# dkouzoup/ms-eetc

Hardware: AMD Instinct MI355X
Metric: OCP solves/sec (N=100, VIRM6, var-speed-limit track) (higher is better)
Workload: dtype f64

## Files before the change

__graft_entry__.py:

```python

import os
import subprocess
import sys
from pathlib import Path

ROOT = Path(__file__).resolve().parent
PKG = ROOT / 'ms-eetc_amd'

for p in (str(PKG), str(ROOT), str(ROOT / 'tests')):
    if p not in sys.path:
        sys.path.insert(0, p)

HIPCC = os.environ.get('HIPCC', '/opt/rocm/bin/hipcc')
HIP_FLAGS = ['--offload-arch=gfx950', '-O3', '-std=c++17', '-fPIC', '-shared', '-Wno-unused-value']
SOLVE_KERNEL_FLAGS = ['-fno-unroll-loops']


def _digest(sources, extra=()):

    import hashlib
    h = hashlib.sha256()
    for s in sources:
        h.update(s.name.encode()); h.update(s.read_bytes())
    for e in extra:
        h.update(str(e).encode())
    return h.hexdigest()


def _stale(target, digest):
    stamp = target.with_name(target.name + '.stamp')
    return (not target.exists()) or (not stamp.exists()) or stamp.read_text().strip() != digest


def _locked(path):

    import contextlib
    import fcntl

    @contextlib.contextmanager
    def cm():
        path.parent.mkdir(exist_ok=True)
        with open(path, 'w') as fh:
            fcntl.flock(fh, fcntl.LOCK_EX)
            try:
                yield
            finally:
                fcntl.flock(fh, fcntl.LOCK_UN)

    return cm()


def _jobs():

    if os.environ.get('MAX_JOBS', '').isdigit() and int(os.environ['MAX_JOBS']) > 0:
        return int(os.environ['MAX_JOBS'])
    n = len(os.sched_getaffinity(0))
    try:
        quota, period = open('/sys/fs/cgroup/cpu.max').read().split()[:2]
        if quota != 'max':
            n = min(n, max(1, int(float(quota)/float(period))))
    except Exception:
        pass
    return n


UNITS = ['msd_api.hip', 'msd_kernels_full.hip', 'msd_kernels_full2.hip', 'msd_kernels_full3.hip', 'msd_kernels_full4.hip', 'msd_kernels_rg.hip', 'msd_kernels_rg2.hip', 'msd_kernels_static.hip', 'msd_kernels_time.hip', 'msd_kernels_time2.hip', 'msd_kernels_dynamic.hip', 'msd_kernels_dynamic2.hip', 'msd_kernels_dynamic3.hip', 'msd_kernels_stream.hip', 'msd_kernels_stream2.hip', 'msd_kernels_stream3.hip', 'msd_kernels_stream4.hip', 'msd_kernels_stream5.hip', 'msd_kernels_stream6.hip', 'msd_kernels_stream7.hip', 'msd_kernels_compose.hip', 'msd_kernels_general.hip', 'msd_kernels_general2.hip', 'msd_kernels_intloss.hip', 'msd_kernels_intloss_table.hip', 'msd_kernels_intloss_table2.hip', 'msd_post.hip',
         'msd_integrators.hip', 'msd_mpc.hip']
SLOWEST_FIRST = ['msd_kernels_stream7.hip', 'msd_kernels_stream2.hip', 'msd_kernels_stream6.hip', 'msd_kernels_stream5.hip', 'msd_kernels_dynamic.hip', 'msd_kernels_stream3.hip',
                 'msd_kernels_stream4.hip', 'msd_kernels_intloss.hip', 'msd_kernels_compose.hip', 'msd_kernels_static.hip', 'msd_kernels_stream.hip']
HOST_UNITS = ('msd_api.hip', 'msd_mpc.hip')
HOST_ONLY_HEADERS = ('msd_handle.hpp', 'msd_select.hpp')


def _unit_headers(u):
    csrc = PKG / 'csrc'
    host = u in HOST_UNITS
    return ([h for h in sorted(csrc.glob('*.hpp')) if host or h.name not in HOST_ONLY_HEADERS] + [ROOT / 'include' / 'mseetc_hip.h']
            + ([ROOT / 'include' / 'mseetc_mpc.h', ROOT / 'include' / 'mseetc_aux.h'] if host else []))


def _hip_digest():
    csrc = PKG / 'csrc'
    deps = [csrc / u for u in UNITS] + sorted(csrc.glob('*.hpp')) + [ROOT / 'include' / 'mseetc_hip.h', ROOT / 'include' / 'mseetc_mpc.h', ROOT / 'include' / 'mseetc_aux.h']
    return _digest(deps, HIP_FLAGS + SOLVE_KERNEL_FLAGS)


def hip_digest():

    return _hip_digest()


def stale():

    return _stale(PKG / 'lib' / 'libmseetc_hip.so', _hip_digest())


def build(force=False):

    lib = PKG / 'lib' / 'libmseetc_hip.so'
    csrc = PKG / 'csrc'
    units = UNITS

    digest = _hip_digest()

    import contextlib
    from oracle import oracle
    fresh = not force and not _stale(lib, digest) and not oracle.stale()

    with (contextlib.nullcontext() if fresh else _locked(PKG / 'lib' / '.build.lock')):
        if force or _stale(lib, digest):
            objdir = PKG / 'lib' / 'obj'
            objdir.mkdir(exist_ok=True)
            flags = [f for f in HIP_FLAGS if f != '-shared']
            todo = []
            for u in units:
                fl = flags + (SOLVE_KERNEL_FLAGS if u.startswith('msd_kernels_') else [])
                obj = objdir / (u + '.o')
                dg = _digest([csrc / u] + _unit_headers(u), fl)
                if force or _stale(obj, dg):
                    todo.append((u, fl, obj, dg))
            from concurrent.futures import ThreadPoolExecutor
            todo.sort(key=lambda t: SLOWEST_FIRST.index(t[0]) if t[0] in SLOWEST_FIRST else len(SLOWEST_FIRST))
            with ThreadPoolExecutor(max_workers=_jobs()) as pool:
                codes = list(pool.map(lambda t: subprocess.call([HIPCC] + t[1] + ['-c', '-o', str(t[2]), str(csrc / t[0])]), todo))
            if any(codes):
                raise RuntimeError("hipcc failed: {}".format(codes))
            for u, fl, obj, dg in todo:
                obj.with_name(obj.name + '.stamp').write_text(dg)
            tmp = lib.with_name(lib.name + '.tmp')
            subprocess.run([HIPCC, '--offload-arch=gfx950', '-shared', '-fPIC', '-o', str(tmp)] + [str(objdir / (u + '.o')) for u in units], check=True)
            os.replace(tmp, lib)
            lib.with_name(lib.name + '.stamp').write_text(digest)

        oracle.build(force)

    import mseetc.ocp
    import mseetc._device

    return lib


def smoke():

    import numpy as np

    build()

    import cases
    from mseetc.ocp import casadiSolver
# ... 28 lines not shown
```

include/mseetc_aux.h:

```cpp
#ifndef MSEETC_AUX_H
#define MSEETC_AUX_H

#include "mseetc_hip.h"

#ifdef __cplusplus
extern "C" {
#endif

int msd_problem_time_first_pass(msd_handle h, int on);
int msd_problem_first_pass_ms(msd_handle h, float *mean_ms, int *launches);

int msd_host_alloc(unsigned long long bytes, void **ptr);
int msd_host_free(void *ptr);

int msd_problem_direct_results(msd_handle h, int on);

int msd_tuning(const char *name, int value);

int msd_plan_describe(const msd_problem_desc *desc, char *buf, int len);

int msd_fastmath_probe(int device, int n, const double *x, double *rcp_out, double *sqrt_out, double *rsqrt_out);

#ifdef __cplusplus
}
#endif
#endif
```

ms-eetc_amd/csrc/msd_api.hip:

```cpp
#include <hip/hip_runtime.h>
#include <dlfcn.h>

#include <algorithm>
#include <cmath>
#include <cstdio>
#include <cstdlib>
#include <cstring>
#include <map>
#include <mutex>
#include <string>
#include <utility>
#include <vector>

#include "msd_handle.hpp"

namespace {
thread_local std::string g_err;
}

#define MSD_KERNEL_UNITS(X) X(full) X(full2) X(full3) X(full4) X(rg) X(rg2) X(static) X(time) X(time2) X(dynamic) X(dynamic2) X(dynamic3) X(stream) X(stream2) X(stream3) \
    X(stream4) X(stream5) X(stream6) X(stream7) X(compose) X(general) X(general2) X(intloss) X(intloss_table) X(intloss_table2)
namespace msd {
#define X(unit) KernelFn kernels_##unit(const KernelId &id);
MSD_KERNEL_UNITS(X)
#undef X
}

namespace msd_host {
int fail(int code, const std::string &msg) { g_err = msg; return code; }
Tuning &tuning() { static Tuning t; return t; }

msd::KernelFn find_kernel(const msd::KernelId &id)
{
    if (!id) return nullptr;
#define X(unit) if (const msd::KernelFn fn = msd::kernels_##unit(id)) return fn;
    MSD_KERNEL_UNITS(X)
#undef X
    return nullptr;
}
bool has_kernel(const msd::KernelId &id) { return find_kernel(id) != nullptr; }
}
using msd_host::fail;

namespace msd_host {

int check_desc(const msd_problem_desc *d)
{
    if (d->abi_version != MSD_ABI_VERSION) return fail(MSD_E_INVALID, "ABI version mismatch");
    if (d->num_intervals < 1) return fail(MSD_E_INVALID, "Number of intervals must be a strictly positive integer!");
    if (d->max_iterations < 1) return fail(MSD_E_INVALID, "Maximum number of iterations must be a strictly positive integer!");
    if (d->num_steps < 1 || d->num_approx_steps < 0) return fail(MSD_E_INVALID, "bad integrator options");
    if (!d->ds || !d->grad || !d->curv || !d->bmax) return fail(MSD_E_INVALID, "null profile array");
    if (!(d->vmin_sq > 0) || !(d->obj_den > 0) || !(d->tol > 0)) return fail(MSD_E_INVALID, "vmin_sq, obj_den and tol must be positive");
    if (d->start_kind != MSD_START_REFERENCE && d->start_kind != MSD_START_PROFILE) return fail(MSD_E_INVALID, "unknown starting point");
    if (d->loss_kind < 0 || d->loss_kind > 2) return fail(MSD_E_UNSUPPORTED, "loss model not available on the device");
    if (d->loss_kind == 2) {
        if (!d->loss_table || d->loss_table_len < 13) return fail(MSD_E_INVALID, "dynamic loss model without its table");
        const int nx = (int)d->loss_table[11], ny = (int)d->loss_table[12];
        if (nx < 1 || ny < 1 || d->loss_table_len != 13 + (nx + 1) + (ny + 1) + 16*nx*ny) return fail(MSD_E_INVALID, "inconsistent loss table");
    }
    for (int i = 0; i < d->num_intervals; i++)
        if (!(d->ds[i] > 0)) return fail(MSD_E_INVALID, "interval lengths must be positive");
    if (d->integrator != 0 && d->integrator != MSD_INTEGRATOR_ADAPTIVE && d->integrator != MSD_INTEGRATOR_COLLOCATION)
        return fail(MSD_E_INVALID, "Unknown integration method!");
    if (d->integrator == MSD_INTEGRATOR_COLLOCATION) {
        if (d->coll_degree < 1 || d->coll_degree > 9) return fail(MSD_E_INVALID, "Order of implicit Runge-Kutta should be a positive integer between 1 and 9!");
        if (d->newton_iterations < 1) return fail(MSD_E_INVALID, "Maximum number of iterations must be a strictly positive integer!");
        if (!d->coll_tables) return fail(MSD_E_INVALID, "collocation integrator without its tables");
    }
    if (d->integrator == MSD_INTEGRATOR_ADAPTIVE && (!(d->int_abstol > 0) || !(d->int_reltol > 0))) return fail(MSD_E_INVALID, "tolerances of the adaptive integrator must be positive");
    if (d->integrate_losses && d->energy_optimal && d->loss_kind == 0)
        return fail(MSD_E_UNSUPPORTED, "integrateLosses needs a loss model (loss_kind 1 or 2)");
    if (d->integrate_losses && d->energy_optimal && d->loss_kind == 2 && d->integrator != 0)
        return fail(MSD_E_UNSUPPORTED, "integrateLosses with a loss table runs with explicit Runge-Kutta shooting (integrator 0)");
    return MSD_OK;
}


static int cu_count(int device, int *out)
{
    static std::mutex mu;
    static int cached[64] = {0};
    std::lock_guard<std::mutex> lock(mu);
    if (device < 64 && cached[device] > 0) { *out = cached[device]; return MSD_OK; }
    hipDeviceProp_t prop;
    HIP_TRY(hipGetDeviceProperties(&prop, device));
    if (device < 64) cached[device] = prop.multiProcessorCount;
    *out = prop.multiProcessorCount;
    return MSD_OK;
}

static int kernel_limits(int device, const void *fn, int threads, size_t lds, int *per_cu)
{
    struct Info { size_t lds_attr = 0; std::map<size_t, int> occupancy; };
    static std::mutex mu;
    static std::map<std::pair<int, const void *>, Info> cache;
    std::lock_guard<std::mutex> lock(mu);
    Info &info = cache[{device, fn}];
    if (lds > info.lds_attr) {
        HIP_TRY(hipFuncSetAttribute(fn, hipFuncAttributeMaxDynamicSharedMemorySize, (int)lds));
        info.lds_attr = lds;
    }
    const size_t step = 8*1024, top = std::min<size_t>(((lds + step - 1)/step)*step, 160*1024);
    auto it = info.occupancy.find(top);
    if (it == info.occupancy.end()) {
        int n = 0;
        if (hipOccupancyMaxActiveBlocksPerMultiprocessor(&n, fn, threads, top) != hipSuccess || n < 1) n = 1;
        it = info.occupancy.emplace(top, n).first;
    }
    *per_cu = it->second;
    return MSD_OK;
}


int select_plan(const msd_problem_desc *d, Plan *out, msd::KernelFn *soc_out)
{
    Plan &pl = *out;
    const int N = d->num_intervals;
    const Family family = family_of(d);
    const int structure = structure_of(d);
    const bool wide = msd_host::dyn_of(family) != msd::LOSS_STATIC;
    msd::Geometry geo = resident(family, N, structure, tuning());
    if (!geo.first || lds_bytes(geo, geo.first, N) > 160*1024) {
        geo = streamed(family, N, structure, tuning());
        if (!geo.first)
            return fail(MSD_E_UNSUPPORTED, family != STATIC ? "numIntervals = " + std::to_string(N) + " exceeds the 1023 intervals of the streamed kernels for the dynamic loss model, the collocation / adaptive shooting integrators and integrateLosses"
                                           : "numIntervals = " + std::to_string(N) + " exceeds the 5119 intervals of the streamed kernel");
    }
    size_t work2 = 0;
    if (!geo.follow) {
        geo.follow = streamed(family, N, structure, tuning()).follow;
        if (!geo.follow) return fail(MSD_E_UNSUPPORTED, "no follow-up kernel for numIntervals = " + std::to_string(N));
        work2 = msd::stream_doubles(N, geo.follow.NT*geo.follow.SPT, wide);
    }
    pl.NT = geo.first.NT; pl.SPT = geo.first.SPT; pl.lds_bytes = lds_bytes(geo, geo.first, N); pl.stream = geo.stream;
    pl.NT2 = geo.follow.NT; pl.SPT2 = geo.follow.SPT; pl.lds_bytes2 = lds_bytes(geo, geo.follow, N);
    fill_problem(pl.P, d);
    pl.fused_family = geo.xch == msd::XCH_FAST;
    pl.work_doubles = geo.stream ? msd::stream_doubles(N, pl.NT*pl.SPT, wide) : std::max(work2, msd::work_doubles(std::max(pl.NT*pl.SPT, work2 ? 0 : pl.NT2*pl.SPT2)));
    pl.nz = (4 + pl.P.withPn)*N + 2; pl.nl = ((pl.P.hasPower ? 2 : 0) + 3 + (pl.P.energyOpt ? 2 : 0))*N;
    pl.kernel = find_kernel(geo.first); pl.kernel2 = find_kernel(geo.follow); pl.kernel_lsq = find_kernel(geo.lsq);
    pl.kernel_soc = nullptr;
    *soc_out = find_kernel(geo.soc);
    return MSD_OK;
}

int make_plan(int device, const msd_problem_desc *d, Plan *out)
{
    Plan &pl = *out;
    msd::KernelFn soc = nullptr;
    int rc = select_plan(d, &pl, &soc);
    if (rc != MSD_OK) return rc;
    int per_cu = 0, cus = 0;
    rc = kernel_limits(device, (const void *)pl.kernel, pl.NT, pl.lds_bytes, &per_cu);
    if (rc != MSD_OK) return rc;
    rc = cu_count(device, &cus);
    if (rc != MSD_OK) return rc;
    pl.max_grid = per_cu*cus;
    pl.max_grid2 = 0;
    if (pl.kernel2) {
        rc = kernel_limits(device, (const void *)pl.kernel2, pl.NT2, pl.lds_bytes2, &per_cu);
        if (rc != MSD_OK) return rc;
        pl.max_grid2 = per_cu*cus;
    }
    pl.max_grid_lsq = 0;
    if (pl.kernel_lsq) {
        rc = kernel_limits(device, (const void *)pl.kernel_lsq, pl.NT, pl.lds_bytes, &per_cu);
        if (rc != MSD_OK) return rc;
        pl.max_grid_lsq = per_cu*cus;
    }
    if (soc) {
        int per_cu_soc = 0;
        if (kernel_limits(device, (const void *)soc, pl.NT, pl.lds_bytes, &per_cu_soc) == MSD_OK && per_cu_soc*cus >= pl.max_grid) pl.kernel_soc = soc;
    }
    return MSD_OK;
}

void pack_profile(const msd_problem_desc *d, double *out)
{
    const int N = d->num_intervals;
    double *ds = out, *grad = ds + N, *curv = grad + N, *bmax = curv + N, *pos = bmax + N + 1;
    memcpy(ds, d->ds, sizeof(double)*N); memcpy(grad, d->grad, sizeof(double)*N); memcpy(curv, d->curv, sizeof(double)*N);
    memcpy(bmax, d->bmax, sizeof(double)*(N + 1));
    pos[0] = 0;
    for (int i = 0; i < N; i++) pos[i + 1] = pos[i] + d->ds[i];
}

static std::string kernel_name(msd::KernelFn fn)
{
    if (!fn) return "-";
    static std::mutex mu;
    static std::map<const void *, std::string> cache;
    std::lock_guard<std::mutex> lock(mu);
    std::string &name = cache[(const void *)fn];
    if (name.empty()) {
        Dl_info info;
        name = (dladdr((const void *)fn, &info) && info.dli_sname && info.dli_saddr == (const void *)fn) ? info.dli_sname : "?";
    }
    return name;
}

std::string plan_text(const Plan &pl, msd::KernelFn soc)
{
    char buf[256];
    snprintf(buf, sizeof buf, "NT=%d SPT=%d lds_bytes=%zu stream=%d fused_family=%d work_doubles=%zu nz=%d nl=%d NT2=%d SPT2=%d lds_bytes2=%zu", pl.NT, pl.SPT, pl.lds_bytes,
             (int)pl.stream, (int)pl.fused_family, pl.work_doubles, pl.nz, pl.nl, pl.NT2, pl.SPT2, pl.lds_bytes2);
    return std::string(buf) + " kernel=" + kernel_name(pl.kernel) + " kernel_lsq=" + kernel_name(pl.kernel_lsq) + " kernel2=" + kernel_name(pl.kernel2) + " kernel_soc=" + kernel_name(soc);
}

int launch_plan(const Plan &pl, hipStream_t stream, double *d_work, int *d_follow, int *d_queue, int nscen, const double *d_scen, const double *d_ovr,
                double *d_z, double *d_lam, double *d_stats, double *d_hist, int hist_cap, const WarmStart &ws, int *d_list, hipEvent_t first_begin, hipEvent_t first_end)
{
    if (!pl.kernel) return fail(MSD_E_INVALID, "the handle holds no problem: its last (re)configuration failed");
    msd::DevProb P = pl.P;
    P.follow = nullptr; P.list = nullptr; P.queue = nullptr; P.socSeen = ws.d_soc_seen;
    P.guess = ws.d_guess; P.guessStride = ws.stride; P.guessStatus = ws.d_status; P.warmMu = ws.mu; P.warmPush = ws.push;
    P.dualIn = ws.d_dual_in; P.dualInStride = ws.dual_stride; P.dualShift = ws.dual_shift; P.dualOut = ws.d_dual_out;
    P.oneAttempt = ws.one_attempt ? 1 : 0;
    P.done = ws.d_done; P.statsHost = ws.d_stats_host; P.budget = ws.budget;
    const bool split = pl.kernel2 != nullptr;
    const bool plain = !pl.fused_family || (ws.d_guess ? ws.d_dual_in != nullptr : P.start == MSD_START_PROFILE);
    const bool first_pass = split && (plain || pl.kernel_lsq != nullptr);
    if (d_list && !first_pass) {
        const msd::KernelFn fn = split ? pl.kernel2 : pl.kernel;
        const int cap = split ? pl.max_grid2 : pl.max_grid;
        P.list = d_list;
        hipLaunchKernelGGL(fn, dim3(std::min(nscen, cap)), dim3(split ? pl.NT2 : pl.NT), split ? pl.lds_bytes2 : pl.lds_bytes, stream, P, nscen, d_scen, d_ovr, d_z, d_lam, d_stats, d_hist, hist_cap, d_work);
        HIP_TRY(hipGetLastError());
        return MSD_OK;
    }
    P.list = d_list;
    const msd::KernelFn fn = (split && !first_pass) ? pl.kernel2 : plain ? ((ws.use_soc && pl.kernel_soc) ? pl.kernel_soc : pl.kernel) : pl.kernel_lsq;
    const int cap = (split && !first_pass) ? pl.max_grid2 : plain ? pl.max_grid : pl.max_grid_lsq;
    const int grid = nscen < cap ? nscen : cap;
    const int threads = (split && !first_pass) ? pl.NT2 : pl.NT;
    const size_t lds_bytes = (split && !first_pass) ? pl.lds_bytes2 : pl.lds_bytes;
    if (first_pass) {
        if (!d_follow) return fail(MSD_E_INVALID, "split solve without its list");
        P.follow = d_follow;
    }
    if (nscen > grid && !d_list) {
        if (!d_queue) return fail(MSD_E_INVALID, "launch without its scenario counter");
        P.queue = d_queue;
        HIP_TRY(hipMemsetAsync(P.queue, 0, sizeof(int), stream));
    }
    if (first_begin) HIP_TRY(hipEventRecord(first_begin, stream));
    hipLaunchKernelGGL(fn, dim3(grid), dim3(threads), lds_bytes, stream, P, nscen, d_scen, d_ovr, d_z, d_lam, d_stats, d_hist, hist_cap, d_work);
    HIP_TRY(hipGetLastError());
    if (first_end) HIP_TRY(hipEventRecord(first_end, stream));
#ifdef MSD_DEBUG_HOOKS
    const bool skip_follow_up = getenv("MSD_DEBUG_NO_FOLLOW_UP") && *getenv("MSD_DEBUG_NO_FOLLOW_UP") == '1';
#else
    constexpr bool skip_follow_up = false;
#endif
    if (first_pass && !skip_follow_up) {
        const int grid2 = std::min(nscen, pl.max_grid2);
        P.queue = nullptr; P.list = d_follow; P.follow = nullptr;
        hipLaunchKernelGGL(pl.kernel2, dim3(grid2), dim3(pl.NT2), pl.lds_bytes2, stream, P, nscen, d_scen, d_ovr, d_z, d_lam, d_stats, d_hist, hist_cap, d_work);
        HIP_TRY(hipGetLastError());
    }
    return MSD_OK;
}

}

using msd_host::check_desc;

extern "C" {

const char *msd_last_error(void) { return g_err.c_str(); }

int msd_tuning(const char *name, int value)
{
    if (!name) return fail(MSD_E_INVALID, "null argument");
    if (!strcmp(name, "no_full")) msd_host::tuning().no_full = value != 0;
    else if (!strcmp(name, "two_nodes_per_lane")) msd_host::tuning().two_nodes_per_lane = value != 0;
    else return fail(MSD_E_INVALID, std::string("unknown tuning switch: ") + name);
    return MSD_OK;
}

int msd_plan_describe(const msd_problem_desc *d, char *buf, int len)
{
    if (!d || !buf || len < 1) return fail(MSD_E_INVALID, "null argument");
    int rc = check_desc(d);
    if (rc != MSD_OK) return rc;
    msd_host::Plan pl;
    msd::KernelFn soc = nullptr;
    rc = msd_host::select_plan(d, &pl, &soc);
    if (rc != MSD_OK) return rc;
    static const char *const family[] = {"STATIC", "DYNAMIC", "INTLOSS", "INTLOSS_TABLE", "GENERAL", "GENERAL_DYNAMIC", "GENERAL_INTLOSS"};
    static const char *const structure[] = {"0", "FULL_BOTH", "FULL_RG", "FULL_TIME_BOTH", "FULL_TIME_RG"};
    const std::string line = std::string("family=") + family[msd_host::family_of(d)] + " structure=" + structure[msd_host::structure_of(d)] + " " + msd_host::plan_text(pl, soc);
    if ((int)line.size() >= len) return fail(MSD_E_INVALID, "msd_plan_describe: the line needs " + std::to_string(line.size() + 1) + " bytes");
    memcpy(buf, line.c_str(), line.size() + 1);
    return MSD_OK;
}

int msd_device_count(void)
{
    int n = 0;
    if (hipGetDeviceCount(&n) != hipSuccess) return 0;
    return n;
}

static int configure(msd_problem *h, const msd_problem_desc *d)
{
    const int N = d->num_intervals;
    msd_host::Plan pl;
    int rc = msd_host::make_plan(h->device, d, &pl);
    if (rc != MSD_OK) return rc;
    HIP_TRY(hipSetDevice(h->device));
    HIP_TRY(hipStreamSynchronize(h->stream));
    h->plan.kernel = nullptr;

    const size_t len = msd_host::profile_doubles(N);
    if (N > h->cap_N) {
        hipFree(h->d_prof); h->d_prof = nullptr; h->cap_N = 0;
        HIP_TRY(hipMalloc((void **)&h->d_prof, sizeof(double)*len));
        h->cap_N = N;
    }
    if (len > h->cap_stage) {
        if (h->h_stage) hipHostFree(h->h_stage);
        h->h_stage = nullptr; h->cap_stage = 0;
        HIP_TRY(hipHostMalloc((void **)&h->h_stage, sizeof(double)*len, hipHostMallocDefault));
        h->cap_stage = len;
    }
    msd_host::pack_profile(d, h->h_stage);
    HIP_TRY(hipMemcpyAsync(h->d_prof, h->h_stage, sizeof(double)*len, hipMemcpyHostToDevice, h->stream));
    if (d->loss_kind == 2) {
        if (d->loss_table_len > h->cap_loss) {
            hipFree(h->d_loss); h->d_loss = nullptr; h->cap_loss = 0;
            HIP_TRY(hipMalloc((void **)&h->d_loss, sizeof(double)*d->loss_table_len));
            h->cap_loss = d->loss_table_len;
        }
        HIP_TRY(hipMemcpy(h->d_loss, d->loss_table, sizeof(double)*d->loss_table_len, hipMemcpyHostToDevice));
    }

    if (d->integrator == MSD_INTEGRATOR_COLLOCATION) {
        const int len = (d->coll_degree + 1)*(d->coll_degree + 2);
        if (!h->d_coll) HIP_TRY(hipMalloc((void **)&h->d_coll, sizeof(double)*10*11));
        HIP_TRY(hipMemcpy(h->d_coll, d->coll_tables, sizeof(double)*len, hipMemcpyHostToDevice));
    }

    msd_host::point_profile(pl.P, h->d_prof);
    pl.P.loss = (d->loss_kind == 2) ? h->d_loss : nullptr;
    pl.P.coll = (d->integrator == MSD_INTEGRATOR_COLLOCATION) ? h->d_coll : nullptr;
    if (pl.work_area() > h->cap_work) {
        hipFree(h->d_work); h->d_work = nullptr; h->cap_work = 0;
        HIP_TRY(hipMalloc((void **)&h->d_work, sizeof(double)*pl.work_area()));
        h->cap_work = pl.work_area();
    }
    if (pl.nz > h->cap_nz || pl.nl > h->cap_nl) {
        hipFree(h->d_scen); hipFree(h->d_ovr); hipFree(h->d_z); hipFree(h->d_lam); hipFree(h->d_stats); hipFree(h->d_guess); hipFree(h->d_z2); hipFree(h->d_stats2);
        h->d_scen = h->d_ovr = h->d_z = h->d_lam = h->d_stats = h->d_guess = h->d_z2 = h->d_stats2 = nullptr; h->cap_scen = 0; h->cap_guess = 0;
        h->prev_nscen = 0;
        h->cap_nz = pl.nz; h->cap_nl = pl.nl;
    }
    if (pl.kernel_soc && !h->h_soc_seen) {
        HIP_TRY(hipHostMalloc((void **)&h->h_soc_seen, sizeof(int), hipHostMallocMapped));
// ... 24 lines not shown
    *out = h;
    return MSD_OK;
}

int msd_problem_reconfigure(msd_handle h, const msd_problem_desc *d)
{
    if (!h || !d) return fail(MSD_E_INVALID, "null argument");
    if (h->begun) return fail(MSD_E_INVALID, "a batch begun with msd_solve_batch_begin has not been waited for (MSD_WAIT_ALL)");
    int rc = check_desc(d);
    if (rc == MSD_OK) rc = configure(h, d);
    if (rc != MSD_OK) h->plan.kernel = nullptr;
    return rc;
}

int msd_problem_destroy(msd_handle h)
{
    if (!h) return MSD_OK;
    if (h->attached_loops > 0) return fail(MSD_E_INVALID, "a receding-horizon loop (msd_mpc_create) still runs on this handle: destroy the loop first");
    hipSetDevice(h->device);
    if (h->begun) hipStreamSynchronize(h->stream);
    hipFree(h->d_prof); hipFree(h->d_loss); hipFree(h->d_work); hipFree(h->d_queue); hipFree(h->d_follow);
    hipFree(h->d_scen); hipFree(h->d_ovr); hipFree(h->d_z); hipFree(h->d_lam); hipFree(h->d_stats); hipFree(h->d_hist); hipFree(h->d_guess); hipFree(h->d_eval);
    hipFree(h->d_z2); hipFree(h->d_stats2); hipFree(h->d_dual); hipFree(h->d_dual2); hipFree(h->d_coll);
    if (h->h_stage) hipHostFree(h->h_stage);
    if (h->h_soc_seen) hipHostFree((void *)h->h_soc_seen);
    if (h->h_done) hipHostFree((void *)h->h_done);
    if (h->h_stats_now) hipHostFree(h->h_stats_now);
    if (h->ev_first) hipEventDestroy(h->ev_first);
    for (int k = 0; k < msd_problem::FP_RING; k++) { if (h->fp_beg[k]) hipEventDestroy(h->fp_beg[k]); if (h->fp_end[k]) hipEventDestroy(h->fp_end[k]); }
    if (h->ev0) hipEventDestroy(h->ev0);
    if (h->ev1) hipEventDestroy(h->ev1);
    if (h->stream) hipStreamDestroy(h->stream);
    delete h;
    return MSD_OK;
}

int msd_problem_nz(msd_handle h) { return h ? h->plan.nz : 0; }
int msd_problem_rows_per_interval(msd_handle h) { return h ? h->plan.nl/h->plan.P.N : 0; }

constexpr int QUEUE_RING = 64;

using msd_host::WarmStart;

static int launch(msd_handle h, int nscen, const double *d_scen, const double *d_ovr, double *d_z, double *d_lam, double *d_stats, double *d_hist, int hist_cap,
                  const WarmStart &ws_in = WarmStart())
{
    if (!h->plan.kernel) return fail(MSD_E_INVALID, "the handle holds no problem: its last (re)configuration failed");
    WarmStart ws = ws_in;
    ws.budget = h->budget;
    if (h->plan.kernel_soc) {
        ws.d_soc_seen = h->d_soc_seen;
        if (*h->h_soc_seen != 0) ws.use_soc = true;
    }
    if (h->plan.kernel2) {
        const size_t need = msd::FOLLOW_HDR + 2*(size_t)nscen;
        if (need > h->cap_follow) {
            HIP_TRY(hipStreamSynchronize(h->stream));
            int keep[msd::FOLLOW_HDR] = {0};
            if (h->d_follow) HIP_TRY(hipMemcpy(keep, h->d_follow, sizeof(int)*msd::FOLLOW_HDR, hipMemcpyDeviceToHost));
            keep[0] = keep[1] = keep[2] = 0;
            hipFree(h->d_follow); h->d_follow = nullptr; h->cap_follow = 0;
            HIP_TRY(hipMalloc((void **)&h->d_follow, sizeof(int)*need));
            HIP_TRY(hipMemcpy(h->d_follow, keep, sizeof(int)*msd::FOLLOW_HDR, hipMemcpyHostToDevice));
            h->cap_follow = need;
        }
    }
    if (!h->d_queue) HIP_TRY(hipMalloc((void **)&h->d_queue, sizeof(int)*QUEUE_RING));
    int *queue = h->d_queue + h->queue_slot;
    h->queue_slot = (h->queue_slot + 1) % QUEUE_RING;
    hipEvent_t e0 = nullptr, e1 = nullptr;
    if (h->time_first_pass && !ws.d_done) {
        const int k = (int)(h->fp_count % msd_problem::FP_RING);
        if (!h->fp_beg[k]) { HIP_TRY(hipEventCreate(&h->fp_beg[k])); HIP_TRY(hipEventCreate(&h->fp_end[k])); }
        e0 = h->fp_beg[k]; e1 = h->fp_end[k];
        h->fp_count++;
    }
    if (ws.d_done) e1 = h->ev_first;
#ifdef MSD_DEBUG_HOOKS
    if (getenv("MSD_DEBUG_PTRS"))
        fprintf(stderr, "[msd] launch nscen %d  work %p (+%zu B)  follow %p  queue %p  prof %p  scen %p  z %p  lam %p  stats %p  hist %p  %s  grid caps %d %d %d\n",
                nscen, (void *)h->d_work, sizeof(double)*h->cap_work, (void *)h->d_follow, (void *)queue, (void *)h->d_prof, (const void *)d_scen, (void *)d_z, (void *)d_lam, (void *)d_stats, (void *)d_hist,
                msd_host::plan_text(h->plan, h->plan.kernel_soc).c_str(), h->plan.max_grid, h->plan.max_grid_lsq, h->plan.max_grid2);
#endif
    return msd_host::launch_plan(h->plan, h->stream, h->d_work, h->d_follow, queue, nscen, d_scen, d_ovr, d_z, d_lam, d_stats, d_hist, hist_cap, ws, nullptr, e0, e1);
}

int msd_solve_batch_device(msd_handle h, int nscen, const double *d_scen, double *d_z, double *d_lam, double *d_stats)
{
    return msd_solve_batch_device_ex(h, nscen, d_scen, nullptr, d_z, d_lam, d_stats);
}

int msd_solve_batch_device_ex(msd_handle h, int nscen, const double *d_scen, const double *d_overrides, double *d_z, double *d_lam, double *d_stats)
{
    if (!h || nscen < 1 || !d_scen || !d_z || !d_stats) return fail(MSD_E_INVALID, "bad argument");
    if (h->begun) return fail(MSD_E_INVALID, "a batch begun with msd_solve_batch_begin has not been waited for (MSD_WAIT_ALL)");
    HIP_TRY(hipSetDevice(h->device));
    return launch(h, nscen, d_scen, d_overrides, d_z, d_lam, d_stats, nullptr, 0);
}

int msd_problem_geometry(msd_handle h, int *threads_per_scenario, int *nodes_per_thread)
{
    if (!h || !threads_per_scenario || !nodes_per_thread) return fail(MSD_E_INVALID, "bad argument");
    *threads_per_scenario = h->plan.NT; *nodes_per_thread = h->plan.SPT;
    return MSD_OK;
}

int msd_problem_follow_counts(msd_handle h, int *counts, int n)
{
    if (!h || !counts || n < 1) return fail(MSD_E_INVALID, "bad argument");
#ifdef MSD_DEBUG_HOOKS
    if (n > 9 && !(getenv("MSD_DEBUG_NO_FOLLOW_UP") && *getenv("MSD_DEBUG_NO_FOLLOW_UP") == '1')) n = 9;
#else
    if (n > 9) n = 9;
#endif
    if (n > (int)h->cap_follow - msd::FOLLOW_TOTAL && h->d_follow) n = (int)h->cap_follow - msd::FOLLOW_TOTAL;
    for (int k = 0; k < n; k++) counts[k] = 0;
    HIP_TRY(hipSetDevice(h->device));
    HIP_TRY(hipStreamSynchronize(h->stream));
    if (h->d_follow) HIP_TRY(hipMemcpy(counts, h->d_follow + msd::FOLLOW_TOTAL, sizeof(int)*n, hipMemcpyDeviceToHost));
    return MSD_OK;
}

int msd_problem_time_first_pass(msd_handle h, int on)
{
    if (!h) return fail(MSD_E_INVALID, "null handle");
    h->time_first_pass = on != 0; h->fp_count = 0;
    return MSD_OK;
}

int msd_problem_first_pass_ms(msd_handle h, float *mean_ms, int *launches)
{
    if (!h || !mean_ms || !launches) return fail(MSD_E_INVALID, "bad argument");
    HIP_TRY(hipSetDevice(h->device));
    HIP_TRY(hipStreamSynchronize(h->stream));
    const int n = (int)std::min<long long>(h->fp_count, msd_problem::FP_RING);
    double sum = 0;
    for (int k = 0; k < n; k++) { float ms = 0; HIP_TRY(hipEventElapsedTime(&ms, h->fp_beg[k], h->fp_end[k])); sum += ms; }
    *mean_ms = n ? (float)(sum/n) : 0.0f; *launches = n;
    return MSD_OK;
}

int msd_synchronize(msd_handle h)
{
    if (!h) return fail(MSD_E_INVALID, "null handle");
    HIP_TRY(hipSetDevice(h->device));
    HIP_TRY(hipStreamSynchronize(h->stream));
    return MSD_OK;
}

int msd_set_history(msd_handle h, double *host_hist, int cap)
{
    if (!h) return fail(MSD_E_INVALID, "null handle");
    h->h_hist = host_hist; h->hist_cap = host_hist ? cap : 0;
    return MSD_OK;
}

int msd_solve_batch(msd_handle h, int nscen, const double *scen, double *z_out, double *lam_out, double *stats, float *kernel_ms)
{
    return msd_solve_batch_ex(h, nscen, scen, nullptr, z_out, lam_out, stats, kernel_ms);
}

int msd_solve_batch_ex(msd_handle h, int nscen, const double *scen, const double *overrides, double *z_out, double *lam_out, double *stats, float *kernel_ms)
{
    return msd_solve_batch_warm(h, nscen, scen, overrides, nullptr, 0.0, 0.0, z_out, lam_out, stats, kernel_ms);
}

static int check_batch(msd_handle h, int nscen, const double *scen, const double *overrides, const double *z_guess, double mu_init, double bound_push,
// ... 372 lines not shown
```

ms-eetc_amd/csrc/msd_geometry.hpp:

```cpp
#pragma once

#include "msd_kernel.hpp"

namespace msd {

using KernelFn = void (*)(DevProb, int, const double *, const double *, double *, double *, double *, double *, int, double *);

struct KernelId {
    int NT = 0, SPT = 0, WPS = 1, DYN = LOSS_STATIC;
    bool STREAM = false, GEN = false;
    int FULL = 0, PART = 0;
    bool SLDS = false, SOCK = false;
    explicit operator bool() const { return NT != 0; }
};
inline bool operator==(const KernelId &a, const KernelId &b)
{
    return a.NT == b.NT && a.SPT == b.SPT && a.WPS == b.WPS && a.DYN == b.DYN && a.STREAM == b.STREAM && a.GEN == b.GEN && a.FULL == b.FULL && a.PART == b.PART
           && a.SLDS == b.SLDS && a.SOCK == b.SOCK;
}

#define MSD_KERNEL(...) if (id == KernelId{__VA_ARGS__}) return solve_kernel<__VA_ARGS__>;
#define MSD_KERNEL_UNUSED(...) if (false) return solve_kernel<__VA_ARGS__>;

struct Geometry {
    KernelId first;
    KernelId follow;
    KernelId lsq;
    KernelId soc;
    bool stream = false;
    int xch = XCH_GENERAL;
    int red = RED_DOUBLES;
    int extra = 0;
};

}
```

ms-eetc_amd/csrc/msd_handle.hpp:

```cpp
#pragma once
#include <hip/hip_runtime.h>

#include <algorithm>
#include <cmath>
#include <string>

#include "msd_kernel.hpp"
#include "msd_geometry.hpp"
#include "msd_select.hpp"
#include "../../include/mseetc_aux.h"

namespace msd_host {

int fail(int code, const std::string &msg);

#define HIP_TRY(expr)                                                                                               \
    do {                                                                                                            \
        hipError_t e_ = (expr);                                                                                     \
        if (e_ != hipSuccess) return msd_host::fail(MSD_E_HIP, std::string(#expr) + ": " + hipGetErrorString(e_));  \
    } while (0)

struct Plan {
    msd::DevProb P;
    int NT = 0, SPT = 0;
    size_t lds_bytes = 0;
    bool stream = false;
    msd::KernelFn kernel = nullptr;
    msd::KernelFn kernel_lsq = nullptr;
    msd::KernelFn kernel2 = nullptr;
    msd::KernelFn kernel_soc = nullptr;
    int NT2 = 0, SPT2 = 0;
    size_t lds_bytes2 = 0;
    int max_grid = 0, max_grid_lsq = 0, max_grid2 = 0;
    bool fused_family = false;
    size_t work_doubles = 0;
    size_t work_area() const { return work_doubles*(size_t)std::max(max_grid, std::max(max_grid2, max_grid_lsq)); }
    int nz = 0, nl = 0;
};

int check_desc(const msd_problem_desc *d);
int select_plan(const msd_problem_desc *d, Plan *out, msd::KernelFn *soc);
int make_plan(int device, const msd_problem_desc *d, Plan *out);
std::string plan_text(const Plan &pl, msd::KernelFn soc);

Tuning &tuning();
msd::KernelFn find_kernel(const msd::KernelId &id);

constexpr size_t profile_doubles(int N) { return 5*(size_t)N + 2; }
void pack_profile(const msd_problem_desc *d, double *out);
inline void point_profile(msd::DevProb &P, const double *d_prof) { P.ds = d_prof; P.grad = P.ds + P.N; P.curv = P.grad + P.N; P.bmax = P.curv + P.N; P.pos = P.bmax + P.N + 1; }

struct WarmStart { const double *d_guess = nullptr; long long stride = 0; const double *d_status = nullptr; double mu = 0, push = 0;
                   const double *d_dual_in = nullptr; long long dual_stride = 0; int dual_shift = 0; double *d_dual_out = nullptr;
                   bool one_attempt = false;
                   bool use_soc = false;
                   int *d_soc_seen = nullptr;
                   int *d_done = nullptr; double *d_stats_host = nullptr;
                   int budget = 0; };

int launch_plan(const Plan &pl, hipStream_t stream, double *d_work, int *d_follow, int *d_queue, int nscen, const double *d_scen, const double *d_ovr,
                double *d_z, double *d_lam, double *d_stats, double *d_hist, int hist_cap, const WarmStart &ws, int *d_list = nullptr,
                hipEvent_t first_begin = nullptr, hipEvent_t first_end = nullptr);

}

struct msd_problem {
    msd_host::Plan plan;
    int device = 0;
    volatile int *h_soc_seen = nullptr;
    int *d_soc_seen = nullptr;
    int *d_follow = nullptr; size_t cap_follow = 0;
    hipStream_t stream = nullptr;
    hipEvent_t ev0 = nullptr, ev1 = nullptr;
    double *d_prof = nullptr, *d_loss = nullptr;
    double *h_stage = nullptr; size_t cap_stage = 0;
    double *d_work = nullptr;
    double *d_eval = nullptr; size_t cap_eval = 0;
    int *d_queue = nullptr;
    int queue_slot = 0;
    size_t cap_work = 0;
    int cap_N = 0, cap_loss = 0, cap_nz = 0, cap_nl = 0;
    double *d_scen = nullptr, *d_ovr = nullptr, *d_z = nullptr, *d_lam = nullptr, *d_stats = nullptr, *d_hist = nullptr, *d_guess = nullptr;
    double *d_z2 = nullptr, *d_stats2 = nullptr;
    int prev_nscen = 0, prev_nz = 0, prev_stp = 0;
    bool direct_results = false, last_direct = false;
    bool keep_duals = false;
    double *d_dual = nullptr, *d_dual2 = nullptr;
    double *d_coll = nullptr;
    size_t cap_dual = 0;
    int prev_dual_nodes = 0;
    int cap_scen = 0, cap_guess = 0;
    double *h_hist = nullptr;
    int hist_cap = 0;
    static constexpr int FP_RING = 64;
    bool time_first_pass = false;
    hipEvent_t fp_beg[FP_RING] = {}, fp_end[FP_RING] = {};
    long long fp_count = 0;
    bool early_results = false;
    int budget = 0;
    volatile int *h_done = nullptr; int *d_done = nullptr;
    double *h_stats_now = nullptr, *d_stats_now = nullptr;
    int cap_done = 0;
    int begun = 0;
    hipEvent_t ev_first = nullptr;
    int attached_loops = 0;
};
```

ms-eetc_amd/csrc/msd_kernel.hpp:

```cpp
#pragma once
#include <type_traits>

#include <hip/hip_runtime.h>

#include <float.h>
#include <math.h>

#include "../../include/mseetc_hip.h"
#include "msd_fastmath.hpp"
#include "msd_scan.hpp"

#ifndef MSD_PHASE_FENCE
#define MSD_PHASE_FENCE 1
#endif
#ifndef MSD_FENCE_PHASES
#define MSD_FENCE_PHASES 0x155
#endif
#ifndef MSD_HOT_FENCES
#define MSD_HOT_FENCES 0
#endif
#ifndef MSD_FENCE_MAX_NT
#define MSD_FENCE_MAX_NT 256
#endif
#ifndef MSD_FENCE_DUALS
// ... 393 lines not shown
    c.red_slot++;
    if (c.lane == 0) {
#pragma unroll
        for (int k = 0; k < K; k++) buf[c.wave*RED_K + k] = v[k];
    }
    __syncthreads();
#pragma unroll
    for (int k = 0; k < K; k++) {
        double r = buf[k];
        for (int w = 1; w < c.nw; w++) r = op(r, buf[w*RED_K + k]);
        v[k] = r;
    }
}

#ifndef MSD_HOST_EMULATION
template <int K> __device__ __forceinline__ void wave_fetch(const double (&x)[K], double (&y)[K], int src)
{
    const int addr = (src & 63) << 2;
#pragma unroll
    for (int k = 0; k < K; k++) {
        const int lo = __builtin_amdgcn_ds_bpermute(addr, __double2loint(x[k]));
        const int hi = __builtin_amdgcn_ds_bpermute(addr, __double2hiint(x[k]));
        y[k] = __hiloint2double(hi, lo);
    }
}
#else
template <int K> __device__ __forceinline__ void wave_fetch(const double (&x)[K], double (&y)[K], int src)
{
    emu_wave_fetch(x, y, K, src);
}
#endif

__device__ __forceinline__ void bar_terms(double x, double lb, double ub, bool hasL, bool hasU, double zL, double zU, double mu, double &Sg, double &gphi)
{
    double S = 0, g = 0;
    if (hasL) { S += zL/(x - lb); g -= mu/(x - lb); }
    if (hasU) { S += zU/(ub - x); g += mu/(ub - x); }
    if (hasL && !hasU) g += K_D*mu;
    if (!hasL && hasU) g -= K_D*mu;
    Sg = S; gphi = g;
}

__device__ __forceinline__ double sigma_clamp(double z, double mu, double s)
{
    const double r = mu/s;
    return fmax(fmin(z, K_SIGMA*r), r*(1.0/K_SIGMA));
}

__device__ __forceinline__ double push_in(double x, double lb, double ub, bool hasL, bool hasU, double kp)
{
    if (hasL && hasU) {
        double pL = fmin(kp*fmax(1.0, fabs(lb)), kp*(ub - lb));
        double pU = fmin(kp*fmax(1.0, fabs(ub)), kp*(ub - lb));
        if (x < lb + pL) x = lb + pL;
        if (x > ub - pU) x = ub - pU;
    } else if (hasL) { double pL = kp*fmax(1.0, fabs(lb)); if (x < lb + pL) x = lb + pL; }
    else if (hasU) { double pU = kp*fmax(1.0, fabs(ub)); if (x > ub - pU) x = ub - pU; }
    return x;
}

__device__ __forceinline__ double hpow(double x, double y)
{
    static_assert(K_MU_SUP == 1.5, "mu^1.5 is computed as mu*sqrt(mu) in the barrier update");
#ifndef MSD_HPOW
#define MSD_HPOW 1
#endif
    return MSD_HPOW ? (double)exp2f((float)y*log2f((float)x)) : pow(x, y);
}

struct LogSum {
    double m = 1.0;
    int e = 0;
#ifndef MSD_LOGSUM
#define MSD_LOGSUM 1
#endif
    double acc = 0.0;
    __device__ __forceinline__ void add(double prod) { if (MSD_LOGSUM) { int ex; m *= frexp(prod, &ex); e += ex; } else acc += log(prod); }
    __device__ __forceinline__ double value() const { return MSD_LOGSUM ? log(m) + 0.6931471805599453*(double)e : acc; }
};

__device__ __forceinline__ bool cmp_le(double lhs, double rhs, double basval) { return lhs - rhs <= 10.0*DBL_EPSILON*fabs(basval); }

constexpr unsigned F_ON_T = 1u, F_ON_B = 2u, F_ON_F = 4u, F_ON_P = 8u, F_ON_S = 16u, F_IVAL = 32u, F_NODE = 64u;

template <int CNT, int NS, bool MEM> struct Field;
template <int CNT, int NS> struct Field<CNT, NS, false> {
    static constexpr bool in_memory = false;
    double v[CNT];
    __device__ __forceinline__ void bind(double *) {}
    __device__ __forceinline__ double &operator[](int k) { return v[k]; }
    __device__ __forceinline__ const double &operator[](int k) const { return v[k]; }
};
template <int CNT, int NS> struct Field<CNT, NS, true> {
    static constexpr bool in_memory = true;
    double *p;
    __device__ __forceinline__ void bind(double *q) { p = q; }
    __device__ __forceinline__ double &operator[](int k) const { return p[k*NS]; }
};

constexpr int W_X = 0, W_SG = 5, W_LAM = 10, W_NU = 12, W_ZL = 17, W_ZU = 22, W_ZLS = 27, W_ZUS = 32, W_DSG = 37, W_RESC = 42, W_RESD = 44,
              W_EV = 49, W_LG = 62, W_LG_FIELDS = 30, W_FIELDS_ITERATE = W_LG + W_LG_FIELDS;
constexpr int W_SC = W_FIELDS_ITERATE, W_RN = W_SC + 2, W_RP = W_SC + 9, W_RZN = W_SC + 16, W_RZP = W_SC + 23, W_RDN = W_SC + 30, W_RDP = W_SC + 37, W_RDZN = W_SC + 44,
              W_RDZP = W_SC + 51, W_XR = W_SC + 58, W_SGR = W_SC + 63, W_OZL = W_SC + 68, W_OZU = W_SC + 73, W_OZLS = W_SC + 78, W_OZUS = W_SC + 83, W_RD = W_SC + 88,
              W_DNU = W_SC + 90, W_RFILT = W_SC + 95, W_SCAL = W_SC + 97, W_RTMP = W_SC + 98;
constexpr int W_WD = W_SC + 103, W_WD_FIELDS = 37;
static_assert(W_DSG == W_WD_FIELDS, "the iterate proper: the fields in front of the slack steps");
constexpr int W_RX = W_WD + W_WD_FIELDS, W_RX_FIELDS = 6;
constexpr int W_FIELDS = W_RX + W_RX_FIELDS;
__host__ __device__ constexpr size_t work_doubles(int node_slots) { return (size_t)W_FIELDS*node_slots; }
__host__ __device__ constexpr size_t stream_doubles(int N, int node_slots, bool dyn)
{
    return (size_t)W_FIELDS*node_slots + (size_t)(dyn ? 31 : 27)*(N + 1) + 6*(size_t)node_slots;
}

template <int NS, bool STREAM>
struct Node {
    int i;
    unsigned flags;
    double ds, G, sct, scb, ubB;
    Field<NV, NS, STREAM> x;
    Field<NR, NS, STREAM> sg;
    Field<2, NS, STREAM> lam;
    Field<NR, NS, STREAM> nu;
    Field<NV, NS, STREAM> zL, zU;
    Field<NR, NS, STREAM> zLs, zUs;
    Field<NR, NS, STREAM> dsg;
    __device__ __forceinline__ void bind(double *w)
    {
        x.bind(w + W_X*NS); sg.bind(w + W_SG*NS); lam.bind(w + W_LAM*NS); nu.bind(w + W_NU*NS); zL.bind(w + W_ZL*NS); zU.bind(w + W_ZU*NS);
        zLs.bind(w + W_ZLS*NS); zUs.bind(w + W_ZUS*NS); dsg.bind(w + W_DSG*NS);
    }
    __device__ __forceinline__ bool ival() const { return (flags & F_IVAL) != 0; }
    __device__ __forceinline__ bool node() const { return (flags & F_NODE) != 0; }
    __device__ __forceinline__ bool on(int k) const { return (flags >> k) & 1u; }
};

struct Uni {
    double tlo, thi, blo, flo, fhi, plo, phi, slo;
    bool rowOn[NR], rL[NR], rU[NR];
    double dL[NR], dU[NR], rs[NR];
    double irs[NR];
    double sf;
};

#ifndef MSD_NODE_FENCE
#define MSD_NODE_FENCE 1
#endif
#ifndef MSD_NODE_FENCE_SITES
#define MSD_NODE_FENCE_SITES 0xFFFu
#endif
template <int SITE> __device__ __forceinline__ void node_fence() { if (MSD_NODE_FENCE && ((MSD_NODE_FENCE_SITES >> SITE) & 1u)) __builtin_amdgcn_sched_barrier(0); }

__device__ __forceinline__ void opaque(double &v) { asm volatile("" : "+v"(v)); }
#ifndef MSD_FENCE_AGPR
#define MSD_FENCE_AGPR 0
#endif
__device__ __forceinline__ void opaque_a(double &v) { asm volatile("" : "+a"(v)); }
__device__ __forceinline__ void opaque_z(double &v) { if (MSD_FENCE_AGPR >= 1) opaque_a(v); else opaque(v); }
__device__ __forceinline__ void opaque_d(double &v) { if (MSD_FENCE_AGPR >= 2) opaque_a(v); else opaque(v); }

__device__ __forceinline__ void publish_done(int *word, int v)
{
#ifdef MSD_HOST_EMULATION
    __atomic_store_n(word, v, __ATOMIC_RELEASE);
#else
    __hip_atomic_store(word, v, __ATOMIC_RELEASE, __HIP_MEMORY_SCOPE_SYSTEM);
// ... 974 lines not shown
            for (int k = 0; k < 2; k++)
#pragma unroll
                for (int m = 0; m < LGW; m++) lgs[j][LGW*k + m] = e.lg[k][m];
        }
    }
    __device__ __forceinline__ void load_ev(int j, Ev &e) const
    {
        e.sb = evs[j][0]; e.sb1 = evs[j][1]; e.b1 = evs[j][2]; e.tb = evs[j][3]; e.tw = evs[j][4]; e.tbb = evs[j][5]; e.tbw = evs[j][6]; e.tww = evs[j][7];
        e.Bb = evs[j][8]; e.Bw = evs[j][9]; e.Bbb = evs[j][10]; e.Bbw = evs[j][11]; e.Bww = evs[j][12];
#pragma unroll
        for (int k = 0; k < 2; k++)
#pragma unroll
            for (int m = 0; m < LGW; m++) e.lg[k][m] = DYN ? lgs[j][LGW*k + m] : 0.0;
    }
    __device__ __forceinline__ void load_ev1(int j, Ev &e) const
    {
        e.sb = evs[j][0]; e.sb1 = evs[j][1]; e.b1 = evs[j][2]; e.tb = evs[j][3]; e.tw = evs[j][4]; e.Bb = evs[j][8]; e.Bw = evs[j][9];
        e.tbb = e.tbw = e.tww = e.Bbb = e.Bbw = e.Bww = 0;
#pragma unroll
        for (int k = 0; k < 2; k++)
#pragma unroll
            for (int m = 0; m < LGW; m++) e.lg[k][m] = DYN ? lgs[j][LGW*k + m] : 0.0;
    }
    static constexpr unsigned H_X = 1u, H_SG = 2u, H_LAM = 4u, H_NU = 8u, H_Z = 16u, H_ZS = 32u, H_DSG = 64u, H_RES = 128u, H_EV = 256u, H_ALL = 511u;
    template <int CNT, class F> __device__ __forceinline__ void put(const F &f, int off, int slot)
    {
        if constexpr (!F::in_memory) {
#pragma unroll
            for (int k = 0; k < CNT; k++) work[(off + k)*NS + slot] = f.v[k];
        }
    }
    template <int CNT, class F> __device__ __forceinline__ void get(F &f, int off, int slot)
    {
        if constexpr (!F::in_memory) {
#pragma unroll
            for (int k = 0; k < CNT; k++) f.v[k] = work[(off + k)*NS + slot];
        }
    }
    template <unsigned M, int BASE = 0> __device__ __forceinline__ void stash()
    {
#pragma unroll
        for (int j = 0; j < SPT; j++) {
            NodeT &nd = n[j];
            const int sl = nd.i + BASE*NS;
            if (M & H_X) put<NV>(nd.x, W_X, sl);
            if (M & H_SG) put<NR>(nd.sg, W_SG, sl);
            if (M & H_LAM) put<2>(nd.lam, W_LAM, sl);
            if (M & H_NU) put<NR>(nd.nu, W_NU, sl);
            if (M & H_Z) { put<NV>(nd.zL, W_ZL, sl); put<NV>(nd.zU, W_ZU, sl); }
            if (M & H_ZS) { put<NR>(nd.zLs, W_ZLS, sl); put<NR>(nd.zUs, W_ZUS, sl); }
            if (M & H_DSG) put<NR>(nd.dsg, W_DSG, sl);
            if (M & H_RES) { put<2>(resc[j], W_RESC, sl); put<NR>(resd[j], W_RESD, sl); }
            if (M & H_EV) { put<13>(evs[j], W_EV, sl); if (DYN) put<2*LGW>(lgs[j], W_LG, sl); }
        }
        asm volatile("" ::: "memory");
    }
    template <unsigned M> __device__ __forceinline__ void fetch()
    {
        asm volatile("" ::: "memory");
#pragma unroll
        for (int j = 0; j < SPT; j++) {
            NodeT &nd = n[j];
            const int sl = nd.i;
            if (M & H_X) get<NV>(nd.x, W_X, sl);
            if (M & H_SG) get<NR>(nd.sg, W_SG, sl);
            if (M & H_LAM) get<2>(nd.lam, W_LAM, sl);
            if (M & H_NU) get<NR>(nd.nu, W_NU, sl);
            if (M & H_Z) { get<NV>(nd.zL, W_ZL, sl); get<NV>(nd.zU, W_ZU, sl); }
            if (M & H_ZS) { get<NR>(nd.zLs, W_ZLS, sl); get<NR>(nd.zUs, W_ZUS, sl); }
            if (M & H_DSG) get<NR>(nd.dsg, W_DSG, sl);
            if (M & H_RES) { get<2>(resc[j], W_RESC, sl); get<NR>(resd[j], W_RESD, sl); }
            if (M & H_EV) { get<13>(evs[j], W_EV, sl); if (DYN) get<2*LGW>(lgs[j], W_LG, sl); }
        }
    }

    template <class F> __device__ static __forceinline__ void fence_v(F &f, int k) { if constexpr (!F::in_memory) opaque(f.v[k]); }
    template <class F> __device__ static __forceinline__ void fence_z(F &f, int k) { if constexpr (!F::in_memory) opaque_z(f.v[k]); }
    template <class F> __device__ static __forceinline__ void fence_d(F &f, int k) { if constexpr (!F::in_memory) opaque_d(f.v[k]); }
    template <class F> __device__ static __forceinline__ void fence_a(F &f, int k) { if constexpr (!F::in_memory) opaque_a(f.v[k]); }

    __device__ __forceinline__ double lbv(int k) const { return k == VT ? U.tlo : k == VB ? U.blo : k == VF ? U.flo : k == VP ? U.plo : U.slo; }
    __device__ __forceinline__ double ubv(int j, int k) const { return k == VT ? U.thi : k == VB ? n[j].ubB : k == VF ? U.fhi : k == VP ? U.phi : INFINITY; }
    __device__ static __forceinline__ bool hasU(int k) { return k != VS; }

    __device__ __forceinline__ void phase_fence(int phase)
    {
#if MSD_PHASE_FENCE
        if (!MSD_HOT_FENCES && (PART == 1 || PART == 3) && FAST) return;
        if (!((MSD_FENCE_PHASES >> phase) & 1)) return;
        if (NT > MSD_FENCE_MAX_NT || STREAM) return;
#pragma unroll
        for (int j = 0; j < SPT; j++) {
            NodeT &nd = n[j];
#pragma unroll
            for (int k = 0; k < NV; k++) { fence_v(nd.x, k); if (MSD_FENCE_DUALS) { fence_z(nd.zL, k); fence_z(nd.zU, k); } }
#pragma unroll
            for (int r = 0; r < NR; r++) { fence_v(nd.sg, r); if (MSD_FENCE_DUALS) { fence_d(nd.nu, r); fence_z(nd.zLs, r); fence_z(nd.zUs, r); fence_d(nd.dsg, r); fence_d(resd[j], r); } }
            if (MSD_FENCE_DUALS) { fence_d(nd.lam, 0); fence_d(nd.lam, 1); fence_d(resc[j], 0); fence_d(resc[j], 1); }
        }
#endif
    }

    __device__ __forceinline__ void commit_uniforms(const Uni &u)
    {
        __syncthreads();
        if (c.tid == 0) U = u;
        __syncthreads();
    }

    __device__ __forceinline__ void publish(const double (&x)[SPT][NV])
    {
        __syncthreads();
#pragma unroll
        for (int j = 0; j < SPT; j++) { const int i = n[j].i; c.xt[i] = x[j][VT]; c.xb[i] = x[j][VB]; c.xf[i] = x[j][VF]; }
        __syncthreads();
    }
    __device__ __forceinline__ void publish_current()
    {
        __syncthreads();
#pragma unroll
        for (int j = 0; j < SPT; j++) { const int i = n[j].i; c.xt[i] = n[j].x[VT]; c.xb[i] = n[j].x[VB]; c.xf[i] = n[j].x[VF]; }
        __syncthreads();
    }
    __device__ __forceinline__ double nb_q(int j) const { return (n[j].i > 0 && n[j].node()) ? c.xf[n[j].i - 1] : 0.0; }

    __device__ __forceinline__ void var_terms(int j, int k, double mu_, double &Sg, double &gphi) const
    {
        bar_terms(n[j].x[k], lbv(k), ubv(j, k), true, hasU(k), n[j].zL[k], n[j].zU[k], mu_, Sg, gphi);
    }
    __device__ __forceinline__ void row_terms(int j, int r, double mu_, double &Sg, double &gphi) const
    {
        bar_terms(n[j].sg[r], U.dL[r], U.dU[r], rL(r), rU(r), n[j].zLs[r], n[j].zUs[r], mu_, Sg, gphi);
    }

    struct LossHess { double bb, bf, bp, bd, ff, fp, fd, pp, pd, dd; };
    __device__ __forceinline__ LossHess loss_hess(double f, double b, const Ev &ev) const
    {
        const double Xv = ev.lg[0][1], Xd = ev.lg[0][2], Xw = ev.lg[0][3], Xvv = ev.lg[0][4], Xvd = ev.lg[1][0], Xvw = ev.lg[1][1], Xdd = ev.lg[1][2],
                     Xdw = ev.lg[1][3], Xww = ev.lg[1][4];
        const double vb = 0.5/ev.sb, vbb = -0.25/(b*ev.sb);
        LossHess L;
        L.bb = f*(Xvv*vb*vb + Xv*vbb); L.bf = f*Xvw*vb + Xv*vb; L.bp = f*Xvw*vb; L.bd = f*Xvd*vb;
        L.ff = f*Xww + 2*Xw; L.fp = f*Xww + Xw; L.fd = f*Xdw + Xd; L.pp = f*Xww; L.pd = f*Xdw; L.dd = f*Xdd;
        return L;
    }
    __device__ __forceinline__ LossHess rows_hess(int j, double f, double b, const Ev &ev) const
    {
        LossHess L;
        if constexpr (ITAB) {
            const double vb = 0.5/ev.sb, vbb = -0.25/(b*ev.sb);
            L.bb = L.bf = L.bp = L.bd = L.ff = L.fp = L.fd = L.pp = L.pd = L.dd = 0;
#pragma unroll
            for (int k = 0; k < 2; k++) {
                const int r = (k == 0) ? RLTR : RLRG;
                const double wk = -n[j].nu[r]*U.rs[r];
                const double *E = ev.lg[k];
                const double g0 = E[1], h00 = E[5 + j4h(0, 0)], h01 = E[5 + j4h(0, 1)], h02 = E[5 + j4h(0, 2)], h03 = E[5 + j4h(0, 3)], h11 = E[5 + j4h(1, 1)],
                             h12 = E[5 + j4h(1, 2)], h13 = E[5 + j4h(1, 3)], h22 = E[5 + j4h(2, 2)], h23 = E[5 + j4h(2, 3)], h33 = E[5 + j4h(3, 3)];
                L.bb += wk*(h00*vb*vb + g0*vbb); L.bf += wk*(h02 + h03)*vb; L.bp += wk*h02*vb; L.bd += wk*h01*vb;
                L.ff += wk*(h22 + 2*h23 + h33); L.fp += wk*(h22 + h23); L.fd += wk*(h12 + h13); L.pp += wk*h22; L.pd += wk*h12; L.dd += wk*h11;
            }
        } else {
            L = loss_hess(f, b, ev);
            const double W = n[j].nu[RLTR]*U.rs[RLTR]*(-P.ct) + n[j].nu[RLRG]*U.rs[RLRG]*P.cr;
            L.bb *= W; L.bf *= W; L.bp *= W; L.bd *= W; L.ff *= W; L.fp *= W; L.fd *= W; L.pp *= W; L.pd *= W; L.dd *= W;
        }
        return L;
    }

    __device__ __forceinline__ void row_grads(int j, const Ev &ev, double (&gb)[NR], double (&gf)[NR], double (&gp)[NR], double (&gs)[NR], double (&gb1)[NR],
                                              double (&gd)[NR]) const
    {
        const double f = n[j].x[VF];
#pragma unroll
        for (int r = 0; r < NR; r++) { gb[r] = gf[r] = gp[r] = gs[r] = gb1[r] = gd[r] = 0; }
        gf[RPW0] = ev.sb; gb[RPW0] = 0.5*f/ev.sb;
        gf[RPW1] = ev.sb1; gb1[RPW1] = 0.5*f/ev.sb1;
        gf[RACC] = 1; gp[RACC] = withPn() ? 1.0 : 0.0; gb[RACC] = -(0.5*P.sr1/ev.sb + P.sr2);
        if (DYN == LOSS_INTEGRATED_TABLE) {
            const double vb = 0.5/ev.sb;
#pragma unroll
            for (int k = 0; k < 2; k++) {
                const int r = (k == 0) ? RLTR : RLRG;
                gs[r] = 1; gf[r] = -(ev.lg[k][3] + ev.lg[k][4]); gp[r] = withPn() ? -ev.lg[k][3] : 0.0; gb[r] = -ev.lg[k][1]*vb; gd[r] = -ev.lg[k][2];
            }
        } else if (DYN == LOSS_INTEGRATED) {
            const double X = ev.lg[0][0], Xv = ev.lg[0][1], Xd = ev.lg[0][2], Xw = ev.lg[0][3], vb = 0.5/ev.sb;
#pragma unroll
            for (int k = 0; k < 2; k++) {
                const int r = (k == 0) ? RLTR : RLRG;
                const double kap = (k == 0) ? -P.ct : P.cr;
                gs[r] = 1; gf[r] = kap*(X + f*Xw); gp[r] = withPn() ? kap*f*Xw : 0.0; gb[r] = kap*f*Xv*vb; gd[r] = kap*f*Xd;
            }
        } else if (DYN == LOSS_TABLE) {
            const double vb = 0.25/ev.sb, vb1 = 0.25/ev.sb1;
            gs[RLTR] = 1; gf[RLTR] = -ev.lg[0][0]; gb[RLTR] = -ev.lg[0][1]*vb; gb1[RLTR] = -ev.lg[0][1]*vb1;
            gs[RLRG] = 1; gf[RLRG] = -ev.lg[1][0]; gb[RLRG] = -ev.lg[1][1]*vb; gb1[RLRG] = -ev.lg[1][1]*vb1;
        } else {
            gs[RLTR] = 1; gf[RLTR] = -P.ct;
            gs[RLRG] = 1; gf[RLRG] = P.cr;
        }
#pragma unroll
        for (int r = 0; r < NR; r++) { gb[r] *= U.rs[r]; gf[r] *= U.rs[r]; gp[r] *= U.rs[r]; gs[r] *= U.rs[r]; gb1[r] *= U.rs[r]; gd[r] *= U.rs[r]; }
    }
    __device__ __forceinline__ void fold_running_time(const Ev &ev, double (&gb)[NR], double (&gf)[NR], double (&gp)[NR], const double (&gd)[NR]) const
    {
        if (!INTEG) return;
#pragma unroll
        for (int r = RLTR; r <= RLRG; r++) { gb[r] += gd[r]*ev.tb; gf[r] += gd[r]*ev.tw; if (withPn()) gp[r] += gd[r]*ev.tw; }
    }

    __device__ __forceinline__ void obj_grads(int j, double q, double &of, double &op, double &os, double &oq, double &off, double &opp) const
    {
        const double sc = U.sf/P.objDen;
        of = op = os = oq = off = opp = 0;
        if (!n[j].ival()) return;
        const double f = n[j].x[VF], p = withPn() ? n[j].x[VP] : 0.0;
        if (energyOpt()) {
            of = sc*n[j].ds; os = INTEG ? sc : sc*n[j].ds;
            if (n[j].i > 0) { of += sc*2e-3*(f - q); oq = -sc*2e-3*(f - q); off = sc*2e-3; }
        } else {
            of = sc*2e-4*f; off = sc*2e-4;
            if (withPn()) { op = sc*2e-4*p; opp = sc*2e-4; }
        }
    }

    struct Dir { double dx[NV], lt, lb; };
    __device__ __forceinline__ void load_dir(int j, Dir &d) const
    {
        const NodeT &nd = n[j];
#pragma unroll
        for (int k = 0; k < NV; k++) d.dx[k] = 0;
        d.lt = d.lb = 0;
        if (!nd.node()) return;
        const double *s = c.S + nd.i*S_STRIDE;
        if (nd.on(VT)) d.dx[VT] = s[S_DT];
        if (nd.on(VB)) d.dx[VB] = s[S_DB];
        if (nd.ival()) {
            if (nd.on(VF)) d.dx[VF] = s[S_DF];
            if (nd.on(VP)) d.dx[VP] = s[S_DP];
            if (nd.on(VS)) d.dx[VS] = s[S_DS];
            d.lt = s[S_LT]; d.lb = s[S_LB];
        }
    }

    struct Err { double dual, primal, primal_u, cmax, cmin, sd, sc, theta, L, D, obj; };

    struct RsSums { double theta, np, lognp, prox; };
    __device__ __forceinline__ void kkt_pass(Err &E, const bool resto = false, const double eta = 0.0, const double rho = 0.0, RsSums *RS = nullptr)
    {
        Ev e[SPT];
#pragma unroll
        for (int j = 0; j < SPT; j++) load_ev1(j, e[j]);
        double gl[SPT][NV];
        double dual = 0, prim = 0, prim_u = 0, cmax = -INFINITY, cmin = INFINITY, sumlam = 0, sumz = 0, nlam = 0, nz = 0;
        double th = 0, logs = 0, damp = 0, obj = 0;
        double rs_th = 0, rs_np = 0, rs_log = 0, rs_prox = 0, rs_prim = 0;
        LogSum lsum;
#pragma unroll
        for (int j = 0; j < SPT; j++) {
            node_fence<0>();
            const NodeT &nd = n[j];
            const double q = nb_q(j);
            double out_q = 0, out_t1 = 0, out_b1 = 0, prod = 1.0;
#pragma unroll
            for (int k = 0; k < NV; k++) gl[j][k] = 0;
            if (nd.ival()) {
                double gb[NR], gf[NR], gp[NR], gs[NR], gb1[NR], gd[NR];
                row_grads(j, e[j], gb, gf, gp, gs, gb1, gd);
                double of, op, os, oq, off, opp;
                obj_grads(j, q, of, op, os, oq, off, opp);
                if (resto) { of = op = os = oq = 0; }
                gl[j][VF] = of; gl[j][VP] = op; gl[j][VS] = os; out_q = oq;
#pragma unroll
                for (int r = 0; r < NR; r++) {
                    if (!rowOn(r)) continue;
                    gl[j][VB] += nd.nu[r]*gb[r]; gl[j][VF] += nd.nu[r]*gf[r]; gl[j][VP] += nd.nu[r]*gp[r]; gl[j][VS] += nd.nu[r]*gs[r]; out_b1 += nd.nu[r]*gb1[r];
                    if (INTEG) { out_t1 += nd.nu[r]*gd[r]; gl[j][VT] -= nd.nu[r]*gd[r]; }
                }
                out_t1 += nd.lam[0]; gl[j][VT] -= nd.lam[0];
                gl[j][VB] -= nd.lam[0]*e[j].tb + nd.lam[1]*e[j].Bb;
                gl[j][VF] -= nd.lam[0]*e[j].tw + nd.lam[1]*e[j].Bw;
                if (withPn()) gl[j][VP] -= nd.lam[0]*e[j].tw + nd.lam[1]*e[j].Bw;
                out_b1 += nd.lam[1];
                prim = fmax(prim, fmax(nd.sct*fabs(resc[j][0]), nd.scb*fabs(resc[j][1])));
                prim_u = fmax(prim_u, fmax(fabs(resc[j][0]), fabs(resc[j][1])));
                th += nd.sct*fabs(resc[j][0]) + nd.scb*fabs(resc[j][1]);
                sumlam += fabs(nd.lam[0])/nd.sct + fabs(nd.lam[1])/nd.scb; nlam += 2;
#pragma unroll
                for (int r = 0; r < NR; r++) {
                    if (!rowOn(r)) continue;
                    const double viol = fabs(resd[j][r]);
                    prim = fmax(prim, viol); prim_u = fmax(prim_u, viol/U.rs[r]); th += viol;
                    sumlam += fabs(nd.nu[r]); nlam += 1;
                    double gsl = -nd.nu[r];
                    if (rL(r)) { const double s = nd.sg[r] - U.dL[r]; gsl -= nd.zLs[r]; const double cp = s*nd.zLs[r]; cmax = fmax(cmax, cp); cmin = fmin(cmin, cp); sumz += nd.zLs[r]; nz += 1; prod *= s; }
                    if (rU(r)) { const double s = U.dU[r] - nd.sg[r]; gsl += nd.zUs[r]; const double cp = s*nd.zUs[r]; cmax = fmax(cmax, cp); cmin = fmin(cmin, cp); sumz += nd.zUs[r]; nz += 1; prod *= s; }
                    if (rL(r) && !rU(r)) damp += nd.sg[r] - U.dL[r];
                    if (!rL(r) && rU(r)) damp += U.dU[r] - nd.sg[r];
                    dual = fmax(dual, fabs(gsl));
                }
                if (resto) {
#pragma unroll
                    for (int jr = 0; jr < 2 + NR; jr++) {
                        if (!rs_on(jr)) continue;
                        const double row = jr == 0 ? nd.sct*resc[j][0] : jr == 1 ? nd.scb*resc[j][1] : resd[j][jr >= 2 ? jr - 2 : 0];
                        const double y = jr == 0 ? nd.lam[0]/nd.sct : jr == 1 ? nd.lam[1]/nd.scb : nd.nu[jr >= 2 ? jr - 2 : 0];
                        const double rn = wf(W_RN + jr, nd.i), rp = wf(W_RP + jr, nd.i), zn = wf(W_RZN + jr, nd.i), zp = wf(W_RZP + jr, nd.i);
                        const double v = fabs(row + rn - rp);
                        rs_prim = fmax(rs_prim, v); rs_th += v;
                        dual = fmax(dual, fmax(fabs(rho + y - zn), fabs(rho - y - zp)));
                        cmax = fmax(cmax, fmax(rn*zn, rp*zp)); cmin = fmin(cmin, fmin(rn*zn, rp*zp));
                        sumz += zn + zp; nz += 2;
                        rs_np += rn + rp; rs_log += log(rn) + log(rp);
                    }
                }
            } else if (nd.i == P.N && !energyOpt() && !resto) gl[j][VT] = U.sf/P.objDen;
            if (nd.node()) {
#pragma unroll
                for (int k = 0; k < NV; k++) {
                    if (!nd.on(k)) continue;
                    prod *= nd.x[k] - lbv(k);
                    if (hasU(k)) prod *= ubv(j, k) - nd.x[k];
                    else damp += nd.x[k] - lbv(k);
// ... 574 lines not shown
    __device__ __forceinline__ bool acceptable(bool okt, double th_t, double ph_t, double th_ref, double phi, double alpha_test, double gphid, bool ftype,
                                              double theta_max, double theta_min, int nfilt) const
    {
        if (!okt || th_t > theta_max) return false;
        bool acc;
        if (ftype && th_ref <= theta_min) acc = cmp_le(ph_t - phi, ETA_PHI*alpha_test*gphid, phi);
        else acc = cmp_le(th_t, (1 - G_THETA)*th_ref, th_ref) || cmp_le(ph_t - phi, -G_PHI*th_ref, phi);
        return acc && filter_ok(nfilt, th_t, ph_t);
    }

    __device__ __forceinline__ void profile_start(double t0, double tEnd, double v0sq, double vNsq)
    {
        const int N = P.N;
        constexpr double A = 0.3, MARG = 0.97*0.97, BFL = 25.0, S0 = 0.02, TFR = 0.995;
        const double L = P.pos[N], span = tEnd - t0;
        double cs = L/span;
        double cap[SPT], up[SPT], dn[SPT];
#pragma unroll
        for (int j = 0; j < SPT; j++) {
            const int i = n[j].i;
            const double ps = (i <= N) ? P.pos[i] : L;
            cap[j] = (i >= 1 && i < N) ? MARG*P.bmax[i] : INFINITY;
            up[j] = v0sq + 2*A*ps; dn[j] = vNsq + 2*A*(L - ps);
        }
#pragma unroll 1
        for (int it = 0; it < 3; it++) {
#pragma unroll
            for (int j = 0; j < SPT; j++) {
                const int i = n[j].i;
                double bi = fmin(fmin(cap[j], cs*cs), fmin(up[j], dn[j]));
                if (i == 0) bi = v0sq;
                if (i == N) bi = vNsq;
                n[j].x[VB] = bi;
                if (i <= N) { c.xb[i] = sqrt(bi); c.o2[i] = bi; }
            }
            __syncthreads();
            double tt = 0;
#pragma unroll
            for (int j = 0; j < SPT; j++) {
                if (!n[j].ival()) continue;
                const int i = n[j].i;
                const double dti = 2*n[j].ds/(c.xb[i] + c.xb[i + 1]);
                c.o1[i] = dti; tt += dti;
            }
            double v[1] = {tt};
            block_reduce<1>(v, OpSum(), c);
            if (it < 2) cs *= uni(v[0])/(span*TFR);
            __syncthreads();
        }
        if (c.tid == 0) {
            double acc = t0;
            for (int i = 0; i <= N; i++) { c.xt[i] = fmin(acc, tEnd); if (i < N) acc += c.o1[i]; }
        }
        __syncthreads();
#pragma unroll
        for (int j = 0; j < SPT; j++) {
            NodeT &nd = n[j];
            const int i = nd.i;
            if (!nd.node()) continue;
            nd.x[VT] = c.xt[i];
            if (!nd.ival()) continue;
            const double b0 = c.o2[i], b1 = c.o2[i + 1], v0 = c.xb[i], v1 = c.xb[i + 1];
            const double bs0 = fmax(b0, BFL), bs1 = fmax(b1, BFL);
            const double vm = 0.5*(sqrt(bs0) + sqrt(bs1));
            const double f = (bs1 - bs0)/(2*nd.ds) + P.sr0 + P.sr1*vm + P.sr2*vm*vm + nd.G;
            double fel = fmin(fmax(f, P.fmin), P.fmax);
            if (hasPower()) { const double vmx = fmax(v0, v1); fel = fmin(fmax(fel, -fabs(P.pwL)/vmx), fabs(P.pwU)/vmx); }
            double fpb = 0.0;
            if (withPn()) {
                const double pb = K_PUSH*fmin(1.0, fabs(P.fminPn));
                fpb = fmin(fmin(fmax(f - fel, P.fminPn), 0.0), -pb);
                fel = fmin(fmax(f - fpb, P.fmin), P.fmax);
                if (hasPower()) { const double vmx = fmax(v0, v1); fel = fmin(fmax(fel, -fabs(P.pwL)/vmx), fabs(P.pwU)/vmx); }
            }
            double sl;
            if (DYN == LOSS_TABLE || ITAB) { const DynLoss D(P.loss, P.lossCoef, P.lossMass); double lr[2][6]; loss_rows(D, fel, 0.5*(v0 + v1), lr); sl = fmax(lr[0][0], lr[1][0])*(ITAB ? nd.ds : 1.0) + S0; }
            else sl = fmax(P.ct*fel, -P.cr*fel)*(INTEG ? nd.ds : 1.0) + S0;
            nd.x[VF] = fel; nd.x[VP] = fpb; nd.x[VS] = sl;
        }
        __syncthreads();
    }

    static constexpr bool FAST = full_energy(FULL) && DYN == LOSS_STATIC && !STREAM && !GEN && MSD_PARALLEL_RICCATI;
    static constexpr int HV = 6;
    double cnt_lam = 0, cnt_z = 0;

    __device__ static __forceinline__ double step_to(double x, double alpha, double d) { return fma(alpha, d, x); }

    static constexpr bool STATIC_LDS = SLDS;
    __device__ __forceinline__ void store_static()
    {
        if constexpr (STATIC_LDS) {
#pragma unroll
            for (int j = 0; j < SPT; j++) { const NodeT &nd = n[j]; const int i = nd.i; c.st[i] = nd.ds; c.st[NS + i] = nd.G; c.st[2*NS + i] = nd.sct; c.st[3*NS + i] = nd.scb; c.st[4*NS + i] = nd.ubB; }
            __syncthreads();
        }
    }
    template <int WHAT> __device__ __forceinline__ void load_static(int j)
    {
        if constexpr (STATIC_LDS) {
            NodeT &nd = n[j]; const int i = nd.i;
            if (WHAT & 1) { nd.ds = c.st[i]; nd.G = c.st[NS + i]; }
            if (WHAT & 2) { nd.sct = c.st[2*NS + i]; nd.scb = c.st[3*NS + i]; }
            if (WHAT & 4) nd.ubB = c.st[4*NS + i];
        }
    }

    __device__ __forceinline__ void publish_fast(const double (&x)[SPT][NV])
    {
        __syncthreads();
#pragma unroll
        for (int j = 0; j < SPT; j++) { const int i = n[j].i; c.xt[i] = x[j][VT]; c.xb[i] = x[j][VB]; c.xs[i] = fsqrt(x[j][VB]); c.xf[i] = x[j][VF]; }
        __syncthreads();
    }

    struct RowG { double g0f, g0b, g1f, g1b1, g2f, g2b, g3f, g3s, g4f, g4s; };
    __device__ __forceinline__ RowG row_grads_fast(double f, double sb, double sb1, double isb, double isb1) const
    {
        RowG g;
        const double r0 = U.rs[RPW0], r1 = U.rs[RPW1], r2 = U.rs[RACC], r3 = U.rs[RLTR], r4 = U.rs[RLRG];
        g.g0f = r0*sb; g.g0b = r0*(0.5*f*isb);
        g.g1f = r1*sb1; g.g1b1 = r1*(0.5*f*isb1);
        g.g2f = r2; g.g2b = -r2*(0.5*P.sr1*isb + P.sr2);
        g.g3f = -r3*P.ct; g.g3s = r3; g.g4f = r4*P.cr; g.g4s = r4;
        return g;
    }

    __device__ __forceinline__ void fused_pass(const bool MERIT, Err &E, double (&h0)[SPT][HV], double (&h1)[SPT][HV], const double dw = 0.0, const bool soc = false)
    {
        const int N = P.N;
        double dual = 0, prim = 0, prim_u = 0, cmax = -INFINITY, cmin = INFINITY, sumlam = 0, sumz = 0, nlam = 0, nz = 0;
        double th = 0, damp = 0, obj = 0;
        LogSum lsum;
        double gl[SPT][NV], Hbb_[SPT], Hbq_[SPT], resd[SPT][NR];
        const double sc = U.sf/P.objDen;
#pragma unroll
        for (int j = 0; j < SPT; j++) {
            node_fence<0>();
            load_static<7>(j);
            NodeT &nd = n[j];
            const int i = nd.i;
            double Htt = 0, Hbb = 0, Hbq = 0, Hbf = 0, Hbp = 0, Hqq = 0, Hqf = 0, Hff = 0, Hfp = 0, Hfs = 0, Hpp = 0, Hss = 0;
            double a0[HV] = {0, 0, 0, 0, 0, 0}, a1[HV] = {0, 0, 0, 0, 0, 0};
            double nHbb = 0, nHbq = 0, nhb0 = 0, nhb1 = 0, out_q = 0, out_t1 = 0, out_b1 = 0, prod = 1.0;
            double tb = 0, tw = 0, Bb = 0, Bw = 0, rt = 0, rb = 0, oa = 0;
#pragma unroll
            for (int k = 0; k < NV; k++) gl[j][k] = 0;
#pragma unroll
            for (int r = 0; r < NR; r++) resd[j][r] = 0;
            if (nd.ival()) {
                const double t = nd.x[VT], b = nd.x[VB], f = nd.x[VF], p = withPn() ? nd.x[VP] : 0.0, s = nd.x[VS];
                const double t1 = c.xt[i + 1], b1 = c.xb[i + 1], sb = c.xs[i], sb1 = c.xs[i + 1];
                const double q = (i > 0) ? c.xf[i - 1] : 0.0;
                Jet tau, bp;
                interval_map<Jet, true>(P, b, f + p, nd.G, nd.ds, tau, bp);
                double cv0_ = t1 - (t + tau.v), cv1_ = b1 - bp.v;
                if constexpr (SOCK) { if (soc) { cv0_ = wf(W_RESC, i); cv1_ = wf(W_RESC + 1, i); } }
                const double cv0 = cv0_, cv1 = cv1_;
                tb = tau.g0; tw = tau.g1; Bb = bp.g0; Bw = bp.g1; rt = -cv0; rb = -cv1;
                const double isb = frcp(sb), isb1 = frcp(sb1);
                const RowG g = row_grads_fast(f, sb, sb1, isb, isb1);
                double dv[NR];
                dv[RPW0] = U.rs[RPW0]*f*sb; dv[RPW1] = U.rs[RPW1]*f*sb1;
                dv[RACC] = U.rs[RACC]*(f + p - (P.sr0 + P.sr1*sb + P.sr2*b) - nd.G);
                dv[RLTR] = U.rs[RLTR]*(s - P.ct*f); dv[RLRG] = U.rs[RLRG]*(s + P.cr*f);
                double of = sc*nd.ds, oq = 0, off = 0;
                const double os = sc*nd.ds;
                if (i > 0) { of += sc*2e-3*(f - q); oq = -sc*2e-3*(f - q); off = sc*2e-3; }
                const double l0 = nd.lam[0], l1 = nd.lam[1];
                const double dyn_w = l0*tw + l1*Bw;
                gl[j][VT] = -l0;
                gl[j][VB] = nd.nu[RPW0]*g.g0b + nd.nu[RACC]*g.g2b - (l0*tb + l1*Bb);
                gl[j][VF] = of + nd.nu[RPW0]*g.g0f + nd.nu[RPW1]*g.g1f + nd.nu[RACC]*g.g2f + nd.nu[RLTR]*g.g3f + nd.nu[RLRG]*g.g4f - dyn_w;
                if (withPn()) gl[j][VP] = nd.nu[RACC]*g.g2f - dyn_w;
                gl[j][VS] = os + nd.nu[RLTR]*g.g3s + nd.nu[RLRG]*g.g4s;
                out_q = oq; out_t1 = l0; out_b1 = nd.nu[RPW1]*g.g1b1 + l1;
                prim = fmax(prim, fmax(nd.sct*fabs(cv0), nd.scb*fabs(cv1)));
                prim_u = fmax(prim_u, fmax(fabs(cv0), fabs(cv1)));
                if (MERIT) th += nd.sct*fabs(cv0) + nd.scb*fabs(cv1);
                sumlam += fabs(l0)*frcp(nd.sct) + fabs(l1)*frcp(nd.scb); if (MERIT) nlam += 2;
                a0[2] = oq; a0[3] = of; a0[5] = os;
                Hff = off;
                if (i > 0) { Hqq = off; Hqf = -off; }
                {
                    const double hbb = -(l0*tau.h00 + l1*bp.h00), hbw = -(l0*tau.h01 + l1*bp.h01), hww = -(l0*tau.h11 + l1*bp.h11);
                    Hbb += hbb; Hbf += hbw; Hff += hww;
                    if (withPn()) { Hbp += hbw; Hfp += hww; Hpp += hww; }
                }
                {
                    const double ib = isb*isb, ib1 = isb1*isb1;
                    Hbf += nd.nu[RPW0]*U.rs[RPW0]*0.5*isb; Hbb += nd.nu[RPW0]*U.rs[RPW0]*(-0.25*f*(ib*isb));
                    nHbq += nd.nu[RPW1]*U.rs[RPW1]*0.5*isb1; nHbb += nd.nu[RPW1]*U.rs[RPW1]*(-0.25*f*(ib1*isb1));
                    Hbb += nd.nu[RACC]*U.rs[RACC]*0.25*P.sr1*(ib*isb);
                }
                double Sg[NR], c0[NR], c1[NR];
#pragma unroll
                for (int r = 0; r < NR; r++) {
                    double rd0_ = dv[r] - nd.sg[r];
                    if constexpr (SOCK) { if (soc) rd0_ = wf(W_RESD + r, i); }
                    const double rd_ = rd0_;
                    resd[j][r] = rd_;
                    const double viol = fabs(rd_);
                    prim = fmax(prim, viol); prim_u = fmax(prim_u, viol*U.irs[r]);
                    if (MERIT) th += viol;
                    sumlam += fabs(nd.nu[r]); if (MERIT) nlam += 1;
                    double gsl = -nd.nu[r], S_, g1_;
                    {
                        const double sl = nd.sg[r] - U.dL[r], z = nd.zLs[r], ri = frcp(sl), cp = sl*z;
                        gsl -= z; cmax = fmax(cmax, cp); cmin = fmin(cmin, cp); sumz += z; nz += 1; prod *= sl;
                        S_ = z*ri; g1_ = -ri;
                    }
                    if (r <= RACC) {
                        const double su = U.dU[r] - nd.sg[r], z = nd.zUs[r], ri = frcp(su), cp = su*z;
                        gsl += z; cmax = fmax(cmax, cp); cmin = fmin(cmin, cp); sumz += z; nz += 1; prod *= su;
                        S_ += z*ri; g1_ += ri;
                    } else { g1_ += K_D; if (MERIT) damp += nd.sg[r] - U.dL[r]; }
                    dual = fmax(dual, fabs(gsl));
                    S_ += dw;
                    Sg[r] = S_; c0[r] = S_*rd_; c1[r] = g1_;
                }
                a0[1] += c0[RPW0]*g.g0b + c0[RACC]*g.g2b;                       a1[1] += c1[RPW0]*g.g0b + c1[RACC]*g.g2b;
                a0[3] += c0[RPW0]*g.g0f + c0[RPW1]*g.g1f + c0[RACC]*g.g2f + c0[RLTR]*g.g3f + c0[RLRG]*g.g4f;
                a1[3] += c1[RPW0]*g.g0f + c1[RPW1]*g.g1f + c1[RACC]*g.g2f + c1[RLTR]*g.g3f + c1[RLRG]*g.g4f;
                if (withPn()) { a0[4] += c0[RACC]*g.g2f; a1[4] += c1[RACC]*g.g2f; }
                a0[5] += c0[RLTR]*g.g3s + c0[RLRG]*g.g4s;                        a1[5] += c1[RLTR]*g.g3s + c1[RLRG]*g.g4s;
                nhb0 = c0[RPW1]*g.g1b1; nhb1 = c1[RPW1]*g.g1b1;
                Hbb += Sg[RPW0]*g.g0b*g.g0b + Sg[RACC]*g.g2b*g.g2b;
                Hbf += Sg[RPW0]*g.g0b*g.g0f + Sg[RACC]*g.g2b*g.g2f;
                if (withPn()) Hbp += Sg[RACC]*g.g2b*g.g2f;
                oa = off + (Sg[RPW0]*g.g0f*g.g0f + Sg[RPW1]*g.g1f*g.g1f + Sg[RLTR]*g.g3f*g.g3f + Sg[RLRG]*g.g4f*g.g4f);
                Hff += Sg[RPW0]*g.g0f*g.g0f + Sg[RPW1]*g.g1f*g.g1f + Sg[RACC]*g.g2f*g.g2f + Sg[RLTR]*g.g3f*g.g3f + Sg[RLRG]*g.g4f*g.g4f;
                if (withPn()) { Hfp += Sg[RACC]*g.g2f*g.g2f; Hpp += Sg[RACC]*g.g2f*g.g2f; }
                Hfs += Sg[RLTR]*g.g3f*g.g3s + Sg[RLRG]*g.g4f*g.g4s;
                Hss += Sg[RLTR]*g.g3s*g.g3s + Sg[RLRG]*g.g4s*g.g4s;
                nHbq += Sg[RPW1]*g.g1f*g.g1b1; nHbb += Sg[RPW1]*g.g1b1*g.g1b1;
            }
            if (nd.node()) {
                double Sv[NV], g1v[NV];
#pragma unroll
                for (int k = 0; k < NV; k++) {
                    Sv[k] = 0; g1v[k] = 0;
                    if ((k == VP && !withPn()) || !nd.on(k)) continue;
                    {
                        const double sl = nd.x[k] - lbv(k), z = nd.zL[k], ri = frcp(sl), cp = sl*z;
                        gl[j][k] -= z; cmax = fmax(cmax, cp); cmin = fmin(cmin, cp); sumz += z; nz += 1; prod *= sl;
                        Sv[k] = z*ri; g1v[k] = -ri;
                    }
                    if (hasU(k)) {
                        const double su = ubv(j, k) - nd.x[k], z = nd.zU[k], ri = frcp(su), cp = su*z;
                        gl[j][k] += z; cmax = fmax(cmax, cp); cmin = fmin(cmin, cp); sumz += z; nz += 1; prod *= su;
                        Sv[k] += z*ri; g1v[k] += ri;
                    } else { g1v[k] += K_D; if (MERIT) damp += nd.x[k] - lbv(k); }
                    Sv[k] += dw;
                }
                Htt += Sv[VT]; a1[0] += g1v[VT]; Hbb += Sv[VB]; a1[1] += g1v[VB]; Hff += Sv[VF]; a1[3] += g1v[VF]; Hpp += Sv[VP]; a1[4] += g1v[VP];
                Hss += Sv[VS]; a1[5] += g1v[VS];
                if (MERIT) {
                    double xl[NV];
#pragma unroll
                    for (int k = 0; k < NV; k++) xl[k] = nd.x[k];
                    obj += objective_term<false, FULL>(P, nd, xl, (i > 0) ? c.xf[i - 1] : 0.0, U.sf);
                }
                double *sB = c.S + i*S_STRIDE;
                if (nd.ival()) {
                    sB[S_TB] = tb; sB[S_TW] = tw; sB[S_BB] = Bb; sB[S_BW] = Bw; sB[S_RT] = rt; sB[S_RB] = rb;
                    const bool last = i == N - 1;
                    const double is = (Hss > 0) ? frcp(Hss) : NAN;
                    oa += Sv[VF];
                    if (!last) {
                        const double wf = Hfs*is;
                        Hff -= Hfs*wf; a0[3] -= wf*a0[5]; a1[3] -= wf*a1[5]; oa -= Hfs*wf;
                    }
                    sB[S_GFS] = Hfs; sB[S_IS] = is;
                    if (withPn()) { sB[S_OA] = oa; sB[S_OB] = Sv[VP]; }
                }
                sB[S_HTT] = Htt; sB[S_HBF] = Hbf; sB[S_HBP] = Hbp; sB[S_HQQ] = Hqq; sB[S_HQF] = Hqf; sB[S_HFF] = Hff; sB[S_HFP] = Hfp; sB[S_HPP] = Hpp;
            }
            Hbb_[j] = Hbb; Hbq_[j] = Hbq;
#pragma unroll
            for (int k = 0; k < HV; k++) { h0[j][k] = a0[k]; h1[j][k] = a1[k]; }
            if (MERIT) lsum.add(prod);
            c.o1[i] = nHbb; c.o2[i] = nHbq; c.o3[i] = nhb0; c.o4[i] = nhb1; c.o5[i] = out_q; c.o6[i] = out_t1; c.o7[i] = out_b1;
        }
        __syncthreads();
#pragma unroll
        for (int j = 0; j < SPT; j++) {
            node_fence<0>();
            const NodeT &nd = n[j];
            if (!nd.node()) continue;
            const int i = nd.i;
            double Hbb = Hbb_[j], Hbq = Hbq_[j];
            if (i > 0) {
                Hbb += c.o1[i - 1]; Hbq += c.o2[i - 1]; h0[j][1] += c.o3[i - 1]; h1[j][1] += c.o4[i - 1];
                gl[j][VT] += c.o6[i - 1]; gl[j][VB] += c.o7[i - 1];
            }
            if (i + 1 < N) gl[j][VF] += c.o5[i + 1];
            double *sB = c.S + i*S_STRIDE;
            sB[S_HBB] = Hbb; sB[S_HBQ] = Hbq;
#pragma unroll
            for (int k = 0; k < NV; k++) if (!(k == VP && !withPn()) && nd.on(k)) dual = fmax(dual, fabs(gl[j][k]));
        }
        __syncthreads();
#pragma unroll
        for (int j = 0; j < SPT; j++) {
            const int i = n[j].i;
            c.o1[i] = resd[j][RPW0]; c.o2[i] = resd[j][RPW1]; c.o3[i] = resd[j][RACC]; c.o4[i] = resd[j][RLTR]; c.o6[i] = resd[j][RLRG];
        }
        double vm[5] = {dual, prim, prim_u, cmax, -cmin};
        block_reduce<5>(vm, OpMax(), c);
        E.dual = uni(vm[0]); E.primal = uni(vm[1]); E.primal_u = uni(vm[2]); E.cmax = uni(vm[3]); E.cmin = -uni(vm[4]);
        if (MERIT) {
            double vs[8] = {sumlam, sumz, nlam, nz, th, lsum.value(), damp, obj};
            block_reduce<8>(vs, OpSum(), c);
            E.sd = uni(fmax(K_SMAX, (vs[0] + vs[1])/fmax(1.0, vs[2] + vs[3]))/K_SMAX);
            E.sc = uni(fmax(K_SMAX, vs[1]/fmax(1.0, vs[3]))/K_SMAX);
            E.theta = uni(vs[4]); E.L = uni(vs[5]); E.D = uni(vs[6]); E.obj = uni(vs[7]);
            cnt_lam = uni(vs[2]); cnt_z = uni(vs[3]);
        } else {
            double vs[2] = {sumlam, sumz};
            block_reduce<2>(vs, OpSum(), c);
            E.sd = uni(fmax(K_SMAX, (vs[0] + vs[1])/fmax(1.0, cnt_lam + cnt_z))/K_SMAX);
            E.sc = uni(fmax(K_SMAX, vs[1]/fmax(1.0, cnt_z))/K_SMAX);
        }
    }

    __device__ __forceinline__ void finish_blocks(const double (&h0)[SPT][HV], const double (&h1)[SPT][HV], double mu_)
    {
#pragma unroll
        for (int j = 0; j < SPT; j++) {
            const NodeT &nd = n[j];
            if (!nd.node()) continue;
            double *sB = c.S + nd.i*S_STRIDE;
            sB[S_HT] = h0[j][0] + mu_*h1[j][0]; sB[S_HB] = h0[j][1] + mu_*h1[j][1]; sB[S_HQ] = h0[j][2] + mu_*h1[j][2];
            sB[S_HF] = h0[j][3] + mu_*h1[j][3]; sB[S_HP] = h0[j][4] + mu_*h1[j][4];
            if (nd.ival()) sB[S_GS] = h0[j][5] + mu_*h1[j][5];
        }
        __syncthreads();
    }

    __device__ __forceinline__ void post_direction(double mu_, double tau_, double &gphid, double &dnorm, bool &tiny_step, double &amax, double &adu)
    {
        const int N = P.N;
        finish_direction();
        const double sc = U.sf/P.objDen;
        double gd = 0, dn = 0, rel = -1.0, rp = 0, rd = 0;
#pragma unroll
        for (int j = 0; j < SPT; j++) {
            node_fence<9>();
            load_static<5>(j);
            NodeT &nd = n[j];
#pragma unroll
            for (int r = 0; r < NR; r++) nd.dsg[r] = 0;
            if (!nd.node()) continue;
            const int i = nd.i;
            Dir d; load_dir(j, d);
            double og[NV] = {0, 0, 0, 0, 0};
            if (nd.ival()) {
                const double f = nd.x[VF], sb = c.xs[i], sb1 = c.xs[i + 1];
                const double q = (i > 0) ? c.xf[i - 1] : 0.0;
                og[VF] = sc*nd.ds; og[VS] = sc*nd.ds;
                if (i > 0) og[VF] += sc*2e-3*(f - q);
                if (i + 1 < N) og[VF] += c.o5[i + 1];
                const double isb = frcp(sb), isb1 = frcp(sb1);
                const RowG g = row_grads_fast(f, sb, sb1, isb, isb1);
                const double db1 = c.S[(i + 1)*S_STRIDE + S_DB];
                nd.dsg[RPW0] = c.o1[i] + (g.g0b*d.dx[VB] + g.g0f*d.dx[VF]);
                nd.dsg[RPW1] = c.o2[i] + (g.g1f*d.dx[VF] + g.g1b1*db1);
                nd.dsg[RACC] = c.o3[i] + (g.g2b*d.dx[VB] + g.g2f*d.dx[VF] + g.g2f*d.dx[VP]);
                nd.dsg[RLTR] = c.o4[i] + (g.g3f*d.dx[VF] + g.g3s*d.dx[VS]);
                nd.dsg[RLRG] = c.o6[i] + (g.g4f*d.dx[VF] + g.g4s*d.dx[VS]);
            }
#pragma unroll
            for (int k = 0; k < NV; k++) {
                if ((k == VP && !withPn()) || !nd.on(k)) continue;
                const double dk = d.dx[k];
                double gp;
                {
                    const double s = nd.x[k] - lbv(k), z = nd.zL[k], w = frcp(s*z), r = z*w, iz = s*w;
                    gp = -mu_*r; rp = fmax(rp, -dk*r);
                    rd = fmax(rd, -(r*(mu_ - z*dk) - z)*iz);
                }
                if (hasU(k)) {
                    const double s = ubv(j, k) - nd.x[k], z = nd.zU[k], w = frcp(s*z), r = z*w, iz = s*w;
                    gp += mu_*r; rp = fmax(rp, dk*r);
                    rd = fmax(rd, -(r*(mu_ + z*dk) - z)*iz);
                } else gp += K_D*mu_;
                gd += (og[k] + gp)*dk;
                dn = fmax(dn, fabs(dk)); rel = fmax(rel, fabs(dk) - 10*DBL_EPSILON*(1 + fabs(nd.x[k])));
            }
            if (nd.ival()) {
#pragma unroll
                for (int r_ = 0; r_ < NR; r_++) {
                    const double dk = nd.dsg[r_];
                    double gp;
                    {
                        const double s = nd.sg[r_] - U.dL[r_], z = nd.zLs[r_], w = frcp(s*z), r = z*w, iz = s*w;
                        gp = -mu_*r; rp = fmax(rp, -dk*r);
                        rd = fmax(rd, -(r*(mu_ - z*dk) - z)*iz);
                    }
                    if (r_ <= RACC) {
                        const double s = U.dU[r_] - nd.sg[r_], z = nd.zUs[r_], w = frcp(s*z), r = z*w, iz = s*w;
                        gp += mu_*r; rp = fmax(rp, dk*r);
                        rd = fmax(rd, -(r*(mu_ + z*dk) - z)*iz);
                    } else gp += K_D*mu_;
                    gd += gp*dk;
                    dn = fmax(dn, fabs(dk)); rel = fmax(rel, fabs(dk) - 10*DBL_EPSILON*(1 + fabs(nd.sg[r_])));
                }
            }
        }
        double v1[1] = {gd}; block_reduce<1>(v1, OpSum(), c);
        double v2[4] = {dn, rel, rp, rd}; block_reduce<4>(v2, OpMax(), c);
        gphid = uni(v1[0]); dnorm = uni(v2[0]); tiny_step = uni(v2[1]) < 0;
        const double rpm = uni(v2[2]), rdm = uni(v2[3]);
        amax = (rpm > tau_) ? tau_/rpm : 1.0;
        adu = (rdm > tau_) ? tau_/rdm : 1.0;
    }

    __device__ __forceinline__ void merit_fast(double alpha, double mu_, Err &T, double &phi, bool &ok, const int soc_store = 0)
    {
        double xt[SPT][NV], st[SPT][NR];
#pragma unroll
        for (int j = 0; j < SPT; j++) {
            node_fence<4>();
            Dir dd; load_dir(j, dd);
#pragma unroll
            for (int k = 0; k < NV; k++) xt[j][k] = step_to(n[j].x[k], alpha, dd.dx[k]);
#pragma unroll
            for (int r = 0; r < NR; r++) st[j][r] = step_to(n[j].sg[r], alpha, n[j].dsg[r]);
        }
        publish_fast(xt);
        double th = 0, damp = 0, bad = 0, obj = 0;
        LogSum lsum;
#pragma unroll
        for (int j = 0; j < SPT; j++) {
            node_fence<5>();
            load_static<7>(j);
            const NodeT &nd = n[j];
            const int i = nd.i;
            double prod = 1.0;
            if (nd.ival()) {
                const double t = xt[j][VT], b = xt[j][VB], f = xt[j][VF], p = withPn() ? xt[j][VP] : 0.0, s = xt[j][VS];
                const double t1 = c.xt[i + 1], b1 = c.xb[i + 1], sb = c.xs[i], sb1 = c.xs[i + 1];
                double tau, bp;
                interval_map<double, true>(P, b, f + p, nd.G, nd.ds, tau, bp);
                th += nd.sct*fabs(t1 - (t + tau)) + nd.scb*fabs(b1 - bp);
                double dv[NR];
                dv[RPW0] = U.rs[RPW0]*f*sb; dv[RPW1] = U.rs[RPW1]*f*sb1;
                dv[RACC] = U.rs[RACC]*(f + p - (P.sr0 + P.sr1*sb + P.sr2*b) - nd.G);
                dv[RLTR] = U.rs[RLTR]*(s - P.ct*f); dv[RLRG] = U.rs[RLRG]*(s + P.cr*f);
                if constexpr (SOCK) {
                    if (soc_store != 0) {
                        const bool first = soc_store == 1;
                        const double *sB = c.S + i*S_STRIDE;
                        const double o0 = first ? -sB[S_RT] : wf(W_RESC, i), o1 = first ? -sB[S_RB] : wf(W_RESC + 1, i);
                        wf(W_RESC, i) = alpha*o0 + (t1 - (t + tau)); wf(W_RESC + 1, i) = alpha*o1 + (b1 - bp);
                        const double oldr[NR] = {first ? c.o1[i] : wf(W_RESD + RPW0, i), first ? c.o2[i] : wf(W_RESD + RPW1, i), first ? c.o3[i] : wf(W_RESD + RACC, i),
                                                 first ? c.o4[i] : wf(W_RESD + RLTR, i), first ? c.o6[i] : wf(W_RESD + RLRG, i)};
#pragma unroll
                        for (int r = 0; r < NR; r++) wf(W_RESD + r, i) = alpha*oldr[r] + (dv[r] - st[j][r]);
                    }
                }
#pragma unroll
                for (int r = 0; r < NR; r++) {
                    th += fabs(dv[r] - st[j][r]);
                    { const double sl = st[j][r] - U.dL[r]; if (sl <= 0) bad = 1; else prod *= sl; }
                    if (r <= RACC) { const double su = U.dU[r] - st[j][r]; if (su <= 0) bad = 1; else prod *= su; }
                    else damp += st[j][r] - U.dL[r];
                }
            }
            if (nd.node()) {
#pragma unroll
                for (int k = 0; k < NV; k++) {
                    if ((k == VP && !withPn()) || !nd.on(k)) continue;
                    { const double sl = xt[j][k] - lbv(k); if (sl <= 0) bad = 1; else prod *= sl; }
                    if (hasU(k)) { const double su = ubv(j, k) - xt[j][k]; if (su <= 0) bad = 1; else prod *= su; }
                    else damp += xt[j][k] - lbv(k);
                }
                obj += objective_term<false, FULL>(P, nd, xt[j], (i > 0) ? c.xf[i - 1] : 0.0, U.sf);
            }
            lsum.add(prod);
        }
        double v[4] = {th, lsum.value(), damp, obj};
        const bool anybad = block_sum_any<4>(v, bad != 0, c);
        T.theta = uni(v[0]); T.L = uni(v[1]); T.D = uni(v[2]); T.obj = uni(v[3]);
        phi = T.obj - mu_*T.L + K_D*mu_*T.D;
        ok = !anybad && isfinite(T.theta) && isfinite(phi);
    }

    __device__ __forceinline__ void update_fast(double apr, double adu, double mu_, const double dw = 0.0)
    {
        const double hi = K_SIGMA*mu_, lo = mu_*(1.0/K_SIGMA);
        bool clamp = false;
#pragma unroll
        for (int j = 0; j < SPT; j++) {
            node_fence<10>();
            load_static<4>(j);
            NodeT &nd = n[j];
            if (!nd.node()) continue;
            Dir dd; load_dir(j, dd);
#pragma unroll
            for (int k = 0; k < NV; k++) {
                if ((k == VP && !withPn()) || !nd.on(k)) continue;
                const double dk = dd.dx[k], xo = nd.x[k], xn = step_to(xo, apr, dk);
                {
                    const double s = xo - lbv(k), z = nd.zL[k], r = frcp(s);
                    const double zn = z + adu*(r*(mu_ - z*dk) - z), cn = zn*(xn - lbv(k));
                    clamp |= !(cn <= hi && cn >= lo);
                    nd.zL[k] = zn;
                }
                if (hasU(k)) {
                    const double s = ubv(j, k) - xo, z = nd.zU[k], r = frcp(s);
                    const double zn = z + adu*(r*(mu_ + z*dk) - z), cn = zn*(ubv(j, k) - xn);
                    clamp |= !(cn <= hi && cn >= lo);
                    nd.zU[k] = zn;
                }
                nd.x[k] = xn;
            }
            if (nd.ival()) {
#pragma unroll
                for (int r_ = 0; r_ < NR; r_++) {
                    const double dk = nd.dsg[r_], so = nd.sg[r_], sn_ = step_to(so, apr, dk);
                    double Sg, gphi;
                    {
                        const double s = so - U.dL[r_], z = nd.zLs[r_], r = frcp(s);
                        Sg = z*r; gphi = -mu_*r;
                        const double zn = z + adu*(r*(mu_ - z*dk) - z), cn = zn*(sn_ - U.dL[r_]);
                        clamp |= !(cn <= hi && cn >= lo);
                        nd.zLs[r_] = zn;
                    }
                    if (r_ <= RACC) {
                        const double s = U.dU[r_] - so, z = nd.zUs[r_], r = frcp(s);
                        Sg += z*r; gphi += mu_*r;
                        const double zn = z + adu*(r*(mu_ + z*dk) - z), cn = zn*(U.dU[r_] - sn_);
                        clamp |= !(cn <= hi && cn >= lo);
                        nd.zUs[r_] = zn;
                    } else gphi += K_D*mu_;
                    nd.nu[r_] += apr*((Sg + dw)*dk + gphi - nd.nu[r_]);
                    nd.sg[r_] = sn_;
                }
                nd.lam[0] += apr*(dd.lt - nd.lam[0]); nd.lam[1] += apr*(dd.lb - nd.lam[1]);
            }
        }
        if (block_any(clamp, c)) {
#pragma unroll
            for (int j = 0; j < SPT; j++) {
                NodeT &nd = n[j];
                if (!nd.node()) continue;
#pragma unroll
                for (int k = 0; k < NV; k++) {
                    if ((k == VP && !withPn()) || !nd.on(k)) continue;
                    nd.zL[k] = sigma_clamp(nd.zL[k], mu_, nd.x[k] - lbv(k));
                    if (hasU(k)) nd.zU[k] = sigma_clamp(nd.zU[k], mu_, ubv(j, k) - nd.x[k]);
                }
                if (!nd.ival()) continue;
#pragma unroll
                for (int r_ = 0; r_ < NR; r_++) {
                    nd.zLs[r_] = sigma_clamp(nd.zLs[r_], mu_, nd.sg[r_] - U.dL[r_]);
                    if (r_ <= RACC) nd.zUs[r_] = sigma_clamp(nd.zUs[r_], mu_, U.dU[r_] - nd.sg[r_]);
                }
            }
        }
    }

    static constexpr int STATUS_GENERAL = -100;
    int why_general = 0;
#include "msd_resto.hpp"

#ifndef MSD_RESTO
#define MSD_RESTO 1
#endif
    static constexpr bool FIRST = PART == 1 || PART == 3;
    static constexpr bool FAMILY_HAS_RESTO = MSD_RESTO && (STREAM || FIRST || PART == 2 || (DYN == LOSS_STATIC && !GEN && NT <= 256));
    static constexpr bool HAS_RESTO = FAMILY_HAS_RESTO && !FIRST;
    static_assert(!(loss_integrated(DYN) && HAS_RESTO && !STREAM), "integrated loss rows: the restoration phase lives in the streamed follow-up kernels");
    static constexpr int STATUS_RESTO = -101;

#ifndef MSD_WATCHDOG
#define MSD_WATCHDOG 1
#endif
    static constexpr int WD_TRIGGER_DEFAULT = 10, WD_TRIAL_MAX = 3;
    static constexpr bool WD_FULL = MSD_WATCHDOG && (PART == 2 || (STREAM && PART == 0));
    static constexpr bool WD_HANDOVER = MSD_WATCHDOG && !WD_FULL && (PART == 1 || PART == 3);
    static constexpr bool RESUMABLE = (FAMILY_HAS_RESTO && !(PART == 1 || PART == 3)) || WD_FULL;
    __device__ static __noinline__ void wd_restore(double *work, const int tid, const int nt)
    {
        for (int j = 0; j < SPT; j++) {
            const int i = tid + j*nt;
            for (int f = 0; f < W_WD_FIELDS; f++) work[(size_t)f*NS + i] = work[(size_t)(W_WD + f)*NS + i];
        }
    }
    __device__ static __noinline__ void wd_store(double *work, const int tid, const int nt)
    {
        for (int j = 0; j < SPT; j++) {
            const int i = tid + j*nt;
            for (int f = 0; f < W_WD_FIELDS; f++) work[(size_t)(W_WD + f)*NS + i] = work[(size_t)f*NS + i];
        }
    }
    static constexpr int STATUS_WDSTART = -103;
    static constexpr int STATUS_WDSTOP = -102;

    template <bool FL>
    __device__ __forceinline__ int run(const double *scen, const double *guess, const double *dual_in, int startKind, int iter_offset, int &iters_out,
                                       double *z_out, double *lam_out, double *dual_out, double *stats, double *hist, int hist_cap, const bool resume = false)
    {
        const int N = P.N;
        const bool ext = guess != nullptr;
        const bool warm = ext || startKind == MSD_START_PROFILE;
        const double kp = ext ? P.warmPush : K_PUSH;
        const double mu_start = ext ? P.warmMu : K_MU_INIT;
        const unsigned long long cyc0 = __builtin_readcyclecounter();
        if (c.tid == 0) { c.misc[1] = 0.0; c.misc[MISC_FALLBACKS] = 0.0; for (int k = 0; k < PH_SLOTS; k++) c.misc[2 + k] = 0.0; }
        c.tmark = cyc0;
        const double t0 = scen[MSD_SC_T0], tEnd = scen[MSD_SC_TEND], v0sq = scen[MSD_SC_V0SQ], vNsq = scen[MSD_SC_VNSQ];

#pragma unroll
        for (int j = 0; j < SPT; j++) {
            node_fence<8>();
            NodeT &nd = n[j];
            nd.i = c.tid + j*c.nt;
            nd.bind(work + nd.i);
            resc[j].bind(work + W_RESC*NS + nd.i); resd[j].bind(work + W_RESD*NS + nd.i);
            evs[j].bind(work + W_EV*NS + nd.i); lgs[j].bind(work + W_LG*NS + nd.i);
            if constexpr (!STREAM) {
#pragma unroll
                for (int k = 0; k < 13; k++) evs[j][k] = 0.0;
            }
            const bool ival = nd.i < N, node = nd.i <= N;
            nd.ds = ival ? P.ds[nd.i] : 0.0;
            nd.G = ival ? track_resistance(P, P.grad[nd.i], P.curv[nd.i]) : 0.0;
            const double bm = (nd.i >= 1 && nd.i < N) ? P.bmax[nd.i] : INFINITY;
            unsigned fl = (ival ? F_IVAL : 0u) | (node ? F_NODE : 0u);
            if (nd.i >= 1 && node && t0 != tEnd) fl |= F_ON_T;
            if (nd.i >= 1 && nd.i < N && P.vminSq != bm) fl |= F_ON_B;
            if (ival && P.fmin != P.fmax) fl |= F_ON_F;
            if (ival && withPn() && P.fminPn != 0.0) fl |= F_ON_P;
            if (ival) fl |= F_ON_S;
            nd.flags = fl;
            nd.ubB = bm + K_BOUND_RELAX*fmax(1.0, fabs(bm));
            if (STREAM && RESUMABLE && !FL && resume) continue;
            const double dt = (tEnd - t0)/N, vel0 = (60/3.6)*(60/3.6);
            nd.x[VT] = t0 + dt*nd.i; nd.x[VB] = vel0; nd.x[VF] = 0.5; nd.x[VP] = withPn() ? -0.1 : 0.0; nd.x[VS] = 1;
            if (ext && node) {
                const int nu = 1 + withPn();
                const double *q = guess + (nu + 3)*nd.i;
                if (ival) { nd.x[VF] = q[0]; nd.x[VP] = withPn() ? q[1] : 0.0; nd.x[VS] = q[nu]; nd.x[VT] = q[nu + 1]; nd.x[VB] = q[nu + 2]; }
                else { nd.x[VT] = q[0]; nd.x[VB] = q[1]; }
            }
            if (nd.i == 0) { nd.x[VT] = t0; nd.x[VB] = v0sq; }
            if (nd.i == N) nd.x[VB] = vNsq;
#pragma unroll
            for (int k = 0; k < NV; k++) nd.zL[k] = nd.zU[k] = 0;
#pragma unroll
            for (int r = 0; r < NR; r++) { nd.sg[r] = nd.nu[r] = nd.zLs[r] = nd.zUs[r] = 0; nd.dsg[r] = 0; }
            nd.lam[0] = nd.lam[1] = 0;
            nd.sct = nd.scb = 1;
        }
        double mu = mu_start, tau = fmax(K_TAU_MIN, 1 - mu);
        if (!(RESUMABLE && !FL && resume)) {
        if (!ext && startKind == MSD_START_PROFILE) profile_start(t0, tEnd, v0sq, vNsq);
        Uni u;
        u.tlo = t0 - K_BOUND_RELAX*fmax(1.0, fabs(t0)); u.thi = tEnd + K_BOUND_RELAX*fmax(1.0, fabs(tEnd));
        u.blo = P.vminSq - K_BOUND_RELAX*fmax(1.0, fabs(P.vminSq));
        u.flo = P.fmin - K_BOUND_RELAX*fmax(1.0, fabs(P.fmin)); u.fhi = P.fmax + K_BOUND_RELAX*fmax(1.0, fabs(P.fmax));
        u.plo = P.fminPn - K_BOUND_RELAX*fmax(1.0, fabs(P.fminPn)); u.phi = K_BOUND_RELAX;
        u.slo = -K_BOUND_RELAX;
#pragma unroll
        for (int r = 0; r < NR; r++) { u.rowOn[r] = false; u.dL[r] = -INFINITY; u.dU[r] = INFINITY; u.rs[r] = 1.0; u.irs[r] = 1.0; u.rL[r] = u.rU[r] = false; }
        if (hasPower()) { u.rowOn[RPW0] = u.rowOn[RPW1] = true; u.dL[RPW0] = u.dL[RPW1] = -fabs(P.pwL); u.dU[RPW0] = u.dU[RPW1] = fabs(P.pwU); }
        u.rowOn[RACC] = true; u.dL[RACC] = P.accMin; u.dU[RACC] = P.accMax;
        if (energyOpt()) { u.rowOn[RLTR] = u.rowOn[RLRG] = true; u.dL[RLTR] = u.dL[RLRG] = 0; }
        u.sf = 1;

        commit_uniforms(u);

        evaluate_current();
        Ev e[SPT];
#pragma unroll
        for (int j = 0; j < SPT; j++) load_ev1(j, e[j]);
        {
            double gmax = 0, rmax[NR] = {0, 0, 0, 0, 0};
#pragma unroll
            for (int j = 0; j < SPT; j++) {
                node_fence<8>();
                NodeT &nd = n[j];
                if (nd.ival()) {
                    double of, op, os, oq, off, opp;
                    obj_grads(j, nb_q(j), of, op, os, oq, off, opp);
                    gmax = fmax(gmax, fmax(fabs(of), fmax(fabs(op), fabs(os))));
                    double mb = (nd.i == N - 1) ? 0.0 : 1.0;
                    if (nd.i > 0) mb = fmax(mb, fabs(e[j].Bb));
                    mb = fmax(mb, fabs(e[j].Bw));
                    nd.scb = mb > 100 ? 100/mb : 1;
                    double mt = 1.0;
                    if (nd.i > 0) mt = fmax(mt, fabs(e[j].tb));
                    mt = fmax(mt, fabs(e[j].tw));
                    nd.sct = mt > 100 ? 100/mt : 1;
                    double gb[NR], gf[NR], gp[NR], gs[NR], gb1[NR], gd[NR];
                    row_grads(j, e[j], gb, gf, gp, gs, gb1, gd);
#pragma unroll
                    for (int r = 0; r < NR; r++) {
                        double m = fmax(fmax(fabs(gf[r]), fabs(gd[r])), fmax(fabs(gp[r]), fabs(gs[r])));
                        if (nd.i > 0) m = fmax(m, fabs(gb[r]));
                        if (nd.i < N - 1) m = fmax(m, fabs(gb1[r]));
                        rmax[r] = fmax(rmax[r], m);
                    }
                } else if (nd.i == N && !energyOpt()) gmax = fmax(gmax, 1.0/P.objDen);
            }
            double v[6] = {gmax, rmax[0], rmax[1], rmax[2], rmax[3], rmax[4]};
            block_reduce<6>(v, OpMax(), c);
            if (uni(v[0]) > 100) u.sf = uni(100/v[0]);
#pragma unroll
            for (int r = 0; r < NR; r++) if (u.rowOn[r] && uni(v[1 + r]) > 100) u.rs[r] = uni(100/v[1 + r]);
        }
#pragma unroll
        for (int r = 0; r < NR; r++) {
            if (!u.rowOn[r]) continue;
            u.dL[r] *= u.rs[r]; u.dU[r] *= u.rs[r]; u.irs[r] = 1.0/u.rs[r];
            u.rL[r] = isfinite(u.dL[r]); u.rU[r] = isfinite(u.dU[r]);
            if (u.rL[r]) u.dL[r] -= K_BOUND_RELAX*fmax(1.0, fabs(u.dL[r]));
            if (u.rU[r]) u.dU[r] += K_BOUND_RELAX*fmax(1.0, fabs(u.dU[r]));
        }
        commit_uniforms(u);

        const bool dualStart = ext && dual_in != nullptr;
#pragma unroll
        for (int j = 0; j < SPT; j++) {
            node_fence<8>();
            const double *q = dualStart ? dual_in + (size_t)MSD_DUAL_STRIDE*n[j].i : nullptr;
#pragma unroll
            for (int k = 0; k < NV; k++) {
                if (!n[j].on(k)) continue;
                n[j].x[k] = push_in(n[j].x[k], lbv(k), ubv(j, k), true, hasU(k), kp);
                n[j].zL[k] = warm ? mu_start/(n[j].x[k] - lbv(k)) : 1.0;
                n[j].zU[k] = hasU(k) ? (warm ? mu_start/(ubv(j, k) - n[j].x[k]) : 1.0) : 0.0;
                if (dualStart) { n[j].zL[k] = fmax(q[7 + k], 1e-3*n[j].zL[k]); if (hasU(k)) n[j].zU[k] = fmax(q[12 + k], 1e-3*n[j].zU[k]); }
            }
        }
        evaluate_current();
#pragma unroll
        for (int j = 0; j < SPT; j++) {
            node_fence<8>();
            if (!n[j].ival()) continue;
#pragma unroll
            for (int r = 0; r < NR; r++) {
                if (!rowOn(r)) continue;
                n[j].sg[r] = push_in(resd[j][r], U.dL[r], U.dU[r], rL(r), rU(r), kp);
                n[j].zLs[r] = rL(r) ? (warm ? mu_start/(n[j].sg[r] - U.dL[r]) : 1.0) : 0.0;
                n[j].zUs[r] = rU(r) ? (warm ? mu_start/(U.dU[r] - n[j].sg[r]) : 1.0) : 0.0;
                resd[j][r] -= n[j].sg[r];
            }
            if (dualStart) {
                const double *q = dual_in + (size_t)MSD_DUAL_STRIDE*n[j].i;
                n[j].lam[0] = q[0]; n[j].lam[1] = q[1];
#pragma unroll
                for (int r = 0; r < NR; r++) {
                    if (!rowOn(r)) continue;
                    n[j].nu[r] = q[2 + r];
                    if (rL(r)) n[j].zLs[r] = fmax(q[17 + r], 1e-3*n[j].zLs[r]);
                    if (rU(r)) n[j].zUs[r] = fmax(q[22 + r], 1e-3*n[j].zUs[r]);
                }
            }
        }


        if constexpr (!FL || PART == 3)
        if (!dualStart)
#if MSD_PROFILE_SKIP_LSQ
        if (ext || startKind != MSD_START_PROFILE)
#endif
        {
            const bool ok = direction(MODE_LSQ, 0.0, 0.0);
            double lmax = 0;
            Dir dd[SPT];
#pragma unroll
            for (int j = 0; j < SPT; j++) {
                load_dir(j, dd[j]);
                if (ok && n[j].ival()) {
                    lmax = fmax(lmax, fmax(fabs(dd[j].lt)/n[j].sct, fabs(dd[j].lb)/n[j].scb));
#pragma unroll
                    for (int r = 0; r < NR; r++) if (rowOn(r)) lmax = fmax(lmax, fabs(n[j].dsg[r]));
                }
            }
            double v[1] = {lmax};
            block_reduce<1>(v, OpMax(), c);
            const double lm = uni(v[0]);
            const bool use = ok && lm <= LAM_INIT_MAX && isfinite(lm);
#pragma unroll
            for (int j = 0; j < SPT; j++) {
                NodeT &nd = n[j];
                const bool tk = use && nd.ival();
                nd.lam[0] = tk ? dd[j].lt : 0.0; nd.lam[1] = tk ? dd[j].lb : 0.0;
#pragma unroll
                for (int r = 0; r < NR; r++) { nd.nu[r] = (tk && rowOn(r)) ? nd.dsg[r] : 0.0; nd.dsg[r] = 0; }
            }
        }
        }

        int nfilt = 0;
        double delta_last = 0, theta_max = 0, theta_min = 0;
        int status = MSD_STATUS_MAXITER, iter = 0, acc_count = 0, tiny_count = 0;
        double ic_dw = 0;
        bool ic_retry = false;
        int soc_mode = 0;
        constexpr int MISC_SOC = 27;
        int n_reg = 0, n_soc = 0, n_back = 0, n_resto = 0, iter_first = 0, forced = 0;
        int wd_short = 0, wd_trial = 0, n_wd = 0, wd_reg_inc = 0;
        bool in_wd = false, wd_arm = false;
        double wd_theta = 0, wd_phi = 0, wd_gphid = 0, wd_delta_last = 0;
        Err E;
        double alpha_pr = 0, alpha_du = 0, dnorm = 0, objv = 0;
        const double mu_floor = fmin(P.tol, 1e-4)/(K_EPS + 1.0);
        bool skip_first = false;
        if constexpr (RESUMABLE && !FL) {
            if (resume) {
// ... 446 lines not shown
                    for (int r = 0; r < NR; r++) {
                        if (!rowOn(r)) continue;
                        const double dzl = rL(r) ? dzL_row(j, r, mu) : 0.0, dzu = rU(r) ? dzU_row(j, r, mu) : 0.0;
                        double Sg, gphi; row_terms(j, r, mu, Sg, gphi);
                        const double dnu = (Sg + dw)*nd.dsg[r] + gphi - nd.nu[r];
                        nd.sg[r] += alpha_pr*nd.dsg[r];
                        nd.nu[r] += alpha_pr*dnu;
                        if (rL(r)) { nd.zLs[r] += alpha_du*dzl; const double s = nd.sg[r] - U.dL[r]; nd.zLs[r] = sigma_clamp(nd.zLs[r], mu, s); }
                        if (rU(r)) { nd.zUs[r] += alpha_du*dzu; const double s = U.dU[r] - nd.sg[r]; nd.zUs[r] = sigma_clamp(nd.zUs[r], mu, s); }
                    }
                    nd.lam[0] += alpha_pr*(dd.lt - nd.lam[0]); nd.lam[1] += alpha_pr*(dd.lb - nd.lam[1]);
                }
            }
            c.mark(PH_UPDATE); phase_fence(PH_UPDATE);
            }
        }
        if ((FL || WD_HANDOVER) && status == STATUS_GENERAL) { iters_out = iter; return status; }
        if (status == STATUS_RESTO || status == STATUS_WDSTOP || status == STATUS_WDSTART) { iters_out = iter; return status; }

        if (dual_out) {
#pragma unroll
            for (int j = 0; j < SPT; j++) {
                node_fence<11>();
                const NodeT &nd = n[j];
                if (!nd.node()) continue;
                double *q = dual_out + (size_t)MSD_DUAL_STRIDE*nd.i;
                q[0] = nd.ival() ? nd.lam[0] : 0.0; q[1] = nd.ival() ? nd.lam[1] : 0.0;
#pragma unroll
                for (int r = 0; r < NR; r++) { q[2 + r] = nd.ival() ? nd.nu[r] : 0.0; q[17 + r] = nd.ival() ? nd.zLs[r] : 0.0; q[22 + r] = nd.ival() ? nd.zUs[r] : 0.0; }
#pragma unroll
                for (int k = 0; k < NV; k++) { q[7 + k] = nd.zL[k]; q[12 + k] = nd.zU[k]; }
            }
        }

        const int stp = 4 + withPn();
#pragma unroll
        for (int j = 0; j < SPT; j++) {
            node_fence<11>();
            const NodeT &nd = n[j];
            if (nd.ival()) {
                double *zi = z_out + stp*nd.i; int k = 0;
                zi[k++] = nd.x[VF]; if (withPn()) zi[k++] = nd.x[VP];
                zi[k++] = nd.x[VS]; zi[k++] = nd.x[VT]; zi[k++] = nd.x[VB];
                if (lam_out) {
                    const int rpi = (hasPower() ? 2 : 0) + 3 + (energyOpt() ? 2 : 0);
                    double *l = lam_out + rpi*nd.i; int m = 0;
                    if (hasPower()) { l[m++] = nd.nu[RPW0]*U.rs[RPW0]/U.sf; l[m++] = nd.nu[RPW1]*U.rs[RPW1]/U.sf; }
                    l[m++] = nd.nu[RACC]*U.rs[RACC]/U.sf;
                    l[m++] = nd.lam[0]/U.sf; l[m++] = nd.lam[1]/U.sf;
                    if (energyOpt()) { l[m++] = nd.nu[RLTR]*U.rs[RLTR]/U.sf; l[m++] = nd.nu[RLRG]*U.rs[RLRG]/U.sf; }
                }
            } else if (nd.i == N) { z_out[stp*N] = nd.x[VT]; z_out[stp*N + 1] = nd.x[VB]; }
        }
        if (c.tid == 0) {
            stats[MSD_ST_STATUS] = status; stats[MSD_ST_ITERS] = iter + iter_offset; stats[MSD_ST_OBJ] = objv;
            stats[MSD_ST_KKT] = total_err(E, 0.0); stats[MSD_ST_MU] = mu; stats[MSD_ST_DUAL_INF] = E.dual/U.sf;
            stats[MSD_ST_CONSTR_VIOL] = E.primal_u; stats[MSD_ST_COMPL] = compl_err(E, 0.0)/U.sf;
            stats[MSD_ST_N_REG] = n_reg; stats[MSD_ST_N_SOC] = n_soc; stats[MSD_ST_N_BACKTRACK] = n_back; stats[MSD_ST_N_RESTO] = n_resto; stats[MSD_ST_N_WATCHDOG] = n_wd;
            stats[MSD_ST_CYC_TOTAL] = (double)(__builtin_readcyclecounter() - cyc0); stats[MSD_ST_CYC_KKT] = c.misc[1]; stats[MSD_ST_N_FALLBACK] = c.misc[MISC_FALLBACKS];
            if (hist && hist_cap >= 4) for (int k = 0; k < PH_SLOTS; k++) hist[HIST_COLS*(hist_cap - 2) + k] = c.misc[2 + k];
        }
        __syncthreads();
        iters_out = iter;
        return status;
    }
};

template <int NT, int SPT, int DYN, bool GEN, int FULL>
__device__ __noinline__ int resto_entry(const DevProb *P, Ctx c, double *work, Uni *U, const double *scen, double *hist, int hist_cap)
{
    Solver<NT, SPT, DYN, true, GEN, FULL> r(*P, c, work, *U);
    int nit = 0;
    const int rr = r.restoration(scen, hist, hist_cap, nit);
    __syncthreads();
    if (c.tid == 0) {
        double *sc = work + (size_t)W_SCAL*NT*SPT;
        sc[Solver<NT, SPT, DYN, true, GEN, FULL>::SC_ITER] += nit;
        sc[Solver<NT, SPT, DYN, true, GEN, FULL>::SC_FORCED] = rr == 1 ? 0 : rr == -1 ? MSD_STATUS_INFEASIBLE : rr == -2 ? MSD_STATUS_MAXITER : MSD_STATUS_LINESEARCH;
    }
    __syncthreads();
    return rr;
}

template <int NT, int SPT, int WPS, int DYN, bool STREAM = false, bool GEN = false, int FULL = 0, int PART = 0, bool SLDS = false, bool SOCK = false>
__global__ void __launch_bounds__(NT, WPS) solve_kernel(DevProb P, int nscen, const double *scen, const double *overrides, double *z_out, double *lam_out,
                                                       double *stats, double *hist, int hist_cap, double *work)
{
    HIP_DYNAMIC_SHARED(double, lds)
    constexpr int NS = NT*SPT;
    if (P.list && P.list[0] == 0) return;
    Ctx c;
    c.tid = threadIdx.x; c.lane = threadIdx.x & 63; c.wave = threadIdx.x >> 6; c.nw = NT/64; c.nt = NT; c.red_slot = 0;
    double *wg_work = work + (STREAM ? stream_doubles(P.N, NS, DYN) : work_doubles(NS))*blockIdx.x;
    if (STREAM) {
        c.S = wg_work + (size_t)W_FIELDS*NS;
        c.xt = c.S + stage_stride(DYN)*(P.N + 1);
        c.filt = lds;
    } else {
        c.S = lds;
        c.xt = c.S + stage_stride(DYN)*(P.N + 1);
    }
    c.xb = c.xt + NS; c.xf = c.xb + NS;
    c.o1 = c.xf + NS; c.o2 = c.o1 + NS; c.o3 = c.o2 + NS;
    using SolverT = Solver<NT, SPT, DYN, STREAM, GEN, FULL, PART, SLDS, SOCK>;
    constexpr bool FASTK = SolverT::FAST;
    c.xs = c.o4 = c.o5 = c.o6 = c.o7 = nullptr;
    if (FASTK) { c.xs = c.o3 + NS; c.o4 = c.xs + NS; c.o5 = c.o4 + NS; c.o6 = c.o5 + NS; c.o7 = c.o6 + NS; }
    if (!STREAM) c.filt = c.o3 + NS + (FASTK ? (XCH_FAST - XCH_GENERAL)*NS : 0);
    c.red = c.filt + 2*FILT_CAP; c.misc = c.red + ((FASTK && NT == 64) ? 0 : RED_DOUBLES);
    double *loss_lds = c.misc + 32 + CONST_DOUBLES;
    c.st = loss_lds + (DYN != LOSS_STATIC ? LOSS_HEAD_CAP : 0);
    c.pool = c.st;
    const double *loss_head = P.loss, *loss_coef = nullptr;
    if ((DYN == LOSS_TABLE || DYN == LOSS_INTEGRATED_TABLE) && P.loss) {
        const int len = 13 + ((int)P.loss[11] + 1) + ((int)P.loss[12] + 1);
        loss_coef = P.loss + len;
        if (len <= LOSS_HEAD_CAP) {
            for (int k = threadIdx.x; k < len; k += NT) loss_lds[k] = P.loss[k];
            loss_head = loss_lds;
        }
    }
    DevProb *Pl = reinterpret_cast<DevProb *>(c.misc + 32);
    Uni *Ul = reinterpret_cast<Uni *>(c.misc + 32 + UNI_OFF);
    static_assert(sizeof(DevProb) <= 8*UNI_OFF && sizeof(Uni) <= 8*(CONST_DOUBLES - UNI_OFF), "LDS room for the uniform records");
    const int nz = (4 + P.withPn)*P.N + 2;
    const int rpi = (P.hasPower ? 2 : 0) + 3 + (P.energyOpt ? 2 : 0);
    constexpr int MISC_NEXT = 25, MISC_SPENT = 26;
    const bool listed = P.list != nullptr;
    for (int turn = 0;; turn++) {
        int sidx, spent0 = -1;
        if (listed) {
            __syncthreads();
            if (c.tid == 0) {
                const int k = atomicAdd(P.list + 1, 1);
                const bool have = k < P.list[0];
                c.misc[MISC_NEXT] = have ? (double)P.list[FOLLOW_HDR + 2*k] : (double)nscen;
                c.misc[MISC_SPENT] = have ? (double)P.list[FOLLOW_HDR + 2*k + 1] : -1.0;
            }
            __syncthreads();
            sidx = wg_uniform((int)c.misc[MISC_NEXT]); spent0 = wg_uniform((int)c.misc[MISC_SPENT]);
        } else if (P.queue) {
            __syncthreads();
            if (c.tid == 0) c.misc[MISC_NEXT] = (double)atomicAdd(P.queue, 1);
            __syncthreads();
            sidx = wg_uniform((int)c.misc[MISC_NEXT]);
        } else sidx = blockIdx.x + turn*gridDim.x;
        if (sidx >= nscen) break;
        DevProb Ps = P;
        Ps.loss = loss_head; Ps.lossCoef = loss_coef;
        if (overrides) {
            const double *o = overrides + (size_t)MSD_OV_COUNT*sidx;
            Ps.sr0 = o[MSD_OV_SR0]; Ps.sr1 = o[MSD_OV_SR1]; Ps.sr2 = o[MSD_OV_SR2];
            Ps.fmax = o[MSD_OV_F_MAX]; Ps.fmin = o[MSD_OV_F_MIN]; Ps.fminPn = o[MSD_OV_F_MIN_PN];
            Ps.pwU = o[MSD_OV_PW_UPPER]; Ps.pwL = o[MSD_OV_PW_LOWER]; Ps.objDen = o[MSD_OV_OBJ_DEN]; Ps.lossMass = o[MSD_OV_TOTAL_MASS];
        }
        const bool budgeted = SolverT::FIRST && P.follow && P.budget > 0 && P.budget < P.maxIter;
        if (budgeted) Ps.maxIter = P.budget;
        bool handed = false;
        __syncthreads();
        if (c.tid == 0) *Pl = Ps;
        __syncthreads();
        SolverT s(*Pl, c, wg_work, *Ul);
        const double *guess = P.guess ? P.guess + (size_t)P.guessStride*sidx : nullptr;
        if (guess && P.guessStatus && P.guessStatus[(size_t)MSD_ST_COUNT*sidx + MSD_ST_STATUS] < 0) guess = nullptr;
        const double *dual_in = (guess && P.dualIn) ? P.dualIn + (size_t)P.dualInStride*sidx + (size_t)MSD_DUAL_STRIDE*P.dualShift : nullptr;
        double *dual_out = P.dualOut ? P.dualOut + (size_t)MSD_DUAL_STRIDE*(P.N + 1)*sidx : nullptr;
        int startKind = P.start, spent = 0, attempt0 = 0;
        if ((PART == 2 || PART == 0) && spent0 >= 0) {
            attempt0 = 1; spent = spent0;
            if (guess) guess = nullptr; else startKind = (startKind == MSD_START_PROFILE) ? MSD_START_REFERENCE : MSD_START_PROFILE;
        }
#ifndef MSD_MAX_ATTEMPTS
#define MSD_MAX_ATTEMPTS 2
#endif
#pragma unroll 1
        for (int attempt = attempt0; attempt < MSD_MAX_ATTEMPTS; attempt++) {
            int iters = 0;
            int st = SolverT::STATUS_GENERAL;
            if constexpr (FASTK && PART != 2) {
                if (PART == 3 || (guess && dual_in) || (!guess && startKind == MSD_START_PROFILE))
                    st = status_uniform(s.template run<true>(scen + (size_t)MSD_SC_COUNT*sidx, guess, guess ? dual_in : nullptr, startKind, spent, iters, z_out + (size_t)nz*sidx,
                                              lam_out ? lam_out + (size_t)rpi*P.N*sidx : nullptr, dual_out, stats + (size_t)MSD_ST_COUNT*sidx,
                                              (hist && sidx == 0) ? hist : nullptr, hist_cap));
                __syncthreads();
            }
            if constexpr (SolverT::FIRST && !FASTK) {
                bool resume = false;
#pragma unroll 1
                for (;;) {
                    st = status_uniform(s.template run<false>(scen + (size_t)MSD_SC_COUNT*sidx, guess, guess ? dual_in : nullptr, startKind, spent, iters, z_out + (size_t)nz*sidx,
                                               lam_out ? lam_out + (size_t)rpi*P.N*sidx : nullptr, dual_out, stats + (size_t)MSD_ST_COUNT*sidx,
                                               (hist && sidx == 0) ? hist : nullptr, hist_cap, resume));
                    __syncthreads();
                    if constexpr (SolverT::WD_FULL) {
                        if (st == SolverT::STATUS_WDSTART) SolverT::wd_store(wg_work, c.tid, c.nt);
                        else if (st == SolverT::STATUS_WDSTOP) SolverT::wd_restore(wg_work, c.tid, c.nt);
                        else break;
                        __syncthreads();
                        resume = true;
                    } else break;
                }
            }
            if constexpr (SolverT::FIRST) {
                const bool over_budget = budgeted && st == MSD_STATUS_MAXITER;
                if (st >= 0 || st == MSD_STATUS_INFEASIBLE || (st == MSD_STATUS_MAXITER && !over_budget)) break;
                const bool again = st == SolverT::STATUS_GENERAL || (SolverT::FAMILY_HAS_RESTO && st == MSD_STATUS_LINESEARCH && P.resto) || over_budget;
                if (again) {
                    if (c.tid == 0) {
                        const int k = atomicAdd(P.follow, 1);
                        P.follow[FOLLOW_HDR + 2*k] = sidx; P.follow[FOLLOW_HDR + 2*k + 1] = (attempt == 0 || over_budget) ? -1 : spent;
                        atomicAdd(P.follow + FOLLOW_TOTAL, 1);
                        atomicAdd(P.follow + FOLLOW_WHY + (over_budget ? 7 : st == SolverT::STATUS_GENERAL ? s.why_general : 4), 1);
                        if (P.socSeen && st == SolverT::STATUS_GENERAL && s.why_general == 3) *P.socSeen = 1;
                    }
                    handed = true;
                    break;
                }
                if (P.oneAttempt) break;
                if (attempt == 0 && c.tid == 0) atomicAdd(P.follow + FOLLOW_WHY + 5, 1);
                spent = iters;
                if (guess) guess = nullptr;
                else startKind = (startKind == MSD_START_PROFILE) ? MSD_START_REFERENCE : MSD_START_PROFILE;
            } else {
            if (st == SolverT::STATUS_GENERAL) {
                bool resume = false;
#pragma unroll 1
                for (;;) {
                    st = status_uniform(s.template run<false>(scen + (size_t)MSD_SC_COUNT*sidx, guess, guess ? dual_in : nullptr, startKind, spent, iters, z_out + (size_t)nz*sidx,
                                               lam_out ? lam_out + (size_t)rpi*P.N*sidx : nullptr, dual_out, stats + (size_t)MSD_ST_COUNT*sidx,
                                               (hist && sidx == 0) ? hist : nullptr, hist_cap, resume));
                    __syncthreads();
                    if constexpr (SolverT::WD_FULL) {
                        if (st == SolverT::STATUS_WDSTOP) { SolverT::wd_restore(wg_work, c.tid, c.nt); __syncthreads(); resume = true; continue; }
                        if (st == SolverT::STATUS_WDSTART) { SolverT::wd_store(wg_work, c.tid, c.nt); __syncthreads(); resume = true; continue; }
                    }
                    if constexpr (SolverT::HAS_RESTO) {
                        if (st != SolverT::STATUS_RESTO) break;
                        resto_entry<NT, SPT, DYN, GEN, FULL>(Pl, c, wg_work, Ul, scen + (size_t)MSD_SC_COUNT*sidx, (hist && sidx == 0) ? hist : nullptr, hist_cap);
                        resume = true;
                    } else break;
                }
            }
            __syncthreads();
            if (st >= 0 || st == MSD_STATUS_INFEASIBLE) break;
            if (st == MSD_STATUS_MAXITER && !(SolverT::HAS_RESTO && stats[(size_t)MSD_ST_COUNT*sidx + MSD_ST_N_RESTO] > 0)) break;
            if (P.oneAttempt) break;
            spent = iters;
            if (guess) guess = nullptr;
            else startKind = (startKind == MSD_START_PROFILE) ? MSD_START_REFERENCE : MSD_START_PROFILE;
            }
        }
        if (P.done) {
            const int word = handed ? 0 : (PART == 2 ? 2 : 1);
            if (word != 0 && P.statsHost && c.tid < MSD_ST_COUNT) P.statsHost[(size_t)MSD_ST_COUNT*sidx + c.tid] = stats[(size_t)MSD_ST_COUNT*sidx + c.tid];
            __syncthreads();
            if (word != 0 && c.tid == 0) publish_done(P.done + sidx, word);
        }
    }
    if (listed) {
        __syncthreads();
        if (c.tid == 0) {
            __threadfence();
            if (atomicAdd(P.list + 2, 1) == (int)gridDim.x - 1) { P.list[0] = 0; P.list[1] = 0; P.list[2] = 0; __threadfence(); }
        }
    }
}

template <int UNUSED>
__global__ void stage_eval_kernel(DevProb P, int n, const double *b, const double *w, const double *ds, const double *grad, const double *curv, double *out)
{
    int k = blockIdx.x*blockDim.x + threadIdx.x;
    if (k >= n) return;
    Jet tau, bp;
    if (P.integ) interval_map_general<Jet>(P, b[k], w[k], track_resistance(P, grad[k], curv[k]), ds[k], tau, bp);
    else interval_map<Jet>(P, b[k], w[k], track_resistance(P, grad[k], curv[k]), ds[k], tau, bp);
    double *o = out + 12*(size_t)k;
    o[0] = tau.v; o[1] = bp.v; o[2] = tau.g0; o[3] = tau.g1; o[4] = bp.g0; o[5] = bp.g1;
    o[6] = tau.h00; o[7] = tau.h01; o[8] = tau.h11; o[9] = bp.h00; o[10] = bp.h01; o[11] = bp.h11;
}

}
```

ms-eetc_amd/csrc/msd_select.hpp:

```cpp
#pragma once

#include <cmath>

#include "msd_geometry.hpp"

namespace msd_host {

using msd::Geometry;
using msd::KernelId;

enum Family { STATIC, DYNAMIC, INTLOSS, INTLOSS_TABLE, GENERAL, GENERAL_DYNAMIC, GENERAL_INTLOSS };
inline Family family_of(const msd_problem_desc *d)
{
    const bool dyn = d->loss_kind == 2, gen = d->integrator != 0, intloss = d->integrate_losses != 0 && d->energy_optimal != 0;
    if (dyn && intloss) return INTLOSS_TABLE;
    if (gen) return dyn ? GENERAL_DYNAMIC : intloss ? GENERAL_INTLOSS : GENERAL;
    return intloss ? INTLOSS : dyn ? DYNAMIC : STATIC;
}
inline int structure_of(const msd_problem_desc *d)
{
    if (d->has_power_rows == 0 || !std::isfinite(d->acc_min) || !std::isfinite(d->acc_max) || !std::isfinite(d->pw_upper) || !std::isfinite(d->pw_lower)) return 0;
    if (d->energy_optimal != 0) return d->with_pn_brake != 0 ? msd::FULL_BOTH : msd::FULL_RG;
    return d->with_pn_brake != 0 ? msd::FULL_TIME_BOTH : msd::FULL_TIME_RG;
}
inline int dyn_of(Family f) { return (f == DYNAMIC || f == GENERAL_DYNAMIC) ? msd::LOSS_TABLE : (f == INTLOSS || f == GENERAL_INTLOSS) ? msd::LOSS_INTEGRATED : f == INTLOSS_TABLE ? msd::LOSS_INTEGRATED_TABLE : msd::LOSS_STATIC; }
inline bool gen_of(Family f) { return f == GENERAL || f == GENERAL_DYNAMIC || f == GENERAL_INTLOSS; }

inline void fill_problem(msd::DevProb &P, const msd_problem_desc *d)
{
    P.N = d->num_intervals; P.withPn = d->with_pn_brake != 0; P.hasPower = d->has_power_rows != 0; P.energyOpt = d->energy_optimal != 0;
    P.numSteps = d->num_steps; P.numApprox = d->num_approx_steps; P.lossKind = d->loss_kind; P.maxIter = d->max_iterations;
    P.sr0 = d->sr0; P.sr1 = d->sr1; P.sr2 = d->sr2; P.g = d->g; P.rho = d->rho; P.fmax = d->f_max; P.fmin = d->f_min; P.fminPn = d->f_min_pn;
    P.pwU = d->pw_upper; P.pwL = d->pw_lower; P.accMin = d->acc_min; P.accMax = d->acc_max; P.ct = d->loss_ct; P.cr = d->loss_cr;
    P.vminSq = d->vmin_sq; P.objDen = d->obj_den; P.tol = d->tol;
    P.guess = nullptr; P.guessStride = 0; P.guessStatus = nullptr; P.warmMu = 0; P.warmPush = 0; P.start = d->start_kind; P.lossMass = 0; P.queue = nullptr; P.follow = nullptr; P.list = nullptr; P.socSeen = nullptr; P.done = nullptr; P.statsHost = nullptr; P.budget = 0; P.dualOut = nullptr; P.dualIn = nullptr; P.dualInStride = 0; P.dualShift = 0;
    P.ds = P.grad = P.curv = P.bmax = P.pos = nullptr;
    P.loss = nullptr; P.lossCoef = nullptr;
    P.integ = d->integrator; P.collD = d->coll_degree; P.newtonIters = d->newton_iterations; P.intAtol = d->int_abstol; P.intRtol = d->int_reltol;
    P.coll = nullptr;
    P.resto = d->no_restoration ? 0 : 1;
    P.oneAttempt = 0;
    P.wdTrigger = d->watchdog_trigger == 0 ? 10 : d->watchdog_trigger;
    if (d->integrator == MSD_INTEGRATOR_ADAPTIVE) P.numApprox = 0;
}

struct Tuning {
    bool no_full = false, two_nodes_per_lane = false;
    int NT = 0, SPT = 0;
};

bool has_kernel(const KernelId &id);

inline size_t lds_bytes(const Geometry &g, const KernelId &k, int N)
{
    return sizeof(double)*(size_t)(k.STREAM ? msd::lds_doubles_stream() : msd::lds_doubles(N, k.NT*k.SPT, k.DYN != msd::LOSS_STATIC, g.xch, g.red) + msd::coop_doubles(k.NT, k.GEN) + g.extra);
}

inline Geometry resident(Family family, int N, int structure, const Tuning &t)
{
    using namespace msd;
    const int nodes = N + 1, DYN = dyn_of(family);
    const bool GEN = gen_of(family), two = t.two_nodes_per_lane;
    Geometry g;
    int FULL = t.no_full ? 0 : structure;
    const auto rung = [&](int top, int NT, int SPT, int WPS = 1) {
        if (t.NT) { NT = t.NT; SPT = t.SPT; top = NT*SPT; }
        const KernelId id{NT, SPT, WPS, DYN, false, GEN, FULL, 1};
        if (nodes > top || !has_kernel(id)) return false;
        g.first = id;
        return true;
    };
    const auto fused = [&](int NT, int SPT, bool slds = false) {
        if (t.NT) { NT = t.NT; SPT = t.SPT; }
        const KernelId id{NT, SPT, 1, LOSS_STATIC, false, false, FULL, 1, slds};
        const int red = NT == 64 ? 0 : RED_DOUBLES;
        if (nodes > NT*SPT || sizeof(double)*(size_t)lds_doubles(N, NT*SPT, false, XCH_FAST, red) > 160*1024 || !has_kernel(id)) return false;
        Geometry s;
        s.first = s.lsq = s.follow = s.soc = id;
        s.lsq.PART = 3;
        s.follow.PART = 2; s.follow.SLDS = false;
        if (NT == 64 && SPT == 1 && !has_kernel(s.follow)) s.follow.SPT = 2;
        if (!has_kernel(s.follow)) return false;
        if (!has_kernel(s.lsq)) s.lsq = KernelId{};
        s.soc.SOCK = true;
        if (!has_kernel(s.soc)) s.soc = KernelId{};
        s.xch = XCH_FAST; s.red = red; s.extra = slds ? STATIC_FIELDS*NT*SPT : 0;
        g = s;
        return true;
    };

    if (family == STATIC && full_energy(FULL)) {
        if (fused(64, 1)) return g;
        if (MSD_STATIC_LDS && nodes > 64 && sizeof(double)*(size_t)(lds_doubles(N, 128, false, XCH_FAST, 0) + STATIC_FIELDS*128) <= 40*1024 && fused(64, 2, true)) return g;
        if (fused(64, 2)) return g;
        if (fused(128, 2) || fused(192, 2) || fused(256, 2)) return g;
    }
    if (family == STATIC && full_time(FULL) && (rung(64, 64, 1) || rung(128, 64, 2) || rung(256, 128, 2))) return g;
    if (family == DYNAMIC && full_energy(FULL) && (rung(64, 64, 1) || (nodes > 64 && !(nodes <= 128 && two) && (rung(128, 128, 1) || rung(256, 128, 2) || rung(384, 192, 2))))) return g;
    if ((family == INTLOSS || family == GENERAL) && FULL == FULL_BOTH && (rung(64, 64, 1) || (two && rung(128, 64, 2)) || rung(128, 128, 1))) return g;

    FULL = 0;
    if (family == INTLOSS_TABLE) { (void)(rung(64, 64, 1) || rung(128, 128, 1)); return g; }
    if (family == GENERAL_DYNAMIC) { (void)(rung(64, 64, 1) || rung(128, 128, 1) || rung(256, 128, 2)); return g; }
    if (family == GENERAL_INTLOSS) { (void)(rung(64, 64, 1) || rung(128, 128, 1) || rung(256, 256, 1)); return g; }
    if (rung(64, 64, 1)) return g;
// ... 27 lines not shown
```

ms-eetc_amd/mseetc/_device.py:

```python

import ctypes
import os
from pathlib import Path

import numpy as np

LIB_PATH = Path(os.environ.get('MSD_LIB', Path(__file__).resolve().parent.parent / 'lib' / 'libmseetc_hip.so'))

ABI_VERSION = 6
INTEGRATOR_ADAPTIVE, INTEGRATOR_COLLOCATION = 1, 2
ST = dict(STATUS=0, ITERS=1, OBJ=2, KKT=3, MU=4, DUAL_INF=5, CONSTR_VIOL=6, COMPL=7, N_REG=8, N_SOC=9, N_BACKTRACK=10, CYC_TOTAL=11, CYC_KKT=12, N_FALLBACK=13, N_RESTO=14, N_WATCHDOG=15, COUNT=16)
SC_COUNT = 4
OV = dict(SR0=0, SR1=1, SR2=2, F_MAX=3, F_MIN=4, F_MIN_PN=5, PW_UPPER=6, PW_LOWER=7, OBJ_DEN=8, TOTAL_MASS=9, COUNT=10)
HIST_COLS = 8

STATUS_MAXITER, STATUS_LINESEARCH, STATUS_INFEASIBLE = -1, -2, -6
WAIT_FIRST_PASS, WAIT_ALL = 1, 2
STATUS_TEXT = {0: 'Solve_Succeeded', 1: 'Solved_To_Acceptable_Level', -1: 'Maximum_Iterations_Exceeded',
               -2: 'Restoration_Failed', -3: 'Error_In_Step_Computation', -4: 'Invalid_Number_Detected',
               -5: 'Search_Direction_Becomes_Too_Small', -6: 'Infeasible_Problem_Detected'}

_dptr = ctypes.POINTER(ctypes.c_double)


class ProblemDesc(ctypes.Structure):

    _fields_ = [('abi_version', ctypes.c_int), ('num_intervals', ctypes.c_int), ('with_pn_brake', ctypes.c_int),
                ('has_power_rows', ctypes.c_int), ('energy_optimal', ctypes.c_int), ('num_steps', ctypes.c_int),
                ('num_approx_steps', ctypes.c_int), ('loss_kind', ctypes.c_int), ('max_iterations', ctypes.c_int),
                ('start_kind', ctypes.c_int), ('integrator', ctypes.c_int), ('coll_degree', ctypes.c_int), ('newton_iterations', ctypes.c_int),
                ('integrate_losses', ctypes.c_int), ('no_restoration', ctypes.c_int), ('watchdog_trigger', ctypes.c_int),
                ('sr0', ctypes.c_double), ('sr1', ctypes.c_double), ('sr2', ctypes.c_double), ('g', ctypes.c_double), ('rho', ctypes.c_double),
                ('f_max', ctypes.c_double), ('f_min', ctypes.c_double), ('f_min_pn', ctypes.c_double),
                ('pw_upper', ctypes.c_double), ('pw_lower', ctypes.c_double), ('acc_min', ctypes.c_double), ('acc_max', ctypes.c_double),
                ('loss_ct', ctypes.c_double), ('loss_cr', ctypes.c_double), ('vmin_sq', ctypes.c_double), ('obj_den', ctypes.c_double),
                ('tol', ctypes.c_double), ('int_abstol', ctypes.c_double), ('int_reltol', ctypes.c_double), ('reserved_d', ctypes.c_double*5),
                ('ds', _dptr), ('grad', _dptr), ('curv', _dptr), ('bmax', _dptr),
                ('loss_table', _dptr), ('loss_table_len', ctypes.c_int), ('reserved_tail', ctypes.c_int), ('coll_tables', _dptr)]


class MpcPlan(ctypes.Structure):

    _fields_ = [('num_resolves', ctypes.c_int), ('stride', ctypes.c_int), ('problems', ctypes.POINTER(ProblemDesc)), ('twins', ctypes.POINTER(ProblemDesc)),
                ('vlim_first', _dptr), ('length', _dptr), ('tail', ctypes.POINTER(ctypes.c_ubyte)), ('vmin', ctypes.c_double), ('vmax_train', ctypes.c_double),
                ('terminal_velocity', ctypes.c_double), ('warm_start', ctypes.c_int), ('warm_mu', ctypes.c_double), ('warm_push', ctypes.c_double),
                ('noise', ctypes.c_double), ('relax_infeasible', ctypes.c_int), ('late_margin', ctypes.c_double)]


MPC = dict(T0=0, V0=1, T=2, STATUS=3, ITERS=4, OBJ=5, RELAXED=6, COUNT=7)


class DeviceError(RuntimeError):
    pass


_lib = None


def lib():

    global _lib

    if _lib is None:

        if not LIB_PATH.exists():
            raise DeviceError("HIP solver library {} not found: run `python -c 'import __graft_entry__ as g; g.build()'` "
                              "(hipcc, gfx950). There is no CPU fallback.".format(LIB_PATH))

        L = ctypes.CDLL(str(LIB_PATH))
        vp = ctypes.c_void_p

        L.msd_last_error.restype = ctypes.c_char_p
        L.msd_device_count.restype = ctypes.c_int
        L.msd_problem_create.argtypes = [ctypes.POINTER(ProblemDesc), ctypes.c_int, ctypes.POINTER(vp)]
        L.msd_problem_destroy.argtypes = [vp]
        L.msd_problem_reconfigure.argtypes = [vp, ctypes.POINTER(ProblemDesc)]
        L.msd_problem_nz.argtypes = [vp]
        L.msd_problem_rows_per_interval.argtypes = [vp]
        L.msd_solve_batch.argtypes = [vp, ctypes.c_int, _dptr, _dptr, _dptr, _dptr, ctypes.POINTER(ctypes.c_float)]
        L.msd_solve_batch_ex.argtypes = [vp, ctypes.c_int, _dptr, _dptr, _dptr, _dptr, _dptr, ctypes.POINTER(ctypes.c_float)]
        L.msd_solve_batch_warm.argtypes = [vp, ctypes.c_int, _dptr, _dptr, _dptr, ctypes.c_double, ctypes.c_double, _dptr, _dptr, _dptr,
                                           ctypes.POINTER(ctypes.c_float)]
        L.msd_interval_integrate.argtypes = [ctypes.c_int, ctypes.c_int, _dptr, ctypes.c_int, _dptr, ctypes.c_int] + [_dptr]*8 + [ctypes.POINTER(ctypes.c_int)]
        L.msd_interval_last_error.restype = ctypes.c_char_p
        L.msd_solve_batch_shifted.argtypes = [vp, ctypes.c_int, _dptr, _dptr, ctypes.c_int, ctypes.c_double, ctypes.c_double, _dptr, _dptr, _dptr,
                                              ctypes.POINTER(ctypes.c_float)]
        L.msd_problem_keep_duals.argtypes = [vp, ctypes.c_int]
        L.msd_problem_direct_results.argtypes = [vp, ctypes.c_int]
        L.msd_problem_early_results.argtypes = [vp, ctypes.c_int]
        L.msd_problem_iteration_budget.argtypes = [vp, ctypes.c_int]
        L.msd_solve_batch_begin.argtypes = [vp, ctypes.c_int, _dptr, _dptr, _dptr, _dptr, _dptr]
        L.msd_solve_batch_wait.argtypes = [vp, ctypes.c_int, ctypes.POINTER(ctypes.c_int)]
        L.msd_solve_batch_done.argtypes = [vp, ctypes.POINTER(ctypes.POINTER(ctypes.c_int)), ctypes.POINTER(_dptr)]
        L.msd_solve_batch_multi.argtypes = [ctypes.POINTER(vp), ctypes.c_int, ctypes.c_int, _dptr, _dptr, _dptr, ctypes.c_double, ctypes.c_double, _dptr, _dptr,
                                            _dptr, ctypes.POINTER(ctypes.c_float)]
        L.msd_solve_batch_device.argtypes = [vp, ctypes.c_int, vp, vp, vp, vp]
        L.msd_solve_batch_device_ex.argtypes = [vp, ctypes.c_int, vp, vp, vp, vp, vp]
        L.msd_problem_geometry.argtypes = [vp, ctypes.POINTER(ctypes.c_int), ctypes.POINTER(ctypes.c_int)]
        L.msd_synchronize.argtypes = [vp]
        L.msd_problem_follow_counts.argtypes = [vp, ctypes.POINTER(ctypes.c_int), ctypes.c_int]
        L.msd_problem_time_first_pass.argtypes = [vp, ctypes.c_int]
        L.msd_problem_first_pass_ms.argtypes = [vp, ctypes.POINTER(ctypes.c_float), ctypes.POINTER(ctypes.c_int)]
        L.msd_device_alloc.argtypes = [vp, ctypes.c_ulonglong, ctypes.POINTER(vp)]
        L.msd_device_free.argtypes = [vp, vp]
        L.msd_copy_to_device.argtypes = [vp, vp, vp, ctypes.c_ulonglong]
        L.msd_copy_to_host.argtypes = [vp, vp, vp, ctypes.c_ulonglong]
        L.msd_timer_begin.argtypes = [vp]
        L.msd_timer_end.argtypes = [vp, ctypes.POINTER(ctypes.c_float)]
        L.msd_stage_eval.argtypes = [vp, ctypes.c_int, _dptr, _dptr, _dptr, _dptr, _dptr, _dptr]
        L.msd_set_history.argtypes = [vp, _dptr, ctypes.c_int]
        L.msd_post_last_error.restype = ctypes.c_char_p
        L.msd_resimulate.argtypes = [ctypes.c_int, ctypes.c_int, ctypes.c_int, _dptr, _dptr, _dptr, _dptr, _dptr, _dptr, _dptr,
                                     ctypes.c_double, ctypes.c_double, _dptr, _dptr]
        L.msd_integrate_losses.argtypes = [ctypes.c_int, ctypes.c_int, ctypes.c_int, _dptr, ctypes.c_int, ctypes.c_double, ctypes.c_double, _dptr, ctypes.c_int,
                                           _dptr, _dptr, _dptr, _dptr, _dptr, _dptr, ctypes.c_double, ctypes.c_double, _dptr, _dptr]

        L.msd_tuning.argtypes = [ctypes.c_char_p, ctypes.c_int]
        L.msd_plan_describe.argtypes = [ctypes.POINTER(ProblemDesc), ctypes.c_char_p, ctypes.c_int]
        L.msd_fastmath_probe.argtypes = [ctypes.c_int, ctypes.c_int] + [_dptr]*4
        L.msd_host_alloc.argtypes = [ctypes.c_ulonglong, ctypes.POINTER(vp)]
        L.msd_host_free.argtypes = [vp]
        L.msd_mpc_create.argtypes = [vp, vp, ctypes.POINTER(MpcPlan), ctypes.POINTER(vp)]
        L.msd_mpc_destroy.argtypes = [vp]
        L.msd_mpc_run.argtypes = [vp, ctypes.c_int, _dptr, ctypes.c_double, ctypes.c_double, _dptr, _dptr, _dptr, _dptr, ctypes.POINTER(ctypes.c_float)]
        L.msd_mpc_nz.argtypes = [vp, ctypes.c_int]

        _lib = L

    return _lib


def _check(rc):

    if rc != 0:
        msg = lib().msd_last_error().decode()
        if rc == -1:
            raise ValueError(msg)
        raise DeviceError("msd error {}: {}".format(rc, msg))


def _d(a):
    return a.ctypes.data_as(_dptr)


START = dict(reference=0, profile=1)


def make_desc(N, withPn, hasPower, energyOptimal, numSteps, numApproxSteps, lossKind, maxIterations, sr, g, rho, fmax, fmin, fminPn,
              pwUpper, pwLower, accMin, accMax, ct, cr, vminSq, objDen, tol, ds, grad, curv, bmax, lossTable=None, start='reference',
              integrator=None, integrateLosses=False, restoration=True, watchdogTrigger=0):

    d = ProblemDesc()
    d.abi_version = ABI_VERSION
    d.num_intervals, d.with_pn_brake, d.has_power_rows, d.energy_optimal = int(N), int(withPn), int(hasPower), int(energyOptimal)
    d.num_steps, d.num_approx_steps, d.loss_kind, d.max_iterations = int(numSteps), int(numApproxSteps), int(lossKind), int(maxIterations)
    d.start_kind = START[start]
    d.no_restoration = 0 if restoration else 1
    d.watchdog_trigger = int(watchdogTrigger)
    d.sr0, d.sr1, d.sr2 = sr
    d.g, d.rho = g, rho
    d.f_max, d.f_min, d.f_min_pn = fmax, fmin, fminPn
    d.pw_upper, d.pw_lower, d.acc_min, d.acc_max = pwUpper, pwLower, accMin, accMax
    d.loss_ct, d.loss_cr, d.vmin_sq, d.obj_den, d.tol = ct, cr, vminSq, objDen, tol
    keep = [np.ascontiguousarray(a, dtype=np.float64) for a in (ds, grad, curv, bmax)]
    d.ds, d.grad, d.curv, d.bmax = [_d(a) for a in keep]
    if lossTable is not None:
        keep.append(np.ascontiguousarray(lossTable, dtype=np.float64))
        d.loss_table, d.loss_table_len = _d(keep[-1]), len(keep[-1])
    if integrator is not None and integrator[0] == 'CVODES':
        d.integrator, d.int_abstol, d.int_reltol = INTEGRATOR_ADAPTIVE, float(integrator[1]), float(integrator[2])
    elif integrator is not None and integrator[0] == 'IRK':
        d.integrator, d.coll_degree, d.newton_iterations = INTEGRATOR_COLLOCATION, int(integrator[1]), int(integrator[2])
        keep.append(np.concatenate([np.asarray(integrator[3], dtype=np.float64).ravel(), np.asarray(integrator[4], dtype=np.float64).ravel()]))
        d.coll_tables = _d(keep[-1])
    elif integrator is not None:
        raise ValueError("Unknown integration method!")
    d.integrate_losses = int(bool(integrateLosses))
    d._keep = keep

    return d


class _Pinned():
# ... 182 lines not shown
        st = self._results.empty('st', (B, ST['COUNT']))
        lam = self._results.empty('lam', (B, self.rowsPerInterval*self.N)) if want_multipliers else None

        if overrides is not None:
            overrides = np.ascontiguousarray(overrides, dtype=np.float64).reshape(B, OV['COUNT'])

        _check(L.msd_solve_batch_begin(self._h, B, _d(scen), _d(overrides) if overrides is not None else None, _d(z),
                                       _d(lam) if lam is not None else None, _d(st)))

        return PendingBatch(self, B, z, lam, st)

    def solve_batch_multi(self, others, scen, want_multipliers=False, overrides=None, guess=None, warmMu=1e-2, warmPush=1e-3):

        L = lib()
        scen = np.ascontiguousarray(scen, dtype=np.float64).reshape(-1, SC_COUNT)
        B = scen.shape[0]
        z = np.zeros((B, self.nz))
        st = np.zeros((B, ST['COUNT']))
        lam = np.zeros((B, self.rowsPerInterval*self.N)) if want_multipliers else None
        ms = ctypes.c_float(0)

        if overrides is not None:
            overrides = np.ascontiguousarray(overrides, dtype=np.float64).reshape(B, OV['COUNT'])

        if guess is not None:
            guess = np.ascontiguousarray(guess, dtype=np.float64).reshape(B, self.nz)

        handles = (ctypes.c_void_p*(1 + len(others)))(self._h, *[o._h for o in others])
        _check(L.msd_solve_batch_multi(handles, len(handles), B, _d(scen), _d(overrides) if overrides is not None else None,
                                       _d(guess) if guess is not None else None, float(warmMu), float(warmPush), _d(z),
                                       _d(lam) if lam is not None else None, _d(st), ctypes.byref(ms)))

        return dict(z=z, stats=st, lam_g=lam, kernel_ms=float(ms.value))


    def alloc(self, nbytes):
        p = ctypes.c_void_p()
        _check(lib().msd_device_alloc(self._h, int(nbytes), ctypes.byref(p)))
        return p

    def free(self, p):
        _check(lib().msd_device_free(self._h, p))

    def to_device(self, dptr, arr):
        arr = np.ascontiguousarray(arr)
        _check(lib().msd_copy_to_device(self._h, dptr, arr.ctypes.data_as(ctypes.c_void_p), arr.nbytes))

    def to_host(self, arr, dptr):
        _check(lib().msd_copy_to_host(self._h, arr.ctypes.data_as(ctypes.c_void_p), dptr, arr.nbytes))

    def solve_batch_device(self, B, d_scen, d_z, d_lam, d_stats, d_overrides=None):
        _check(lib().msd_solve_batch_device_ex(self._h, int(B), d_scen, d_overrides, d_z, d_lam, d_stats))

    def direct_results(self, on=True):

        _check(lib().msd_problem_direct_results(self._h, int(bool(on))))
        return self

    def keep_duals(self, on=True):
        _check(lib().msd_problem_keep_duals(self._h, int(bool(on))))
        return self

    def geometry(self):
        nt, spt = ctypes.c_int(0), ctypes.c_int(0)
        _check(lib().msd_problem_geometry(self._h, ctypes.byref(nt), ctypes.byref(spt)))
        return nt.value, spt.value

    def synchronize(self):
        _check(lib().msd_synchronize(self._h))

    def time_first_pass(self, on=True):
        _check(lib().msd_problem_time_first_pass(self._h, int(bool(on))))

    def first_pass_ms(self):
        ms, n = ctypes.c_float(0), ctypes.c_int(0)
        _check(lib().msd_problem_first_pass_ms(self._h, ctypes.byref(ms), ctypes.byref(n)))
        return float(ms.value), int(n.value)

    def follow_counts(self):
        out = (ctypes.c_int*9)()
        _check(lib().msd_problem_follow_counts(self._h, out, 9))
        return int(out[0]), [int(v) for v in out[1:]]

    def timer_begin(self):
        _check(lib().msd_timer_begin(self._h))

    def timer_end(self):
        ms = ctypes.c_float(0)
        _check(lib().msd_timer_end(self._h, ctypes.byref(ms)))
        return float(ms.value)

    def stage_eval(self, b, w, ds, grad, curv):
        arrs = [np.ascontiguousarray(np.atleast_1d(a), dtype=np.float64) for a in (b, w, ds, grad, curv)]
        n = len(arrs[0])
        out = np.zeros((n, 12))
        _check(lib().msd_stage_eval(self._h, n, *[_d(a) for a in arrs], _d(out)))
        return out


def stage_eval(model, optsRK, time, velocitySquared, ds, force, gradient, curvature):

    n = len(np.atleast_1d(velocitySquared))
    one = np.ones(1)
    desc = make_desc(1, model.withPnBrake, False, True, optsRK.numSteps, optsRK.numApproxSteps, 0, 1, (model.sr0, model.sr1, model.sr2),
                     model.g, model.rho, 1.0, -1.0, -1.0, 0.0, 0.0, -1.0, 1.0, 0.0, 0.0, 1.0, 1.0, 1e-8, one, 0*one, 0*one, np.ones(2))
    prob = DeviceProblem(desc)

    try:
        out = prob.stage_eval(velocitySquared, force, ds, gradient, curvature)
    finally:
        prob.close()

    return {'time': np.atleast_1d(np.asarray(time, dtype=float)) + out[:, 0], 'velSquared': out[:, 1], 'sens': out}


def interval_integrate(model, method, params, time, velocitySquared, ds, force, gradient, curvature, device=0):

    arrs = [np.ascontiguousarray(np.atleast_1d(a), dtype=np.float64) for a in (time, velocitySquared, ds, force, gradient, curvature)]
    n = max(len(a) for a in arrs)
    arrs = [np.ascontiguousarray(np.broadcast_to(a, (n,))) for a in arrs]
    params = _c(params)
    train5 = _c([model.sr0, model.sr1, model.sr2, model.g, model.rho])
    t, b, st = np.zeros(n), np.zeros(n), np.zeros(n, dtype=np.int32)
    L = lib()
    rc = L.msd_interval_integrate(int(device), n, _d(train5), int(method), _d(params), len(params), *[_d(a) for a in arrs], _d(t), _d(b),
                                  st.ctypes.data_as(ctypes.POINTER(ctypes.c_int)))
    if rc != 0:
        msg = L.msd_interval_last_error().decode()
        if rc == -1:
            raise ValueError(msg)
        raise DeviceError("msd integrator error {}: {}".format(rc, msg))

    return {'time': t, 'velSquared': b, 'status': st}


def fastmath_probe(x, device=0):
    L = lib()
    x = np.ascontiguousarray(x, dtype=np.float64)
    out = [np.empty_like(x) for _ in range(3)]
    if L.msd_fastmath_probe(int(device), x.size, _d(x), *[_d(a) for a in out]) != 0:
        raise DeviceError(L.msd_interval_last_error().decode())
    return out


def _check_post(rc):

    if rc != 0:
        msg = lib().msd_post_last_error().decode()
        if rc == -1:
            raise ValueError(msg)
        raise DeviceError("msd post-processing error {}: {}".format(rc, msg))


def _c(a, shape=None):
    a = np.ascontiguousarray(a, dtype=np.float64)
    return a if shape is None else a.reshape(shape)


def resimulate(model, force, dts, grad, curv, s0, v0, abstol=1e-12, reltol=1e-14, device=0):

    force, dts = _c(force), _c(dts)
    B, N = force.shape
    pos, vel = np.zeros((B, N + 1)), np.zeros((B, N + 1))
    train5 = _c([model.sr0, model.sr1, model.sr2, model.g, model.rho])
    _check_post(lib().msd_resimulate(int(device), B, N, _d(train5), _d(force), _d(dts), _d(_c(grad)), _d(_c(curv)), _d(_c(s0)), _d(_c(v0)),
                                     float(abstol), float(reltol), _d(pos), _d(vel)))
# ... 72 lines not shown
```

Before: 1.098 million.

## Split early-results first-pass kernels and use structural lane masks in fast solver

Adds separate EARLY kernel instantiations that hold the budgeted early-exit and host-result handoff code, so the default fast first-pass kernel is compiled without that logic and the extra branches and registers it needs. The fast solver also works out variable activity masks from the node structure instead of reading per-node flag words, which cuts flag loads in the barrier and step loops. It also tightens structure selection for degenerate force bounds. The cost is more kernel instantiations and launch-selection logic, and if no early twin is available when early results are requested, the launch now fails with an error.

```diff
diff --git a/__graft_entry__.py b/__graft_entry__.py
--- a/__graft_entry__.py
+++ b/__graft_entry__.py
@@ -64,7 +64,7 @@
     return n
 
 
-UNITS = ['msd_api.hip', 'msd_kernels_full.hip', 'msd_kernels_full2.hip', 'msd_kernels_full3.hip', 'msd_kernels_full4.hip', 'msd_kernels_rg.hip', 'msd_kernels_rg2.hip', 'msd_kernels_static.hip', 'msd_kernels_time.hip', 'msd_kernels_time2.hip', 'msd_kernels_dynamic.hip', 'msd_kernels_dynamic2.hip', 'msd_kernels_dynamic3.hip', 'msd_kernels_stream.hip', 'msd_kernels_stream2.hip', 'msd_kernels_stream3.hip', 'msd_kernels_stream4.hip', 'msd_kernels_stream5.hip', 'msd_kernels_stream6.hip', 'msd_kernels_stream7.hip', 'msd_kernels_compose.hip', 'msd_kernels_general.hip', 'msd_kernels_general2.hip', 'msd_kernels_intloss.hip', 'msd_kernels_intloss_table.hip', 'msd_kernels_intloss_table2.hip', 'msd_post.hip',
+UNITS = ['msd_api.hip', 'msd_kernels_full.hip', 'msd_kernels_full2.hip', 'msd_kernels_full3.hip', 'msd_kernels_full4.hip', 'msd_kernels_full5.hip', 'msd_kernels_full6.hip', 'msd_kernels_rg.hip', 'msd_kernels_rg2.hip', 'msd_kernels_rg3.hip', 'msd_kernels_static.hip', 'msd_kernels_time.hip', 'msd_kernels_time2.hip', 'msd_kernels_dynamic.hip', 'msd_kernels_dynamic2.hip', 'msd_kernels_dynamic3.hip', 'msd_kernels_stream.hip', 'msd_kernels_stream2.hip', 'msd_kernels_stream3.hip', 'msd_kernels_stream4.hip', 'msd_kernels_stream5.hip', 'msd_kernels_stream6.hip', 'msd_kernels_stream7.hip', 'msd_kernels_compose.hip', 'msd_kernels_general.hip', 'msd_kernels_general2.hip', 'msd_kernels_intloss.hip', 'msd_kernels_intloss_table.hip', 'msd_kernels_intloss_table2.hip', 'msd_post.hip',
          'msd_integrators.hip', 'msd_mpc.hip']
 SLOWEST_FIRST = ['msd_kernels_stream7.hip', 'msd_kernels_stream2.hip', 'msd_kernels_stream6.hip', 'msd_kernels_stream5.hip', 'msd_kernels_dynamic.hip', 'msd_kernels_stream3.hip',
                  'msd_kernels_stream4.hip', 'msd_kernels_intloss.hip', 'msd_kernels_compose.hip', 'msd_kernels_static.hip', 'msd_kernels_stream.hip']
diff --git a/include/mseetc_aux.h b/include/mseetc_aux.h
--- a/include/mseetc_aux.h
+++ b/include/mseetc_aux.h
@@ -19,6 +19,8 @@
 
 int msd_plan_describe(const msd_problem_desc *desc, char *buf, int len);
 
+int msd_problem_last_first_pass(msd_handle h, char *buf, int len);
+
 int msd_fastmath_probe(int device, int n, const double *x, double *rcp_out, double *sqrt_out, double *rsqrt_out);
 
 #ifdef __cplusplus
diff --git a/ms-eetc_amd/csrc/msd_api.hip b/ms-eetc_amd/csrc/msd_api.hip
--- a/ms-eetc_amd/csrc/msd_api.hip
+++ b/ms-eetc_amd/csrc/msd_api.hip
@@ -18,7 +18,7 @@
 thread_local std::string g_err;
 }
 
-#define MSD_KERNEL_UNITS(X) X(full) X(full2) X(full3) X(full4) X(rg) X(rg2) X(static) X(time) X(time2) X(dynamic) X(dynamic2) X(dynamic3) X(stream) X(stream2) X(stream3) \
+#define MSD_KERNEL_UNITS(X) X(full) X(full2) X(full3) X(full4) X(full5) X(full6) X(rg) X(rg2) X(rg3) X(static) X(time) X(time2) X(dynamic) X(dynamic2) X(dynamic3) X(stream) X(stream2) X(stream3) \
     X(stream4) X(stream5) X(stream6) X(stream7) X(compose) X(general) X(general2) X(intloss) X(intloss_table) X(intloss_table2)
 namespace msd {
 #define X(unit) KernelFn kernels_##unit(const KernelId &id);
@@ -142,6 +142,7 @@
     pl.kernel = find_kernel(geo.first); pl.kernel2 = find_kernel(geo.follow); pl.kernel_lsq = find_kernel(geo.lsq);
     pl.kernel_soc = nullptr;
     *soc_out = find_kernel(geo.soc);
+    pl.kernel_early = find_kernel(geo.early(geo.first)); pl.kernel_lsq_early = find_kernel(geo.early(geo.lsq)); pl.kernel_soc_early = find_kernel(geo.early(geo.soc));
     return MSD_OK;
 }
 
@@ -173,6 +174,12 @@
         int per_cu_soc = 0;
         if (kernel_limits(device, (const void *)soc, pl.NT, pl.lds_bytes, &per_cu_soc) == MSD_OK && per_cu_soc*cus >= pl.max_grid) pl.kernel_soc = soc;
     }
+    const auto twin = [&](msd::KernelFn &early, msd::KernelFn plain, int grid) {
+        int per_cu_early = 0;
+        if (!plain) early = nullptr;
+        else if (early && early != plain && !(kernel_limits(device, (const void *)early, pl.NT, pl.lds_bytes, &per_cu_early) == MSD_OK && per_cu_early*cus >= grid)) early = nullptr;
+    };
+    twin(pl.kernel_early, pl.kernel, pl.max_grid); twin(pl.kernel_lsq_early, pl.kernel_lsq, pl.max_grid_lsq); twin(pl.kernel_soc_early, pl.kernel_soc, pl.max_grid);
     return MSD_OK;
 }
 
@@ -209,7 +216,8 @@
 }
 
 int launch_plan(const Plan &pl, hipStream_t stream, double *d_work, int *d_follow, int *d_queue, int nscen, const double *d_scen, const double *d_ovr,
-                double *d_z, double *d_lam, double *d_stats, double *d_hist, int hist_cap, const WarmStart &ws, int *d_list, hipEvent_t first_begin, hipEvent_t first_end)
+                double *d_z, double *d_lam, double *d_stats, double *d_hist, int hist_cap, const WarmStart &ws, int *d_list, hipEvent_t first_begin, hipEvent_t first_end,
+                msd::KernelFn *first_out)
 {
     if (!pl.kernel) return fail(MSD_E_INVALID, "the handle holds no problem: its last (re)configuration failed");
     msd::DevProb P = pl.P;
@@ -225,12 +233,18 @@
         const msd::KernelFn fn = split ? pl.kernel2 : pl.kernel;
         const int cap = split ? pl.max_grid2 : pl.max_grid;
         P.list = d_list;
+        if (first_out) *first_out = fn;
         hipLaunchKernelGGL(fn, dim3(std::min(nscen, cap)), dim3(split ? pl.NT2 : pl.NT), split ? pl.lds_bytes2 : pl.lds_bytes, stream, P, nscen, d_scen, d_ovr, d_z, d_lam, d_stats, d_hist, hist_cap, d_work);
         HIP_TRY(hipGetLastError());
         return MSD_OK;
     }
     P.list = d_list;
-    const msd::KernelFn fn = (split && !first_pass) ? pl.kernel2 : plain ? ((ws.use_soc && pl.kernel_soc) ? pl.kernel_soc : pl.kernel) : pl.kernel_lsq;
+    const bool early = ws.d_done != nullptr || ws.budget > 0;
+    const msd::KernelFn fn = (split && !first_pass) ? pl.kernel2
+                           : plain ? ((ws.use_soc && pl.kernel_soc && (!early || pl.kernel_soc_early)) ? (early ? pl.kernel_soc_early : pl.kernel_soc) : (early ? pl.kernel_early : pl.kernel))
+                                   : (early ? pl.kernel_lsq_early : pl.kernel_lsq);
+    if (!fn) return fail(MSD_E_UNSUPPORTED, "this build holds no first-pass kernel with the early results inside for the handle's problem");
+    if (first_out) *first_out = fn;
     const int cap = (split && !first_pass) ? pl.max_grid2 : plain ? pl.max_grid : pl.max_grid_lsq;
     const int grid = nscen < cap ? nscen : cap;
     const int threads = (split && !first_pass) ? pl.NT2 : pl.NT;
@@ -275,6 +289,7 @@
     if (!name) return fail(MSD_E_INVALID, "null argument");
     if (!strcmp(name, "no_full")) msd_host::tuning().no_full = value != 0;
     else if (!strcmp(name, "two_nodes_per_lane")) msd_host::tuning().two_nodes_per_lane = value != 0;
+    else if (!strcmp(name, "geometry")) { msd_host::tuning().NT = value > 0 ? value/16 : 0; msd_host::tuning().SPT = value > 0 ? value%16 : 0; }
     else return fail(MSD_E_INVALID, std::string("unknown tuning switch: ") + name);
     return MSD_OK;
 }
@@ -465,7 +480,16 @@
                 nscen, (void *)h->d_work, sizeof(double)*h->cap_work, (void *)h->d_follow, (void *)queue, (void *)h->d_prof, (const void *)d_scen, (void *)d_z, (void *)d_lam, (void *)d_stats, (void *)d_hist,
                 msd_host::plan_text(h->plan, h->plan.kernel_soc).c_str(), h->plan.max_grid, h->plan.max_grid_lsq, h->plan.max_grid2);
 #endif
-    return msd_host::launch_plan(h->plan, h->stream, h->d_work, h->d_follow, queue, nscen, d_scen, d_ovr, d_z, d_lam, d_stats, d_hist, hist_cap, ws, nullptr, e0, e1);
+    return msd_host::launch_plan(h->plan, h->stream, h->d_work, h->d_follow, queue, nscen, d_scen, d_ovr, d_z, d_lam, d_stats, d_hist, hist_cap, ws, nullptr, e0, e1, &h->last_first);
+}
+
+int msd_problem_last_first_pass(msd_handle h, char *buf, int len)
+{
+    if (!h || !buf || len < 1) return fail(MSD_E_INVALID, "null argument");
+    const std::string name = msd_host::kernel_name(h->last_first);
+    if ((int)name.size() >= len) return fail(MSD_E_INVALID, "msd_problem_last_first_pass: the name needs " + std::to_string(name.size() + 1) + " bytes");
+    memcpy(buf, name.c_str(), name.size() + 1);
+    return MSD_OK;
 }
 
 int msd_solve_batch_device(msd_handle h, int nscen, const double *d_scen, double *d_z, double *d_lam, double *d_stats)
diff --git a/ms-eetc_amd/csrc/msd_geometry.hpp b/ms-eetc_amd/csrc/msd_geometry.hpp
--- a/ms-eetc_amd/csrc/msd_geometry.hpp
+++ b/ms-eetc_amd/csrc/msd_geometry.hpp
@@ -10,16 +10,17 @@
     int NT = 0, SPT = 0, WPS = 1, DYN = LOSS_STATIC;
     bool STREAM = false, GEN = false;
     int FULL = 0, PART = 0;
-    bool SLDS = false, SOCK = false;
+    bool SLDS = false, SOCK = false, EARLY = false;
     explicit operator bool() const { return NT != 0; }
 };
 inline bool operator==(const KernelId &a, const KernelId &b)
 {
     return a.NT == b.NT && a.SPT == b.SPT && a.WPS == b.WPS && a.DYN == b.DYN && a.STREAM == b.STREAM && a.GEN == b.GEN && a.FULL == b.FULL && a.PART == b.PART
-           && a.SLDS == b.SLDS && a.SOCK == b.SOCK;
+           && a.SLDS == b.SLDS && a.SOCK == b.SOCK && a.EARLY == b.EARLY;
 }
 
 #define MSD_KERNEL(...) if (id == KernelId{__VA_ARGS__}) return solve_kernel<__VA_ARGS__>;
+#define MSD_KERNEL_EARLY(...) if (KernelId twin_{__VA_ARGS__}; (twin_.EARLY = true, id == twin_)) return solve_kernel_early<__VA_ARGS__>;
 #define MSD_KERNEL_UNUSED(...) if (false) return solve_kernel<__VA_ARGS__>;
 
 struct Geometry {
@@ -27,6 +28,7 @@
     KernelId follow;
     KernelId lsq;
     KernelId soc;
+    KernelId early(const KernelId &k) const { KernelId e = k; if (k && xch == XCH_FAST && (k.PART == 1 || k.PART == 3)) e.EARLY = true; return e; }
     bool stream = false;
     int xch = XCH_GENERAL;
     int red = RED_DOUBLES;
diff --git a/ms-eetc_amd/csrc/msd_handle.hpp b/ms-eetc_amd/csrc/msd_handle.hpp
--- a/ms-eetc_amd/csrc/msd_handle.hpp
+++ b/ms-eetc_amd/csrc/msd_handle.hpp
@@ -29,6 +29,7 @@
     msd::KernelFn kernel_lsq = nullptr;
     msd::KernelFn kernel2 = nullptr;
     msd::KernelFn kernel_soc = nullptr;
+    msd::KernelFn kernel_early = nullptr, kernel_lsq_early = nullptr, kernel_soc_early = nullptr;
     int NT2 = 0, SPT2 = 0;
     size_t lds_bytes2 = 0;
     int max_grid = 0, max_grid_lsq = 0, max_grid2 = 0;
@@ -60,7 +61,8 @@
 
 int launch_plan(const Plan &pl, hipStream_t stream, double *d_work, int *d_follow, int *d_queue, int nscen, const double *d_scen, const double *d_ovr,
                 double *d_z, double *d_lam, double *d_stats, double *d_hist, int hist_cap, const WarmStart &ws, int *d_list = nullptr,
-                hipEvent_t first_begin = nullptr, hipEvent_t first_end = nullptr);
+                hipEvent_t first_begin = nullptr, hipEvent_t first_end = nullptr,
+                msd::KernelFn *first_out = nullptr);
 
 }
 
@@ -103,5 +105,6 @@
     int cap_done = 0;
     int begun = 0;
     hipEvent_t ev_first = nullptr;
+    msd::KernelFn last_first = nullptr;
     int attached_loops = 0;
 };
diff --git a/ms-eetc_amd/csrc/msd_kernel.hpp b/ms-eetc_amd/csrc/msd_kernel.hpp
--- a/ms-eetc_amd/csrc/msd_kernel.hpp
+++ b/ms-eetc_amd/csrc/msd_kernel.hpp
@@ -499,6 +499,9 @@
 __device__ __forceinline__ bool cmp_le(double lhs, double rhs, double basval) { return lhs - rhs <= 10.0*DBL_EPSILON*fabs(basval); }
 
 constexpr unsigned F_ON_T = 1u, F_ON_B = 2u, F_ON_F = 4u, F_ON_P = 8u, F_ON_S = 16u, F_IVAL = 32u, F_NODE = 64u;
+#ifndef MSD_FLAG_WORD_MASKS
+#define MSD_FLAG_WORD_MASKS 0
+#endif
 
 template <int CNT, int NS, bool MEM> struct Field;
 template <int CNT, int NS> struct Field<CNT, NS, false> {
@@ -1639,6 +1642,22 @@
     __device__ __forceinline__ double lbv(int k) const { return k == VT ? U.tlo : k == VB ? U.blo : k == VF ? U.flo : k == VP ? U.plo : U.slo; }
     __device__ __forceinline__ double ubv(int j, int k) const { return k == VT ? U.thi : k == VB ? n[j].ubB : k == VF ? U.fhi : k == VP ? U.phi : INFINITY; }
     __device__ static __forceinline__ bool hasU(int k) { return k != VS; }
+    static constexpr bool STRUCT_MASKS = full_energy(FULL) && DYN == LOSS_STATIC && !STREAM && !GEN && MSD_PARALLEL_RICCATI && !MSD_FLAG_WORD_MASKS;
+    __device__ __forceinline__ bool on(int j, int k) const
+    {
+        const NodeT &nd = n[j];
+        if constexpr (STRUCT_MASKS) return k == VT ? (nd.node() && nd.i > 0) : k == VB ? (nd.ival() && nd.i > 0) : k == VP ? (full_pn(FULL) && nd.ival()) : nd.ival();
+        else return nd.on(k);
+    }
+    __device__ __forceinline__ bool structural_start() const
+    {
+        bool same = true;
+#pragma unroll
+        for (int j = 0; j < SPT; j++)
+#pragma unroll
+            for (int k = 0; k < NV; k++) same = same && n[j].on(k) == on(j, k);
+        return same;
+    }
 
     __device__ __forceinline__ void phase_fence(int phase)
     {
@@ -1783,20 +1802,22 @@
     }
 
     struct Dir { double dx[NV], lt, lb; };
+    template <bool FUSED = false>
     __device__ __forceinline__ void load_dir(int j, Dir &d) const
     {
         const NodeT &nd = n[j];
+        const auto free = [&](int k) { return FUSED ? on(j, k) : nd.on(k); };
 #pragma unroll
         for (int k = 0; k < NV; k++) d.dx[k] = 0;
         d.lt = d.lb = 0;
         if (!nd.node()) return;
         const double *s = c.S + nd.i*S_STRIDE;
-        if (nd.on(VT)) d.dx[VT] = s[S_DT];
-        if (nd.on(VB)) d.dx[VB] = s[S_DB];
+        if (free(VT)) d.dx[VT] = s[S_DT];
+        if (free(VB)) d.dx[VB] = s[S_DB];
         if (nd.ival()) {
-            if (nd.on(VF)) d.dx[VF] = s[S_DF];
-            if (nd.on(VP)) d.dx[VP] = s[S_DP];
-            if (nd.on(VS)) d.dx[VS] = s[S_DS];
+            if (free(VF)) d.dx[VF] = s[S_DF];
+            if (free(VP)) d.dx[VP] = s[S_DP];
+            if (free(VS)) d.dx[VS] = s[S_DS];
             d.lt = s[S_LT]; d.lb = s[S_LB];
         }
     }
@@ -2537,6 +2558,7 @@
     }
 
     static constexpr bool FAST = full_energy(FULL) && DYN == LOSS_STATIC && !STREAM && !GEN && MSD_PARALLEL_RICCATI;
+    static_assert(STRUCT_MASKS == (FAST && !MSD_FLAG_WORD_MASKS), "structural lane masks: the kernels with the fused iteration");
     static constexpr int HV = 6;
     double cnt_lam = 0, cnt_z = 0;
 
@@ -2695,7 +2717,7 @@
 #pragma unroll
                 for (int k = 0; k < NV; k++) {
                     Sv[k] = 0; g1v[k] = 0;
-                    if ((k == VP && !withPn()) || !nd.on(k)) continue;
+                    if ((k == VP && !withPn()) || !on(j, k)) continue;
                     {
                         const double sl = nd.x[k] - lbv(k), z = nd.zL[k], ri = frcp(sl), cp = sl*z;
                         gl[j][k] -= z; cmax = fmax(cmax, cp); cmin = fmin(cmin, cp); sumz += z; nz += 1; prod *= sl;
@@ -2753,7 +2775,7 @@
             double *sB = c.S + i*S_STRIDE;
             sB[S_HBB] = Hbb; sB[S_HBQ] = Hbq;
 #pragma unroll
-            for (int k = 0; k < NV; k++) if (!(k == VP && !withPn()) && nd.on(k)) dual = fmax(dual, fabs(gl[j][k]));
+            for (int k = 0; k < NV; k++) if (!(k == VP && !withPn()) && on(j, k)) dual = fmax(dual, fabs(gl[j][k]));
         }
         __syncthreads();
 #pragma unroll
@@ -2808,7 +2830,7 @@
             for (int r = 0; r < NR; r++) nd.dsg[r] = 0;
             if (!nd.node()) continue;
             const int i = nd.i;
-            Dir d; load_dir(j, d);
+            Dir d; load_dir<true>(j, d);
             double og[NV] = {0, 0, 0, 0, 0};
             if (nd.ival()) {
                 const double f = nd.x[VF], sb = c.xs[i], sb1 = c.xs[i + 1];
@@ -2827,7 +2849,7 @@
             }
 #pragma unroll
             for (int k = 0; k < NV; k++) {
-                if ((k == VP && !withPn()) || !nd.on(k)) continue;
+                if ((k == VP && !withPn()) || !on(j, k)) continue;
                 const double dk = d.dx[k];
                 double gp;
                 {
@@ -2877,7 +2899,7 @@
 #pragma unroll
         for (int j = 0; j < SPT; j++) {
             node_fence<4>();
-            Dir dd; load_dir(j, dd);
+            Dir dd; load_dir<true>(j, dd);
 #pragma unroll
             for (int k = 0; k < NV; k++) xt[j][k] = step_to(n[j].x[k], alpha, dd.dx[k]);
 #pragma unroll
@@ -2926,7 +2948,7 @@
             if (nd.node()) {
 #pragma unroll
                 for (int k = 0; k < NV; k++) {
-                    if ((k == VP && !withPn()) || !nd.on(k)) continue;
+                    if ((k == VP && !withPn()) || !on(j, k)) continue;
                     { const double sl = xt[j][k] - lbv(k); if (sl <= 0) bad = 1; else prod *= sl; }
                     if (hasU(k)) { const double su = ubv(j, k) - xt[j][k]; if (su <= 0) bad = 1; else prod *= su; }
                     else damp += xt[j][k] - lbv(k);
@@ -2952,10 +2974,10 @@
             load_static<4>(j);
             NodeT &nd = n[j];
             if (!nd.node()) continue;
-            Dir dd; load_dir(j, dd);
+            Dir dd; load_dir<true>(j, dd);
 #pragma unroll
             for (int k = 0; k < NV; k++) {
-                if ((k == VP && !withPn()) || !nd.on(k)) continue;
+                if ((k == VP && !withPn()) || !on(j, k)) continue;
                 const double dk = dd.dx[k], xo = nd.x[k], xn = step_to(xo, apr, dk);
                 {
                     const double s = xo - lbv(k), z = nd.zL[k], r = frcp(s);
@@ -3003,7 +3025,7 @@
                 if (!nd.node()) continue;
 #pragma unroll
                 for (int k = 0; k < NV; k++) {
-                    if ((k == VP && !withPn()) || !nd.on(k)) continue;
+                    if ((k == VP && !withPn()) || !on(j, k)) continue;
                     nd.zL[k] = sigma_clamp(nd.zL[k], mu_, nd.x[k] - lbv(k));
                     if (hasU(k)) nd.zU[k] = sigma_clamp(nd.zU[k], mu_, ubv(j, k) - nd.x[k]);
                 }
@@ -3110,6 +3132,9 @@
             nd.lam[0] = nd.lam[1] = 0;
             nd.sct = nd.scb = 1;
         }
+        if constexpr (FL && STRUCT_MASKS) {
+            if (block_any(!structural_start(), c)) { why_general = 0; iters_out = 0; return STATUS_GENERAL; }
+        }
         double mu = mu_start, tau = fmax(K_TAU_MIN, 1 - mu);
         if (!(RESUMABLE && !FL && resume)) {
         if (!ext && startKind == MSD_START_PROFILE) profile_start(t0, tEnd, v0sq, vNsq);
@@ -3184,7 +3209,7 @@
             const double *q = dualStart ? dual_in + (size_t)MSD_DUAL_STRIDE*n[j].i : nullptr;
 #pragma unroll
             for (int k = 0; k < NV; k++) {
-                if (!n[j].on(k)) continue;
+                if (!(FL ? on(j, k) : n[j].on(k))) continue;
                 n[j].x[k] = push_in(n[j].x[k], lbv(k), ubv(j, k), true, hasU(k), kp);
                 n[j].zL[k] = warm ? mu_start/(n[j].x[k] - lbv(k)) : 1.0;
                 n[j].zU[k] = hasU(k) ? (warm ? mu_start/(ubv(j, k) - n[j].x[k]) : 1.0) : 0.0;
@@ -3797,9 +3822,9 @@
     return rr;
 }
 
-template <int NT, int SPT, int WPS, int DYN, bool STREAM = false, bool GEN = false, int FULL = 0, int PART = 0, bool SLDS = false, bool SOCK = false>
-__global__ void __launch_bounds__(NT, WPS) solve_kernel(DevProb P, int nscen, const double *scen, const double *overrides, double *z_out, double *lam_out,
-                                                       double *stats, double *hist, int hist_cap, double *work)
+template <int NT, int SPT, int WPS, int DYN, bool STREAM, bool GEN, int FULL, int PART, bool SLDS, bool SOCK, bool EARLY>
+__device__ __forceinline__ void solve_body(const DevProb &P, int nscen, const double *scen, const double *overrides, double *z_out, double *lam_out,
+                                           double *stats, double *hist, int hist_cap, double *work)
 {
     HIP_DYNAMIC_SHARED(double, lds)
     constexpr int NS = NT*SPT;
@@ -3819,6 +3844,10 @@
     c.o1 = c.xf + NS; c.o2 = c.o1 + NS; c.o3 = c.o2 + NS;
     using SolverT = Solver<NT, SPT, DYN, STREAM, GEN, FULL, PART, SLDS, SOCK>;
     constexpr bool FASTK = SolverT::FAST;
+#ifndef MSD_EARLY_IN_DEFAULT
+#define MSD_EARLY_IN_DEFAULT 0
+#endif
+    constexpr bool EARLY_RESULTS = EARLY || MSD_EARLY_IN_DEFAULT || !(FASTK && SolverT::FIRST);
     c.xs = c.o4 = c.o5 = c.o6 = c.o7 = nullptr;
     if (FASTK) { c.xs = c.o3 + NS; c.o4 = c.xs + NS; c.o5 = c.o4 + NS; c.o6 = c.o5 + NS; c.o7 = c.o6 + NS; }
     if (!STREAM) c.filt = c.o3 + NS + (FASTK ? (XCH_FAST - XCH_GENERAL)*NS : 0);
@@ -3869,7 +3898,7 @@
             Ps.fmax = o[MSD_OV_F_MAX]; Ps.fmin = o[MSD_OV_F_MIN]; Ps.fminPn = o[MSD_OV_F_MIN_PN];
             Ps.pwU = o[MSD_OV_PW_UPPER]; Ps.pwL = o[MSD_OV_PW_LOWER]; Ps.objDen = o[MSD_OV_OBJ_DEN]; Ps.lossMass = o[MSD_OV_TOTAL_MASS];
         }
-        const bool budgeted = SolverT::FIRST && P.follow && P.budget > 0 && P.budget < P.maxIter;
+        const bool budgeted = EARLY_RESULTS && SolverT::FIRST && P.follow && P.budget > 0 && P.budget < P.maxIter;
         if (budgeted) Ps.maxIter = P.budget;
         bool handed = false;
         __syncthreads();
@@ -3965,7 +3994,7 @@
             else startKind = (startKind == MSD_START_PROFILE) ? MSD_START_REFERENCE : MSD_START_PROFILE;
             }
         }
-        if (P.done) {
+        if (EARLY_RESULTS && P.done) {
             const int word = handed ? 0 : (PART == 2 ? 2 : 1);
             if (word != 0 && P.statsHost && c.tid < MSD_ST_COUNT) P.statsHost[(size_t)MSD_ST_COUNT*sidx + c.tid] = stats[(size_t)MSD_ST_COUNT*sidx + c.tid];
             __syncthreads();
@@ -3979,6 +4008,19 @@
             if (atomicAdd(P.list + 2, 1) == (int)gridDim.x - 1) { P.list[0] = 0; P.list[1] = 0; P.list[2] = 0; __threadfence(); }
         }
     }
+}
+
+template <int NT, int SPT, int WPS, int DYN, bool STREAM = false, bool GEN = false, int FULL = 0, int PART = 0, bool SLDS = false, bool SOCK = false>
+__global__ void __launch_bounds__(NT, WPS) solve_kernel(DevProb P, int nscen, const double *scen, const double *overrides, double *z_out, double *lam_out,
+                                                       double *stats, double *hist, int hist_cap, double *work)
+{
+    solve_body<NT, SPT, WPS, DYN, STREAM, GEN, FULL, PART, SLDS, SOCK, false>(P, nscen, scen, overrides, z_out, lam_out, stats, hist, hist_cap, work);
+}
+template <int NT, int SPT, int WPS, int DYN, bool STREAM = false, bool GEN = false, int FULL = 0, int PART = 0, bool SLDS = false, bool SOCK = false>
+__global__ void __launch_bounds__(NT, WPS) solve_kernel_early(DevProb P, int nscen, const double *scen, const double *overrides, double *z_out, double *lam_out,
+                                                             double *stats, double *hist, int hist_cap, double *work)
+{
+    solve_body<NT, SPT, WPS, DYN, STREAM, GEN, FULL, PART, SLDS, SOCK, true>(P, nscen, scen, overrides, z_out, lam_out, stats, hist, hist_cap, work);
 }
 
 template <int UNUSED>
diff --git a/ms-eetc_amd/csrc/msd_kernels_full5.hip b/ms-eetc_amd/csrc/msd_kernels_full5.hip
--- /dev/null
+++ b/ms-eetc_amd/csrc/msd_kernels_full5.hip
@@ -0,0 +1,26 @@
+#include <hip/hip_runtime.h>
+
+#include "msd_geometry.hpp"
+
+namespace msd {
+KernelFn kernels_full5(const KernelId &id)
+{
+#ifndef MSD_HOT_ONLY_64X2
+    MSD_KERNEL_EARLY(64, 1, 1, LOSS_STATIC, false, false, FULL_BOTH, 1)
+    MSD_KERNEL_EARLY(64, 1, 1, LOSS_STATIC, false, false, FULL_BOTH, 3)
+#endif
+    MSD_KERNEL_EARLY(64, 2, 1, LOSS_STATIC, false, false, FULL_BOTH, 1, true)
+    MSD_KERNEL_EARLY(64, 2, 1, LOSS_STATIC, false, false, FULL_BOTH, 3, true)
+    MSD_KERNEL_EARLY(64, 2, 1, LOSS_STATIC, false, false, FULL_BOTH, 1)
+    MSD_KERNEL_EARLY(64, 2, 1, LOSS_STATIC, false, false, FULL_BOTH, 3)
+#ifndef MSD_HOT_ONLY_64X2
+    MSD_KERNEL_EARLY(128, 2, 1, LOSS_STATIC, false, false, FULL_BOTH, 1)
+    MSD_KERNEL_EARLY(128, 2, 1, LOSS_STATIC, false, false, FULL_BOTH, 3)
+    MSD_KERNEL_EARLY(192, 2, 1, LOSS_STATIC, false, false, FULL_BOTH, 1)
+    MSD_KERNEL_EARLY(192, 2, 1, LOSS_STATIC, false, false, FULL_BOTH, 3)
+    MSD_KERNEL_EARLY(256, 2, 1, LOSS_STATIC, false, false, FULL_BOTH, 1)
+    MSD_KERNEL_EARLY(256, 2, 1, LOSS_STATIC, false, false, FULL_BOTH, 3)
+#endif
+    return nullptr;
+}
+}
diff --git a/ms-eetc_amd/csrc/msd_kernels_full6.hip b/ms-eetc_amd/csrc/msd_kernels_full6.hip
--- /dev/null
+++ b/ms-eetc_amd/csrc/msd_kernels_full6.hip
@@ -0,0 +1,12 @@
+#include <hip/hip_runtime.h>
+
+#include "msd_geometry.hpp"
+
+namespace msd {
+KernelFn kernels_full6(const KernelId &id)
+{
+    MSD_KERNEL_EARLY(64, 1, 1, LOSS_STATIC, false, false, FULL_BOTH, 1, false, true)
+    MSD_KERNEL_EARLY(64, 2, 1, LOSS_STATIC, false, false, FULL_BOTH, 1, true, true)
+    return nullptr;
+}
+}
diff --git a/ms-eetc_amd/csrc/msd_kernels_rg3.hip b/ms-eetc_amd/csrc/msd_kernels_rg3.hip
--- /dev/null
+++ b/ms-eetc_amd/csrc/msd_kernels_rg3.hip
@@ -0,0 +1,22 @@
+#include <hip/hip_runtime.h>
+
+#include "msd_geometry.hpp"
+
+namespace msd {
+KernelFn kernels_rg3(const KernelId &id)
+{
+    MSD_KERNEL_EARLY(64, 1, 1, LOSS_STATIC, false, false, FULL_RG, 1)
+    MSD_KERNEL_EARLY(64, 1, 1, LOSS_STATIC, false, false, FULL_RG, 3)
+    MSD_KERNEL_EARLY(64, 2, 1, LOSS_STATIC, false, false, FULL_RG, 1, true)
+    MSD_KERNEL_EARLY(64, 2, 1, LOSS_STATIC, false, false, FULL_RG, 3, true)
+    MSD_KERNEL_EARLY(64, 2, 1, LOSS_STATIC, false, false, FULL_RG, 1)
+    MSD_KERNEL_EARLY(64, 2, 1, LOSS_STATIC, false, false, FULL_RG, 3)
+    MSD_KERNEL_EARLY(128, 2, 1, LOSS_STATIC, false, false, FULL_RG, 1)
+    MSD_KERNEL_EARLY(128, 2, 1, LOSS_STATIC, false, false, FULL_RG, 3)
+    MSD_KERNEL_EARLY(192, 2, 1, LOSS_STATIC, false, false, FULL_RG, 1)
+    MSD_KERNEL_EARLY(192, 2, 1, LOSS_STATIC, false, false, FULL_RG, 3)
+    MSD_KERNEL_EARLY(256, 2, 1, LOSS_STATIC, false, false, FULL_RG, 1)
+    MSD_KERNEL_EARLY(256, 2, 1, LOSS_STATIC, false, false, FULL_RG, 3)
+    return nullptr;
+}
+}
diff --git a/ms-eetc_amd/csrc/msd_select.hpp b/ms-eetc_amd/csrc/msd_select.hpp
--- a/ms-eetc_amd/csrc/msd_select.hpp
+++ b/ms-eetc_amd/csrc/msd_select.hpp
@@ -20,7 +20,10 @@
 inline int structure_of(const msd_problem_desc *d)
 {
     if (d->has_power_rows == 0 || !std::isfinite(d->acc_min) || !std::isfinite(d->acc_max) || !std::isfinite(d->pw_upper) || !std::isfinite(d->pw_lower)) return 0;
-    if (d->energy_optimal != 0) return d->with_pn_brake != 0 ? msd::FULL_BOTH : msd::FULL_RG;
+    if (d->energy_optimal != 0) {
+        if (d->f_min == d->f_max || (d->with_pn_brake != 0 && d->f_min_pn == 0.0)) return 0;
+        return d->with_pn_brake != 0 ? msd::FULL_BOTH : msd::FULL_RG;
+    }
     return d->with_pn_brake != 0 ? msd::FULL_TIME_BOTH : msd::FULL_TIME_RG;
 }
 inline int dyn_of(Family f) { return (f == DYNAMIC || f == GENERAL_DYNAMIC) ? msd::LOSS_TABLE : (f == INTLOSS || f == GENERAL_INTLOSS) ? msd::LOSS_INTEGRATED : f == INTLOSS_TABLE ? msd::LOSS_INTEGRATED_TABLE : msd::LOSS_STATIC; }
diff --git a/ms-eetc_amd/mseetc/_device.py b/ms-eetc_amd/mseetc/_device.py
--- a/ms-eetc_amd/mseetc/_device.py
+++ b/ms-eetc_amd/mseetc/_device.py
@@ -99,6 +99,7 @@
         L.msd_problem_geometry.argtypes = [vp, ctypes.POINTER(ctypes.c_int), ctypes.POINTER(ctypes.c_int)]
         L.msd_synchronize.argtypes = [vp]
         L.msd_problem_follow_counts.argtypes = [vp, ctypes.POINTER(ctypes.c_int), ctypes.c_int]
+        L.msd_problem_last_first_pass.argtypes = [vp, ctypes.c_char_p, ctypes.c_int]
         L.msd_problem_time_first_pass.argtypes = [vp, ctypes.c_int]
         L.msd_problem_first_pass_ms.argtypes = [vp, ctypes.POINTER(ctypes.c_float), ctypes.POINTER(ctypes.c_int)]
         L.msd_device_alloc.argtypes = [vp, ctypes.c_ulonglong, ctypes.POINTER(vp)]
@@ -447,6 +448,11 @@
         _check(lib().msd_problem_follow_counts(self._h, out, 9))
         return int(out[0]), [int(v) for v in out[1:]]
 
+    def last_first_pass(self):
+        buf = ctypes.create_string_buffer(512)
+        _check(lib().msd_problem_last_first_pass(self._h, buf, len(buf)))
+        return buf.value.decode()
+
     def timer_begin(self):
         _check(lib().msd_timer_begin(self._h))
 
```

Result: faster. 1.134 million, median of 6 (+3.3%).
